# Mictronics/multi-sdr-gps-sim

Measured on NVIDIA H100. Metric: IQ Msamples/s, higher is better.
Workload: dtype f64 NCO / int32 accumulate / int8 out

## Files before the change

### include/gpsb200.h

```cpp
#ifndef GPSB200_H
#define GPSB200_H

#include <stdbool.h>
#include <stddef.h>
#include <stdint.h>

#ifdef __cplusplus
extern "C" {
#endif

#define GPSB200_SAMPLERATE        3000000
#define GPSB200_BLOCK_SAMPLES     300000
#define GPSB200_BLOCK_ELEMS       600000
#define GPSB200_MAX_CHAN          32
#define GPSB200_NAV_WORDS         60
#define GPSB200_CA_LEN            1023
#define GPSB200_SC08              1
#define GPSB200_SC16              2
#define GPSB200_HACKRF_BUFFER     262144

enum {
    GPSB200_OK = 0,
    GPSB200_ERR_ARG = -1,
    GPSB200_ERR_CUDA = -2,
    GPSB200_ERR_RANGE = -3,
    GPSB200_ERR_NOMEM = -4,
    GPSB200_ERR_INTERNAL = -5,
    GPSB200_ERR_END = -6
};

typedef struct gpsb200_chan {
    int32_t prn;
    int32_t iword;
    int32_t ibit;
    int32_t icode;
    int32_t nav_frame;
    int32_t reserved;
    double f_carr;
    double f_code;
    double carr_phase;
    double code_phase;
    double gain;
} gpsb200_chan_t;

typedef struct gpsb200_config {
    int32_t device;
    int32_t max_chan;
    int32_t max_blocks;
    int32_t max_nav_frames;
    int32_t host_threads;
    int32_t run_samples;
} gpsb200_config_t;

typedef struct gpsb200_ctx gpsb200_ctx_t;

typedef struct gpsb200_stats {
    double host_chain_ms;
    double h2d_ms, kernel_ms, d2h_ms;
    double checkpoint_kernel_ms, synth_kernel_ms, probe_kernel_ms;
    int64_t h2d_bytes, d2h_bytes;
    int32_t launches;
    int32_t chain_fallbacks;
} gpsb200_stats_t;

int gpsb200_create(const gpsb200_config_t *cfg, gpsb200_ctx_t **out);
void gpsb200_destroy(gpsb200_ctx_t *ctx);
const char *gpsb200_last_error(const gpsb200_ctx_t *ctx);
const char *gpsb200_version(void);

int gpsb200_bind_numa(int device);

int gpsb200_set_nav(gpsb200_ctx_t *ctx, int frame, int chan, const uint32_t dwrd[GPSB200_NAV_WORDS]);

int gpsb200_synth_blocks(gpsb200_ctx_t *ctx, const gpsb200_chan_t *chans, int nblk, int nchan,
                         int sample_size, void *dst, double *carr_phase_out, gpsb200_stats_t *stats);

int gpsb200_synth_blocks_scatter(gpsb200_ctx_t *ctx, const gpsb200_chan_t *chans, int nblk, int nchan,
                                 int sample_size, void *const *dst_blocks, double *carr_phase_out,
                                 gpsb200_stats_t *stats);

int gpsb200_synth_blocks_device(gpsb200_ctx_t *ctx, const gpsb200_chan_t *chans, int nblk, int nchan,
                                int sample_size, void *dst_device, void *stream,
                                double *carr_phase_out, gpsb200_stats_t *stats);

typedef struct gpsb200_slice_link {
    int32_t prn_first[GPSB200_MAX_CHAN];
    int32_t prn_last[GPSB200_MAX_CHAN];
    int32_t reset_inside[GPSB200_MAX_CHAN];
    double first_phase[GPSB200_MAX_CHAN];
    double value[GPSB200_MAX_CHAN];
} gpsb200_slice_link_t;
int gpsb200_slice_prepare(gpsb200_ctx_t *ctx, const gpsb200_chan_t *chans, int nblk, int nchan, int sample_size,
                          void *dst_device, void *dst_host, void *stream, gpsb200_slice_link_t *link);
int gpsb200_slice_wait(gpsb200_ctx_t *ctx);
int gpsb200_slice_probe(gpsb200_ctx_t *ctx, const int32_t *prn_in, const double *phase_guess_in, int eager);
int gpsb200_slice_finish(gpsb200_ctx_t *ctx, const int32_t *prn_in, const double *phase_in, int32_t *prn_out,
                         double *phase_out, gpsb200_stats_t *stats);
typedef void (*gpsb200_handoff_fn)(void *user, const int32_t *prn_out, const double *phase_out);
int gpsb200_slice_finish_cb(gpsb200_ctx_t *ctx, const int32_t *prn_in, const double *phase_in, int32_t *prn_out,
                            double *phase_out, gpsb200_stats_t *stats, gpsb200_handoff_fn handoff, void *user);
int gpsb200_slice_link_host(const gpsb200_chan_t *chans, int nblk, int nchan, gpsb200_slice_link_t *link);
int gpsb200_link_apply(const gpsb200_slice_link_t *link, int nchan, const int32_t *prn_in, const double *phase_in,
                       int32_t *prn_out, double *phase_out);

int gpsb200_debug_corrupt_chain(gpsb200_ctx_t *ctx, int on);

int gpsb200_debug_run_checkpoints(gpsb200_ctx_t *ctx, int nblk, int nchan, void *out);

int gpsb200_debug_block_probes(gpsb200_ctx_t *ctx, int nblk, int nchan, void *probes_out, double *seg_out,
                               double *guess_out);

int gpsb200_debug_synth_shape(gpsb200_ctx_t *ctx, int nblk, int nchan, int sample_size, const char **kernel,
                              int *ctas_per_block, int *runs_per_cta);

const char *gpsb200_synth_kernel_name(const gpsb200_ctx_t *ctx, int nchan);

int gpsb200_replay_device(gpsb200_ctx_t *ctx, void *dst_device, void *stream, int kernel_mask);

double gpsb200_carrier_advance(double carr_phase, double f_carr, int64_t nsamples);

int gpsb200_carrier_chain(const gpsb200_chan_t *chans, int nblk, int nchan, const double *phase_in,
                          double *phase_out, int threads);

int gpsb200_carrier_chain_device(gpsb200_ctx_t *ctx, const gpsb200_chan_t *chans, int nblk, int nchan,
                                 const double *phase_in, double *phase_out);

int gpsb200_carrier_probe_fixup(double start, double guess, double f_carr, int64_t nsamples, double *end_out);

int gpsb200_span_chain_host(const double *f_carr, int nblk, double start_true, double start_guess, double *starts_out);

int gpsb200_checkpoint_segments_host(double start_true, double start_guess, double f_carr, int run_samples,
                                     double *starts_out, int *nseg_out);

int gpsb200_carrier_probe_host(double guess, double f_carr, int64_t nsamples, int run_samples, int mode, void *probe_out,
                               double *seg_out);

int gpsb200_lanes_model_block(const gpsb200_chan_t *chans, int nchan, const uint32_t *nav, int run_samples, int force,
                              int16_t *iq, double *carr_out, int64_t *counters, uint32_t *signs);

int gpsb200_lanes_window_band_host(const uint32_t *steps, const uint32_t *bases, int64_t n, uint8_t *out);

int gpsb200_codegen(int prn, uint8_t ca[GPSB200_CA_LEN]);

#define GPSB200_ACQ_MAX_MS    100
#define GPSB200_ACQ_MAX_BINS  1024
#define GPSB200_ACQ_CODE_SAMPLES 3000
typedef struct gpsb200_acq_config {
    int64_t s0;
    int32_t ms;
    int32_t nprn;
    int32_t prn[32];
    double f_lo_hz;
    double step_hz;
    int32_t nbins;
    int32_t reserved;
} gpsb200_acq_config_t;
typedef struct gpsb200_acq_result {
    int32_t prn;
    int32_t bin;
    int32_t delay;
    int32_t reserved;
    double doppler_hz;
    double delay_chips;
    uint64_t p1, p2;
    double ratio;
} gpsb200_acq_result_t;
int gpsb200_acquire(gpsb200_ctx_t *ctx, const void *iq, int64_t nsamples, int sample_size, const gpsb200_acq_config_t *cfg,
                    gpsb200_acq_result_t *res, uint64_t *grid);
int gpsb200_acquire_device(gpsb200_ctx_t *ctx, const void *iq_device, int64_t nsamples, int sample_size,
                           const gpsb200_acq_config_t *cfg, gpsb200_acq_result_t *res, uint64_t *grid, void *stream);
int gpsb200_acquire_windows(gpsb200_ctx_t *ctx, const void *iq, int64_t nsamples, int sample_size,
                            const gpsb200_acq_config_t *cfg, const double *f_lo_prn, gpsb200_acq_result_t *res,
                            uint64_t *grid);
int gpsb200_debug_acq_split(gpsb200_ctx_t *ctx, int force, int nprn, int nbins);
int gpsb200_acquire_windows_device(gpsb200_ctx_t *ctx, const void *iq_device, int64_t nsamples, int sample_size,
                                   const gpsb200_acq_config_t *cfg, const double *f_lo_prn, gpsb200_acq_result_t *res,
                                   uint64_t *grid, void *stream);

#define GPSB200_TRK_CODE_STEP_NOM 1464583848u
#define GPSB200_TRK_CODE_STEP_MIN 1464095816u
#define GPSB200_TRK_CODE_STEP_MAX 1465072205u
#define GPSB200_TRK_FLL_EPOCHS    200
#define GPSB200_TRK_MAX_CHAN      32
typedef struct gpsb200_track_state {
    int32_t prn;
    int32_t epochs;
    int64_t sample;
    uint64_t code_phase;
    int64_t carr_freq;
    uint32_t carr_phase;
    int32_t carr_step;
    uint32_t code_step;
    int32_t prev_i, prev_q;
    int32_t lock_i, lock_q;
    int32_t lock;
} gpsb200_track_state_t;
typedef struct gpsb200_track_epoch {
    int64_t sample;
    int32_t e_i, e_q, p_i, p_q, l_i, l_q;
    uint32_t carr_phase;
    int32_t carr_step;
    uint32_t code_phase;
    uint32_t code_step;
    int32_t lock;
    int32_t reserved;
} gpsb200_track_epoch_t;
int gpsb200_track_start(int prn, double doppler_hz, int64_t sample, gpsb200_track_state_t *state);
int gpsb200_track(gpsb200_ctx_t *ctx, const void *iq, int64_t nsamples, int sample_size, int64_t base,
                  gpsb200_track_state_t *state, int nchan, int max_epochs, gpsb200_track_epoch_t *epochs,
                  int32_t *nepochs);
int gpsb200_track_device(gpsb200_ctx_t *ctx, const void *iq_device, int64_t nsamples, int sample_size, int64_t base,
                         gpsb200_track_state_t *state, int nchan, int max_epochs, gpsb200_track_epoch_t *epochs,
                         int32_t *nepochs, void *stream);

typedef struct gpsb200_nav_bit {
    int64_t sample;
    int64_t sum;
    int32_t value;
    int32_t locked;
} gpsb200_nav_bit_t;
typedef struct gpsb200_nav_word {
    int64_t sample;
    uint32_t raw;
    uint32_t data;
    int32_t parity_ok;
    int32_t subframe;
    int32_t tow;
    int32_t index;
} gpsb200_nav_word_t;
typedef struct gpsb200_nav_sync {
    int32_t bit_edge;
    int32_t nbits;
    int32_t frame_bit;
    int32_t inverted;
    int32_t nwords;
    int32_t words_ok;
    int32_t subframes;
    int32_t first_tow;
} gpsb200_nav_sync_t;
int gpsb200_nav_decode(const gpsb200_track_epoch_t *epochs, int64_t n, gpsb200_nav_bit_t *bits, int64_t max_bits,
                       gpsb200_nav_word_t *words, int64_t max_words, gpsb200_nav_sync_t *sync);
int gpsb200_nav_word_check(uint32_t word, uint32_t prev, uint32_t *data);
uint32_t gpsb200_nav_parity(uint32_t data24, int d29, int d30);

typedef struct gpsb200_ephemeris {
    int32_t valid;
    int32_t week;
    int32_t iodc, iode;
    int32_t health;
    int32_t ura;
    int32_t reserved[2];
    double toc;
    double af0, af1, af2;
    double tgd;
    double toe;
    double m0, deltan;
    double ecc, sqrta;
    double omg0, inc0, aop;
// ... 362 lines not shown
```

### multi-sdr-gps-sim_b200/api.py

```python
import ctypes as C
import os

import numpy as np

BLOCK_SAMPLES = 300000
BLOCK_ELEMS = 600000
SC08, SC16 = 1, 2

_HERE = os.path.dirname(os.path.abspath(__file__))


def lib_path():
    return os.path.join(_HERE, "libgpsb200.so")


class GpsB200Error(RuntimeError):
    def __init__(self, code, msg):
        super().__init__("gpsb200 error %d: %s" % (code, msg))
        self.code = code


class Chan(C.Structure):
    _fields_ = [("prn", C.c_int32), ("iword", C.c_int32), ("ibit", C.c_int32), ("icode", C.c_int32),
                ("nav_frame", C.c_int32), ("reserved", C.c_int32),
# ... 221 lines not shown
    c["t_a"], c["s_a"], c["week"], c["nodes"] = float(t_a), int(s_a), int(week), int(nodes)
    return c


SNAPSHOT_CONFIG_DTYPE = np.dtype([("min_ratio", "<f8"), ("iterations", "<i4"), ("reserved", "<i4")])
SNAPSHOT_DTYPE = np.dtype([("prn", "<i4"), ("status", "<i4"), ("sample", "<i8"), ("code_phase", "<u8"),
                           ("code_step", "<u4"), ("carr_step", "<i4"), ("iterations", "<i4"), ("last_step", "<i4"),
                           ("power", "<u8"), ("ratio", "<f8")])
assert (SNAPSHOT_CONFIG_DTYPE.itemsize, SNAPSHOT_DTYPE.itemsize) == (16, 56)
SNAP_OK, SNAP_WEAK, SNAP_NO_CONVERGENCE = 0, 1, 2
SNAP_ITERATIONS, SNAP_MAX_ITER = 12, 16
SNAP_BATCH_SCRATCH = 256 << 20


def snapshot_batch_pass(nprn, nbins, ms, sample_size=SC08):
    b = nprn * nbins * 24028 + nprn * 128 + 8 + acq_window_samples(ms) * 2 * int(sample_size)
    return max(1, SNAP_BATCH_SCRATCH // b)


def snapshot_config(min_ratio=2.5, iterations=SNAP_ITERATIONS):
    c = np.zeros(1, SNAPSHOT_CONFIG_DTYPE)[0]
    c["min_ratio"], c["iterations"] = float(min_ratio), int(iterations)
    return c


COLLECTIVE_CONFIG_DTYPE = np.dtype([("n", "<i4", 4), ("step", "<f8", 4), ("mask_deg", "<f8"), ("distinct_m", "<f8"),
                                    ("reserved", "<i8")])
COLLECTIVE_DTYPE = np.dtype([("status", "<i4"), ("nused", "<i4"), ("used", "<u4"), ("shift", "<i4"), ("winner", "<i4"),
                             ("runner", "<i4"), ("score", "<u4"), ("runner_score", "<u4"), ("o_t", "<f8"),
                             ("x", "<f8", 3), ("lat_deg", "<f8"), ("lon_deg", "<f8"), ("height", "<f8"),
                             ("runner_dist", "<f8")])
CD_SCORE_DTYPE = np.dtype([("score", "<u4"), ("shift", "<i4")])
CD_CELL_DTYPE = np.dtype([("bin", "<i4"), ("delay", "<i4")])
assert (COLLECTIVE_CONFIG_DTYPE.itemsize, COLLECTIVE_DTYPE.itemsize) == (72, 96)
CD_OK, CD_FEW, CD_AMBIGUOUS = 0, 1, 2
CD_MAX_HYP, CD_MIN_USED, CD_Q_SHIFT, CD_Q_CAP, CD_AMBIGUOUS_PCT = 1 << 24, 4, 8, 8192, 90


def collective_config(ext_m, step_m, ext_s=0.0, step_s=1.0, up_ext_m=0.0, up_step_m=1.0, mask_deg=5.0,
                      distinct_m=None):
    c = np.zeros(1, COLLECTIVE_CONFIG_DTYPE)[0]
    for a, (e, st) in enumerate(((ext_m, step_m), (ext_m, step_m), (up_ext_m, up_step_m), (ext_s, step_s))):
        c["n"][a] = 2 * int(np.floor(float(e) / float(st) + 1e-9)) + 1 if e > 0 else 1
        c["step"][a] = float(st)
    c["mask_deg"] = float(mask_deg)
    c["distinct_m"] = 2.0 * float(step_m) if distinct_m is None else float(distinct_m)
    return c


def search_nodes(n=SEARCH_NODES):
    xyz = np.zeros((max(1, int(n)), 3))
    rc = lib().gpsb200_search_nodes(int(n), xyz.ctypes.data)
    if rc:
        raise GpsB200Error(rc, "gpsb200_search_nodes")
    return xyz


def rinex_ephemeris(path, week, sow, rinex3=False):
    eph = np.zeros(32, EPHEMERIS_DTYPE)
    rc = lib().gpsb200_rinex_ephemeris(os.fsencode(str(path)), int(bool(rinex3)), int(week), float(sow), eph.ctypes.data)
    if rc:
        raise GpsB200Error(rc, "gpsb200_rinex_ephemeris")
    return eph


def raim_thresholds(p_fa, p_md):
    T, lam = np.zeros(RAIM_MAX_DOF), np.zeros(RAIM_MAX_DOF)
    rc = lib().gpsb200_raim_thresholds(float(p_fa), float(p_md), T.ctypes.data, lam.ctypes.data)
    if rc:
        raise GpsB200Error(rc, "gpsb200_raim_thresholds")
    return T, lam


def nav_words_of_frame(words60):
    w = np.asarray(words60, np.uint32) & 0x3FFFFFFF
    out = np.zeros(w.size, NAV_WORD_DTYPE)
    prev = 0
    for i, raw in enumerate(w):
        ok, data = nav_word_check(int(raw), prev)
        out[i]["raw"], out[i]["data"], out[i]["parity_ok"], out[i]["index"] = int(raw), data, int(ok), i
        out[i]["subframe"], out[i]["tow"] = ((data >> 2) & 7, (data >> 7) & 0x1FFFF) if i % 10 == 1 else (0, -1)
        prev = int(raw)
    return out


def nav_ephemeris(words):
    w = np.ascontiguousarray(words, dtype=NAV_WORD_DTYPE)
    eph, iono = np.zeros(1, EPHEMERIS_DTYPE), np.zeros(1, IONO_DTYPE)
    rc = lib().gpsb200_nav_ephemeris(w.ctypes.data if w.size else None, w.size, eph.ctypes.data, iono.ctypes.data)
    if rc:
        raise GpsB200Error(rc, "gpsb200_nav_ephemeris")
    return eph[0], iono[0]


def nav_almanac(words, week):
    w = np.ascontiguousarray(words, dtype=NAV_WORD_DTYPE)
    rec = np.zeros(32, ALMANAC_RECORD_DTYPE)
    wna = C.c_int32(0)
    rc = lib().gpsb200_nav_almanac(w.ctypes.data if w.size else None, w.size, int(week), rec.ctypes.data, C.byref(wna))
    if rc:
        raise GpsB200Error(rc, "gpsb200_nav_almanac")
    return rec, int(wna.value)


SKY_DTYPE = np.dtype([("prn", "<i4"), ("valid", "<i4"), ("el_deg", "<f8"), ("az_deg", "<f8"), ("range_m", "<f8"),
                      ("doppler_hz", "<f8")])
assert SKY_DTYPE.itemsize == 40


def almanac_predict(rec, week, sow, x_a):
    r = np.ascontiguousarray(rec, dtype=ALMANAC_RECORD_DTYPE)
    assert r.size == 32
    x = np.ascontiguousarray(x_a, dtype=np.float64).reshape(3)
    out = np.zeros(32, SKY_DTYPE)
    rc = lib().gpsb200_almanac_predict(r.ctypes.data, int(week), float(sow), x.ctypes.data, out.ctypes.data)
    if rc:
        raise GpsB200Error(rc, "gpsb200_almanac_predict")
    return out


def nav_time_anchor(words, sync):
    w = np.ascontiguousarray(words, dtype=NAV_WORD_DTYPE)
    sy = np.array(sync, dtype=NAV_SYNC_DTYPE).reshape(1)
    ep, ms = C.c_int32(0), C.c_int64(0)
    rc = lib().gpsb200_nav_time_anchor(w.ctypes.data if w.size else None, w.size, sy.ctypes.data, C.byref(ep), C.byref(ms))
    if rc:
        raise GpsB200Error(rc, "gpsb200_nav_time_anchor")
    return int(ep.value), int(ms.value)


def pvt_config(s0, step, nfix, iono=None):
    c = np.zeros(1, PVT_CONFIG_DTYPE)[0]
    c["s0"], c["step"], c["nfix"] = int(s0), int(step), int(nfix)
    if iono is not None:
        c["iono"] = 1
        c["alpha"], c["beta"] = np.asarray(iono[0], np.float64), np.asarray(iono[1], np.float64)
    return c


HANDOFF_FN = C.CFUNCTYPE(None, C.c_void_p, C.POINTER(C.c_int32), C.POINTER(C.c_double))

_lib = None

EXPORTS = ["gpsb200_create", "gpsb200_destroy", "gpsb200_last_error", "gpsb200_version", "gpsb200_set_nav",
           "gpsb200_synth_blocks", "gpsb200_synth_blocks_scatter", "gpsb200_synth_blocks_device", "gpsb200_replay_device",
           "gpsb200_carrier_advance", "gpsb200_carrier_chain", "gpsb200_carrier_chain_device", "gpsb200_carrier_probe_fixup",
           "gpsb200_codegen", "gpsb200_acquire", "gpsb200_acquire_device", "gpsb200_acquire_windows",
           "gpsb200_acquire_windows_device", "gpsb200_debug_acq_split", "gpsb200_nav_almanac", "gpsb200_almanac_predict", "gpsb200_track_start",
           "gpsb200_track",
           "gpsb200_track_device", "gpsb200_nav_decode", "gpsb200_nav_word_check", "gpsb200_nav_parity",
           "gpsb200_nav_ephemeris", "gpsb200_nav_time_anchor", "gpsb200_pvt", "gpsb200_pvt_replay",
           "gpsb200_pvt_raim", "gpsb200_raim_thresholds", "gpsb200_pvt_araim", "gpsb200_araim_kfa", "gpsb200_pvt_coarse", "gpsb200_pvt_search", "gpsb200_search_nodes", "gpsb200_snapshot_measure", "gpsb200_snapshot_measure_device", "gpsb200_snapshot_batch", "gpsb200_snapshot_batch_device", "gpsb200_pvt_snapshot", "gpsb200_pvt_snapshot_search", "gpsb200_collective", "gpsb200_collective_device", "gpsb200_rinex_ephemeris", "gpsb200_bind_numa", "gpsb200_span_chain_host", "gpsb200_lanes_model_block",
           "gpsb200_lanes_window_band_host", "gpsb200_slice_prepare", "gpsb200_slice_probe",
           "gpsb200_slice_finish", "gpsb200_slice_finish_cb", "gpsb200_slice_wait", "gpsb200_link_apply", "gpsb200_slice_link_host", "gpsb200_debug_corrupt_chain", "gpsb200_synth_kernel_name",
           "gpsb200_debug_run_checkpoints", "gpsb200_checkpoint_segments_host",
           "gpsb200_carrier_probe_host", "gpsb200_debug_block_probes", "gpsb200_debug_synth_shape",
           "gpsb200_scenario_create", "gpsb200_scenario_destroy", "gpsb200_scenario_error",
           "gpsb200_scenario_blocks", "gpsb200_scenario_channels", "gpsb200_scenario_nav_frames",
           "gpsb200_scenario_chans", "gpsb200_scenario_nav", "gpsb200_scenario_almanac_date", "gpsb200_almanac_read",
           "gpsb200_scenario_open", "gpsb200_scenario_advance", "gpsb200_scenario_frame", "gpsb200_scenario_key",
           "gpsb200_scenario_steer_state", "gpsb200_scenario_open_now", "gpsb200_scenario_create_now",
           "gpsb200_scenario_start_date", "gpsb200_scenario_start_time",
           "fifo_create", "fifo_destroy", "fifo_wait_next", "fifo_wait_full", "fifo_halt", "fifo_acquire",
           "fifo_enqueue", "fifo_dequeue", "fifo_release", "fifo_set_compat_drop",
           "gpsb200_iqfile_start", "gpsb200_iqfile_stop", "gpsb200_fifo_push", "gpsb200_fifo_push_flush"]


def lib():
    global _lib
    if _lib is None:
        if not os.path.exists(lib_path()):
            raise GpsB200Error(-2, "libgpsb200.so not built (run __graft_entry__.build()); there is no CPU fallback")
        L = C.CDLL(lib_path())
        L.gpsb200_create.argtypes = [C.POINTER(Config), C.POINTER(C.c_void_p)]
        L.gpsb200_destroy.argtypes = [C.c_void_p]
        L.gpsb200_last_error.argtypes = [C.c_void_p]
        L.gpsb200_last_error.restype = C.c_char_p
        L.gpsb200_version.restype = C.c_char_p
        L.gpsb200_set_nav.argtypes = [C.c_void_p, C.c_int, C.c_int, C.c_void_p]
        L.gpsb200_synth_blocks.argtypes = [C.c_void_p, C.c_void_p, C.c_int, C.c_int, C.c_int, C.c_void_p,
                                           C.c_void_p, C.POINTER(Stats)]
        L.gpsb200_synth_blocks_scatter.argtypes = [C.c_void_p, C.c_void_p, C.c_int, C.c_int, C.c_int, C.c_void_p,
                                                   C.c_void_p, C.POINTER(Stats)]
        L.gpsb200_synth_blocks_device.argtypes = [C.c_void_p, C.c_void_p, C.c_int, C.c_int, C.c_int, C.c_void_p,
                                                  C.c_void_p, C.c_void_p, C.POINTER(Stats)]
        L.gpsb200_replay_device.argtypes = [C.c_void_p, C.c_void_p, C.c_void_p, C.c_int]
        L.gpsb200_carrier_advance.argtypes = [C.c_double, C.c_double, C.c_int64]
        L.gpsb200_carrier_advance.restype = C.c_double
        L.gpsb200_codegen.argtypes = [C.c_int, C.c_void_p]
        L.gpsb200_scenario_create.argtypes = [C.POINTER(ScenarioConfig), C.POINTER(C.c_void_p)]
        L.gpsb200_scenario_destroy.argtypes = [C.c_void_p]
        L.gpsb200_scenario_error.argtypes = [C.c_void_p]
        L.gpsb200_scenario_error.restype = C.c_char_p
        for fn in ("blocks", "channels", "nav_frames"):
            getattr(L, "gpsb200_scenario_" + fn).argtypes = [C.c_void_p]
        L.gpsb200_scenario_chans.argtypes = [C.c_void_p]
        L.gpsb200_scenario_chans.restype = C.c_void_p
        L.gpsb200_scenario_nav.argtypes = [C.c_void_p]
        L.gpsb200_scenario_nav.restype = C.c_void_p
        L.gpsb200_scenario_almanac_date.argtypes = [C.c_void_p]
        L.gpsb200_scenario_almanac_date.restype = C.c_char_p
        L.gpsb200_almanac_read.argtypes = [C.c_char_p, C.c_void_p, C.POINTER(C.c_int32)]
        L.gpsb200_scenario_open.argtypes = [C.POINTER(ScenarioConfig), C.POINTER(C.c_void_p)]
        L.gpsb200_scenario_open_now.argtypes = [C.POINTER(ScenarioConfig), C.POINTER(C.c_void_p)]
        L.gpsb200_scenario_create_now.argtypes = [C.POINTER(ScenarioConfig), C.POINTER(C.c_void_p)]
        L.gpsb200_scenario_start_date.argtypes = [C.c_void_p]
        L.gpsb200_scenario_start_date.restype = C.c_char_p
        L.gpsb200_scenario_start_time.argtypes = [C.c_void_p, C.POINTER(C.c_int32), C.POINTER(C.c_double)]
        L.gpsb200_scenario_advance.argtypes = [C.c_void_p, C.c_int, C.c_void_p, C.POINTER(C.c_int32)]
        L.gpsb200_scenario_frame.argtypes = [C.c_void_p, C.c_int]
        L.gpsb200_scenario_frame.restype = C.c_void_p
        L.gpsb200_scenario_key.argtypes = [C.c_void_p, C.c_int]
        L.gpsb200_scenario_steer_state.argtypes = [C.c_void_p, C.POINTER(SteerState)]
        L.gpsb200_carrier_probe_fixup.argtypes = [C.c_double, C.c_double, C.c_double, C.c_int64, C.POINTER(C.c_double)]
        L.gpsb200_carrier_chain_device.argtypes = [C.c_void_p, C.c_void_p, C.c_int, C.c_int, C.c_void_p, C.c_void_p]
        L.gpsb200_carrier_chain.argtypes = [C.c_void_p, C.c_int, C.c_int, C.c_void_p, C.c_void_p, C.c_int]
        L.gpsb200_span_chain_host.argtypes = [C.c_void_p, C.c_int, C.c_double, C.c_double, C.c_void_p]
        L.gpsb200_slice_prepare.argtypes = [C.c_void_p, C.c_void_p, C.c_int, C.c_int, C.c_int, C.c_void_p, C.c_void_p,
                                            C.c_void_p, C.POINTER(SliceLink)]
        L.gpsb200_slice_finish_cb.argtypes = [C.c_void_p, C.c_void_p, C.c_void_p, C.c_void_p, C.c_void_p, C.POINTER(Stats),
                                              HANDOFF_FN, C.c_void_p]
        L.gpsb200_slice_wait.argtypes = [C.c_void_p]
        L.gpsb200_slice_link_host.argtypes = [C.c_void_p, C.c_int, C.c_int, C.POINTER(SliceLink)]
        L.gpsb200_slice_probe.argtypes = [C.c_void_p, C.c_void_p, C.c_void_p, C.c_int]
        L.gpsb200_slice_finish.argtypes = [C.c_void_p, C.c_void_p, C.c_void_p, C.c_void_p, C.c_void_p, C.POINTER(Stats)]
        L.gpsb200_link_apply.argtypes = [C.POINTER(SliceLink), C.c_int, C.c_void_p, C.c_void_p, C.c_void_p, C.c_void_p]
        L.gpsb200_debug_corrupt_chain.argtypes = [C.c_void_p, C.c_int]
        L.gpsb200_debug_run_checkpoints.argtypes = [C.c_void_p, C.c_int, C.c_int, C.c_void_p]
        L.gpsb200_checkpoint_segments_host.argtypes = [C.c_double, C.c_double, C.c_double, C.c_int, C.c_void_p,
                                                       C.POINTER(C.c_int)]
        L.gpsb200_carrier_probe_host.argtypes = [C.c_double, C.c_double, C.c_int64, C.c_int, C.c_int, C.c_void_p,
                                                 C.c_void_p]
        L.gpsb200_debug_block_probes.argtypes = [C.c_void_p, C.c_int, C.c_int, C.c_void_p, C.c_void_p, C.c_void_p]
        L.gpsb200_debug_synth_shape.argtypes = [C.c_void_p, C.c_int, C.c_int, C.c_int, C.POINTER(C.c_char_p),
                                                C.POINTER(C.c_int), C.POINTER(C.c_int)]
        L.gpsb200_synth_kernel_name.argtypes = [C.c_void_p, C.c_int]
        L.gpsb200_synth_kernel_name.restype = C.c_char_p
        L.gpsb200_acquire.argtypes = [C.c_void_p, C.c_void_p, C.c_int64, C.c_int, C.POINTER(AcqConfig), C.c_void_p,
                                      C.c_void_p]
        L.gpsb200_acquire_device.argtypes = [C.c_void_p, C.c_void_p, C.c_int64, C.c_int, C.POINTER(AcqConfig),
                                             C.c_void_p, C.c_void_p, C.c_void_p]
        L.gpsb200_acquire_windows.argtypes = [C.c_void_p, C.c_void_p, C.c_int64, C.c_int, C.POINTER(AcqConfig),
                                              C.c_void_p, C.c_void_p, C.c_void_p]
        L.gpsb200_acquire_windows_device.argtypes = [C.c_void_p, C.c_void_p, C.c_int64, C.c_int, C.POINTER(AcqConfig),
                                                     C.c_void_p, C.c_void_p, C.c_void_p, C.c_void_p]
        L.gpsb200_debug_acq_split.argtypes = [C.c_void_p, C.c_int, C.c_int, C.c_int]
        L.gpsb200_nav_almanac.argtypes = [C.c_void_p, C.c_int64, C.c_int32, C.c_void_p, C.POINTER(C.c_int32)]
        L.gpsb200_almanac_predict.argtypes = [C.c_void_p, C.c_int32, C.c_double, C.c_void_p, C.c_void_p]
        L.gpsb200_track_start.argtypes = [C.c_int, C.c_double, C.c_int64, C.c_void_p]
        L.gpsb200_track.argtypes = [C.c_void_p, C.c_void_p, C.c_int64, C.c_int, C.c_int64, C.c_void_p, C.c_int, C.c_int,
                                    C.c_void_p, C.c_void_p]
        L.gpsb200_track_device.argtypes = [C.c_void_p, C.c_void_p, C.c_int64, C.c_int, C.c_int64, C.c_void_p, C.c_int,
                                           C.c_int, C.c_void_p, C.c_void_p, C.c_void_p]
        L.gpsb200_nav_decode.argtypes = [C.c_void_p, C.c_int64, C.c_void_p, C.c_int64, C.c_void_p, C.c_int64, C.c_void_p]
        L.gpsb200_nav_word_check.argtypes = [C.c_uint32, C.c_uint32, C.POINTER(C.c_uint32)]
        L.gpsb200_nav_parity.argtypes = [C.c_uint32, C.c_int, C.c_int]
        L.gpsb200_nav_parity.restype = C.c_uint32
        L.gpsb200_nav_ephemeris.argtypes = [C.c_void_p, C.c_int64, C.c_void_p, C.c_void_p]
        L.gpsb200_nav_time_anchor.argtypes = [C.c_void_p, C.c_int64, C.c_void_p, C.POINTER(C.c_int32),
                                              C.POINTER(C.c_int64)]
        L.gpsb200_pvt.argtypes = [C.c_void_p, C.c_void_p, C.c_int, C.c_void_p, C.c_void_p, C.c_int, C.c_void_p, C.c_void_p,
                                  C.c_void_p]
        L.gpsb200_pvt_replay.argtypes = [C.c_void_p, C.c_void_p]
        L.gpsb200_pvt_raim.argtypes = [C.c_void_p, C.c_void_p, C.c_int, C.c_void_p, C.c_void_p, C.c_int, C.c_void_p,
                                       C.c_void_p, C.c_void_p, C.c_void_p, C.c_void_p]
        L.gpsb200_raim_thresholds.argtypes = [C.c_double, C.c_double, C.c_void_p, C.c_void_p]
        L.gpsb200_pvt_araim.argtypes = L.gpsb200_pvt_raim.argtypes
        L.gpsb200_araim_kfa.argtypes = [C.c_double, C.c_double, C.c_void_p, C.c_void_p]
        L.gpsb200_pvt_coarse.argtypes = L.gpsb200_pvt_raim.argtypes + [C.c_void_p]
        L.gpsb200_pvt_search.argtypes = L.gpsb200_pvt_coarse.argtypes + [C.c_void_p]
        L.gpsb200_search_nodes.argtypes = [C.c_int, C.c_void_p]
        L.gpsb200_snapshot_measure.argtypes = [C.c_void_p, C.c_void_p, C.c_int64, C.c_int, C.POINTER(AcqConfig),
                                               C.c_void_p, C.c_void_p, C.c_void_p]
        L.gpsb200_snapshot_measure_device.argtypes = L.gpsb200_snapshot_measure.argtypes + [C.c_void_p]
        L.gpsb200_snapshot_batch.argtypes = [C.c_void_p, C.c_void_p, C.c_int64, C.c_int, C.POINTER(AcqConfig), C.c_int,
                                             C.c_void_p, C.c_void_p, C.c_void_p, C.c_void_p, C.c_void_p]
        L.gpsb200_snapshot_batch_device.argtypes = L.gpsb200_snapshot_batch.argtypes + [C.c_void_p]
        L.gpsb200_pvt_snapshot.argtypes = [C.c_void_p, C.c_void_p, C.c_int, C.c_void_p, C.c_void_p, C.c_void_p,
                                           C.c_void_p, C.c_void_p, C.c_void_p, C.c_void_p]
        L.gpsb200_pvt_snapshot_search.argtypes = L.gpsb200_pvt_snapshot.argtypes + [C.c_void_p]
        L.gpsb200_collective.argtypes = [C.c_void_p, C.c_void_p, C.c_int64, C.c_int, C.POINTER(AcqConfig), C.c_void_p,
                                         C.c_void_p, C.c_void_p, C.c_void_p, C.c_void_p, C.c_void_p, C.c_void_p,
                                         C.c_void_p, C.c_void_p]
        L.gpsb200_collective_device.argtypes = L.gpsb200_collective.argtypes + [C.c_void_p]
        L.gpsb200_rinex_ephemeris.argtypes = [C.c_char_p, C.c_int, C.c_int32, C.c_double, C.c_void_p]
        _lib = L
    return _lib


def bind_numa(device=0):
    L = lib()
    L.gpsb200_bind_numa.argtypes = [C.c_int]
    L.gpsb200_bind_numa.restype = C.c_int
    return int(L.gpsb200_bind_numa(int(device)))


def codegen(prn):
    ca = np.zeros(1023, np.uint8)
    rc = lib().gpsb200_codegen(prn, ca.ctypes.data)
    if rc:
        raise GpsB200Error(rc, "gpsb200_codegen(%d)" % prn)
    return ca


def carrier_advance(phase, f_carr, nsamples):
    return lib().gpsb200_carrier_advance(float(phase), float(f_carr), int(nsamples))


def carrier_chain(chans, phase_in=None, threads=16):
    a = np.ascontiguousarray(chans, dtype=CHAN_DTYPE)
    nblk, nchan = a.shape
    out = np.zeros(nchan, np.float64)
    pin = None if phase_in is None else np.ascontiguousarray(phase_in, dtype=np.float64)
    rc = lib().gpsb200_carrier_chain(a.ctypes.data, nblk, nchan, None if pin is None else pin.ctypes.data,
                                     out.ctypes.data, threads)
    if rc:
        raise GpsB200Error(rc, "gpsb200_carrier_chain")
    return out


def lanes_model_block(chans_row, nav_frame, run_samples=2400, force=0, want_signs=False):
    a = np.ascontiguousarray(chans_row, dtype=CHAN_DTYPE)
    nv = np.ascontiguousarray(nav_frame, dtype=np.uint32)
    iq = np.zeros(BLOCK_ELEMS, np.int16)
    co = np.zeros(a.size, np.float64)
    cnt = np.zeros(4, np.int64)
    signs = np.zeros((a.size, BLOCK_SAMPLES // 96, 3), np.uint32) if want_signs else None
    L = lib()
    L.gpsb200_lanes_model_block.argtypes = [C.c_void_p, C.c_int, C.c_void_p, C.c_int, C.c_int, C.c_void_p, C.c_void_p, C.c_void_p,
                                            C.c_void_p]
    rc = L.gpsb200_lanes_model_block(a.ctypes.data, a.size, nv.ctypes.data, run_samples, force, iq.ctypes.data, co.ctypes.data,
                                     cnt.ctypes.data, None if signs is None else signs.ctypes.data)
    if rc:
        raise GpsB200Error(rc, "gpsb200_lanes_model_block")
    return (iq, co, cnt, signs) if want_signs else (iq, co, cnt)


def lanes_window_band(steps, bases):
    st, bs = np.broadcast_arrays(np.asarray(steps, np.uint32), np.asarray(bases, np.uint32))
    st = np.ascontiguousarray(st.ravel())
    bs = np.ascontiguousarray(bs.ravel())
    out = np.zeros(st.size, np.uint8)
    L = lib()
    L.gpsb200_lanes_window_band_host.argtypes = [C.c_void_p, C.c_void_p, C.c_int64, C.c_void_p]
    rc = L.gpsb200_lanes_window_band_host(st.ctypes.data, bs.ctypes.data, st.size, out.ctypes.data)
    if rc:
        raise GpsB200Error(rc, "gpsb200_lanes_window_band_host")
    return out.astype(bool)


def span_chain_host(f_carr, start_true, start_guess):
    f = np.ascontiguousarray(f_carr, dtype=np.float64)
    out = np.zeros(f.size + 1)
    rc = lib().gpsb200_span_chain_host(f.ctypes.data, f.size, float(start_true), float(start_guess), out.ctypes.data)
    if rc < 0:
        raise GpsB200Error(rc, "gpsb200_span_chain_host")
    return out if rc == 1 else None


def checkpoint_segments_host(start_true, start_guess, f_carr, run_samples=2400):
    out = np.zeros(8)
    nseg = C.c_int(0)
    rc = lib().gpsb200_checkpoint_segments_host(float(start_true), float(start_guess), float(f_carr), int(run_samples),
                                            out.ctypes.data, C.byref(nseg))
    if rc < 0:
        raise GpsB200Error(rc, "gpsb200_checkpoint_segments_host")
    return rc == 1, out[:nseg.value]


def carrier_probe_host(guess, f_carr, nsamples=BLOCK_SAMPLES, run_samples=2400, mode=1):
    probe = np.zeros(1, CARRIER_PROBE_DTYPE)
    seg = np.zeros((2, 7))
    rc = lib().gpsb200_carrier_probe_host(float(guess), float(f_carr), int(nsamples), int(run_samples), int(mode),
                                          probe.ctypes.data, seg.ctypes.data)
    if rc:
        raise GpsB200Error(rc, "gpsb200_carrier_probe_host")
    return probe[0], seg


def slice_link_host(chans):
# ... 141 lines not shown
        self._check(lib().gpsb200_scenario_key(self._h, ord(k) if isinstance(k, str) else int(k)))

    def state(self):
        st = SteerState()
        self._check(lib().gpsb200_scenario_steer_state(self._h, C.byref(st)))
        return st

    def run(self, steer, chunk=None):
        events = {}
        for b, keys, rep in steer:
            events[int(b)] = events.get(int(b), "") + keys * int(rep)
        parts, frames = [], {}
        b = 0
        while True:
            if b in events:
                for k in events.pop(b):
                    self.key(k)
            st = self.state()
            if st.next_block >= st.end_block:
                break
            nxt = min([e for e in events if e > b] + [st.end_block])
            n = nxt - b if chunk is None else min(chunk, nxt - b)
            ch = self.advance(n)
            for f in np.unique(ch["nav_frame"]):
                if f not in frames:
                    frames[int(f)] = self.frame(int(f))
            parts.append(ch)
            b += ch.shape[0]
        chans = np.concatenate(parts) if parts else np.zeros((0, self.channels), CHAN_DTYPE)
        nav = np.stack([frames[f] for f in sorted(frames)]) if frames else np.zeros((0, self.channels, 60), np.uint32)
        return chans, nav


class Context:

    def __init__(self, max_chan, max_blocks, device=0, max_nav_frames=1, host_threads=0, run_samples=0):
        self._h = C.c_void_p()
        self.cfg = Config(device, max_chan, max_blocks, max_nav_frames, host_threads, run_samples)
        rc = lib().gpsb200_create(C.byref(self.cfg), C.byref(self._h))
        if rc:
            msg = lib().gpsb200_last_error(self._h).decode() if self._h else "gpsb200_create: bad configuration"
            if self._h:
                lib().gpsb200_destroy(self._h)
                self._h = C.c_void_p()
            raise GpsB200Error(rc, msg)

    def close(self):
        if self._h:
            lib().gpsb200_destroy(self._h)
            self._h = C.c_void_p()

    def __enter__(self):
        return self

    def __exit__(self, *a):
        self.close()

    def _check(self, rc):
        if rc:
            raise GpsB200Error(rc, lib().gpsb200_last_error(self._h).decode())

    def set_nav(self, frame, chan, words):
        w = np.ascontiguousarray(words, dtype=np.uint32)
        assert w.size == 60
        self._check(lib().gpsb200_set_nav(self._h, frame, chan, w.ctypes.data))

    def set_nav_frames(self, frames):
        for f in range(frames.shape[0]):
            for c in range(frames.shape[1]):
                self.set_nav(f, c, frames[f, c])

    @staticmethod
    def _chans(chans):
        a = np.ascontiguousarray(chans, dtype=CHAN_DTYPE)
        assert a.ndim == 2
        return a

    def synth_blocks(self, chans, sample_size=SC08, out=None, want_stats=False):
        a = self._chans(chans)
        nblk, nchan = a.shape
        dt = np.int16 if sample_size == SC16 else np.int8
        if out is None:
            out = np.empty(nblk * BLOCK_ELEMS, dt)
        assert out.dtype == dt and out.size >= nblk * BLOCK_ELEMS and out.flags.c_contiguous
        cp = np.zeros(nchan, np.float64)
        st = Stats()
        self._check(lib().gpsb200_synth_blocks(self._h, a.ctypes.data, nblk, nchan, sample_size,
                                               out.ctypes.data, cp.ctypes.data, C.byref(st)))
        return (out, cp, st) if want_stats else (out, cp)

    def synth_blocks_scatter(self, chans, sample_size, blocks, want_stats=False):
        a = self._chans(chans)
        nblk, nchan = a.shape
        dt = np.int16 if sample_size == SC16 else np.int8
        assert len(blocks) == nblk and all(b.dtype == dt and b.size >= BLOCK_ELEMS and b.flags.c_contiguous for b in blocks)
        ptrs = (C.c_void_p * nblk)(*[b.ctypes.data for b in blocks])
        cp = np.zeros(nchan, np.float64)
        st = Stats()
        self._check(lib().gpsb200_synth_blocks_scatter(self._h, a.ctypes.data, nblk, nchan, sample_size,
                                                       C.cast(ptrs, C.c_void_p), cp.ctypes.data, C.byref(st)))
        return (cp, st) if want_stats else cp

    def synth_blocks_device(self, chans, sample_size, dst_ptr, stream=0, want_stats=False):
        a = self._chans(chans)
        nblk, nchan = a.shape
        cp = np.zeros(nchan, np.float64)
        st = Stats()
        self._check(lib().gpsb200_synth_blocks_device(self._h, a.ctypes.data, nblk, nchan, sample_size,
                                                      C.c_void_p(dst_ptr), C.c_void_p(stream), cp.ctypes.data,
                                                      C.byref(st) if want_stats else None))
        return (cp, st) if want_stats else cp

    def slice_prepare(self, chans, sample_size, dst_ptr=0, stream=0, dst_host=None):
        a = self._chans(chans)
        nblk, nchan = a.shape
        link = SliceLink()
        hp = None if dst_host is None else C.c_void_p(dst_host.ctypes.data)
        self._check(lib().gpsb200_slice_prepare(self._h, a.ctypes.data, nblk, nchan, sample_size, C.c_void_p(dst_ptr),
                                                hp, C.c_void_p(stream), C.byref(link)))
        self._slice_nchan = nchan
        return link

    def slice_probe(self, prn_in=None, phase_guess_in=None, eager=False):
        pi = None if prn_in is None else np.ascontiguousarray(prn_in, dtype=np.int32)
        xi = None if phase_guess_in is None else np.ascontiguousarray(phase_guess_in, dtype=np.float64)
        self._check(lib().gpsb200_slice_probe(self._h, None if pi is None else pi.ctypes.data,
                                              None if xi is None else xi.ctypes.data, 1 if eager else 0))

    def slice_finish(self, prn_in=None, phase_in=None, want_stats=False, handoff=None):
        n = self._slice_nchan
        pi = None if prn_in is None else np.ascontiguousarray(prn_in, dtype=np.int32)
        xi = None if phase_in is None else np.ascontiguousarray(phase_in, dtype=np.float64)
        po, xo = np.zeros(n, np.int32), np.zeros(n, np.float64)
        st = Stats()

        def _cb(_user, p_prn, p_ph):
            handoff(np.ctypeslib.as_array(p_prn, shape=(n,)).copy(), np.ctypeslib.as_array(p_ph, shape=(n,)).copy())

        cb = HANDOFF_FN(_cb) if handoff is not None else C.cast(None, HANDOFF_FN)
        self._check(lib().gpsb200_slice_finish_cb(self._h, None if pi is None else pi.ctypes.data,
                                                  None if xi is None else xi.ctypes.data, po.ctypes.data, xo.ctypes.data,
                                                  C.byref(st), cb, None))
        return (po, xo, st) if want_stats else (po, xo)

    def slice_wait(self):
        self._check(lib().gpsb200_slice_wait(self._h))

    def synth_kernel_name(self, nchan):
        return lib().gpsb200_synth_kernel_name(self._h, int(nchan)).decode()

    def debug_corrupt_chain(self, on):
        self._check(lib().gpsb200_debug_corrupt_chain(self._h, int(on)))

    def debug_run_checkpoints(self, nblk, nchan):
        nruns = BLOCK_SAMPLES // (self.cfg.run_samples or 2400)
        out = np.zeros((nblk, nruns, nchan), RUN_CKPT_DTYPE)
        self._check(lib().gpsb200_debug_run_checkpoints(self._h, nblk, nchan, out.ctypes.data))
        return out

    def debug_block_probes(self, nblk, nchan):
        probes = np.zeros((nblk, nchan), CARRIER_PROBE_DTYPE)
        seg = np.zeros((nblk, nchan, 2, 7))
        guess = np.zeros((nblk, nchan))
        self._check(lib().gpsb200_debug_block_probes(self._h, nblk, nchan, probes.ctypes.data, seg.ctypes.data,
                                                     guess.ctypes.data))
        return probes, seg, guess

    def debug_synth_shape(self, nblk, nchan, sample_size=SC08):
        name, per_block, per_cta = C.c_char_p(), C.c_int(0), C.c_int(0)
        self._check(lib().gpsb200_debug_synth_shape(self._h, int(nblk), int(nchan), int(sample_size), C.byref(name),
                                                    C.byref(per_block), C.byref(per_cta)))
        return name.value.decode(), per_block.value, per_cta.value

    def carrier_chain(self, chans, phase_in=None):
        a = self._chans(chans)
        nblk, nchan = a.shape
        out = np.zeros(nchan, np.float64)
        pin = None if phase_in is None else np.ascontiguousarray(phase_in, dtype=np.float64)
        self._check(lib().gpsb200_carrier_chain_device(self._h, a.ctypes.data, nblk, nchan,
                                                       None if pin is None else pin.ctypes.data, out.ctypes.data))
        return out

    def acquire(self, iq=None, sample_size=SC08, prns=range(1, 33), ms=10, s0=0, f_lo=-5000.0, step=250.0, nbins=41,
                want_grid=False, device_ptr=None, nsamples=None, stream=0):
        return self._acquire(None, iq, sample_size, [int(p) for p in prns], ms, s0, f_lo, step, nbins, want_grid,
                             device_ptr, nsamples, stream)

    def acquire_windows(self, iq=None, sample_size=SC08, prns=(), f_lo_prn=(), step=250.0, nbins=5, ms=10, s0=0,
                        want_grid=False, device_ptr=None, nsamples=None, stream=0):
        prns = [int(p) for p in prns]
        flo = np.ascontiguousarray(f_lo_prn, dtype=np.float64).reshape(-1)
        if flo.size != len(prns):
            raise GpsB200Error(ERR_ARG, "acquire_windows: %d first bins for %d PRNs" % (flo.size, len(prns)))
        return self._acquire(flo, iq, sample_size, prns, ms, s0, 0.0, step, nbins, want_grid, device_ptr, nsamples,
                             stream)

    def _acquire(self, f_lo_prn, iq, sample_size, prns, ms, s0, f_lo, step, nbins, want_grid, device_ptr, nsamples,
                 stream):
        cfg = self._acq_config(prns, ms, s0, f_lo, step, nbins)
        res = np.zeros(max(1, min(len(prns), 32)), ACQ_RESULT_DTYPE)
        grid = np.zeros((max(1, len(prns)), max(1, int(nbins)), ACQ_CODE_SAMPLES), np.uint64) if want_grid else None
        gp = None if grid is None else grid.ctypes.data
        src, n, dev = self._rx_source(iq, device_ptr, nsamples, stream)
        if f_lo_prn is None:
            fn, fp = lib().gpsb200_acquire_device if dev else lib().gpsb200_acquire, ()
        else:
            fn = lib().gpsb200_acquire_windows_device if dev else lib().gpsb200_acquire_windows
            fp = (f_lo_prn.ctypes.data if f_lo_prn.size else None,)
        self._check(fn(self._h, src, n, int(sample_size), C.byref(cfg), *fp, res.ctypes.data, gp, *dev))
        return (res, grid) if want_grid else res

    @staticmethod
    def _acq_config(prns, ms, s0, f_lo, step, nbins):
        cfg = AcqConfig()
        cfg.s0, cfg.ms, cfg.nprn = int(s0), int(ms), len(prns)
        for i, p in enumerate(prns[:32]):
            cfg.prn[i] = p
        cfg.f_lo_hz, cfg.step_hz, cfg.nbins = float(f_lo), float(step), int(nbins)
        return cfg

    @staticmethod
    def _rx_source(iq, device_ptr, nsamples, stream):
        if device_ptr is not None:
            assert iq is None and nsamples is not None
            return C.c_void_p(device_ptr), int(nsamples), (C.c_void_p(stream),)
        a = np.ascontiguousarray(iq)
        n = a.size // 2 if nsamples is None else int(nsamples)
        assert n <= a.size // 2
        return a.ctypes, n, ()

    def debug_acq_split(self, nprn, nbins, force=-1):
        rc = lib().gpsb200_debug_acq_split(self._h, int(force), int(nprn), int(nbins))
        if rc < 0:
            self._check(rc)
        return rc

    def track(self, states, iq=None, sample_size=SC08, base=0, max_epochs=None, device_ptr=None, nsamples=None, stream=0):
        st = np.array(states, dtype=TRACK_STATE_DTYPE).reshape(-1).copy()
        nchan = st.size
        src, n, dev = self._rx_source(iq, device_ptr, nsamples, stream)
        me = int(max_epochs) if max_epochs is not None else n // 2999 + 1
        out = np.zeros((max(1, nchan), max(1, me)), TRACK_EPOCH_DTYPE)
        cnt = np.zeros(max(1, nchan), np.int32)
        fn = lib().gpsb200_track_device if dev else lib().gpsb200_track
        self._check(fn(self._h, src, n, int(sample_size), int(base), st.ctypes.data, nchan, me, out.ctypes.data,
                       cnt.ctypes.data, *dev))
        return [out[c, :cnt[c]].copy() for c in range(nchan)], st

    def pvt(self, chans, epochs, cfg, want_residuals=False, nepochs=None):
        ch, nchan, ep, n, me, cf, fixes, res = self._pvt_args(chans, epochs, cfg, want_residuals, nepochs)
        self._check(lib().gpsb200_pvt(self._h, ch.ctypes.data, nchan, ep.ctypes.data, n.ctypes.data, me, cf.ctypes.data,
                                      fixes.ctypes.data, None if res is None else res.ctypes.data))
        return (fixes, res) if want_residuals else fixes

    def pvt_raim(self, chans, epochs, cfg, raim, want_residuals=False, nepochs=None):
        ch, nchan, ep, n, me, cf, fixes, res = self._pvt_args(chans, epochs, cfg, want_residuals, nepochs)
        rc = np.array(raim, dtype=RAIM_CONFIG_DTYPE).reshape(1)
        out = np.zeros(fixes.size, RAIM_DTYPE)
        self._check(lib().gpsb200_pvt_raim(self._h, ch.ctypes.data, nchan, ep.ctypes.data, n.ctypes.data, me,
                                           cf.ctypes.data, rc.ctypes.data, fixes.ctypes.data,
                                           None if res is None else res.ctypes.data, out.ctypes.data))
        return (fixes, out, res) if want_residuals else (fixes, out)

    def pvt_araim(self, chans, epochs, cfg, araim, want_residuals=False, nepochs=None):
        ch, nchan, ep, n, me, cf, fixes, res = self._pvt_args(chans, epochs, cfg, want_residuals, nepochs)
        ac = np.array(araim, dtype=ARAIM_CONFIG_DTYPE).reshape(1)
        out = np.zeros(fixes.size, ARAIM_DTYPE)
        self._check(lib().gpsb200_pvt_araim(self._h, ch.ctypes.data, nchan, ep.ctypes.data, n.ctypes.data, me,
                                            cf.ctypes.data, ac.ctypes.data, fixes.ctypes.data,
                                            None if res is None else res.ctypes.data, out.ctypes.data))
        return (fixes, out, res) if want_residuals else (fixes, out)

    def pvt_coarse(self, chans, epochs, cfg, apriori, want_residuals=False, want_ms=False, nepochs=None):
        ch, nchan, ep, n, me, cf, fixes, res = self._pvt_args(chans, epochs, cfg, want_residuals, nepochs)
        ap = np.array(apriori, dtype=COARSE_CONFIG_DTYPE).reshape(1)
        out = np.zeros(fixes.size, COARSE_DTYPE)
        ms = np.zeros((fixes.size, max(1, nchan)), np.int64) if want_ms else None
        self._check(lib().gpsb200_pvt_coarse(self._h, ch.ctypes.data, nchan, ep.ctypes.data, n.ctypes.data, me,
                                             cf.ctypes.data, ap.ctypes.data, fixes.ctypes.data,
                                             None if res is None else res.ctypes.data, out.ctypes.data,
                                             None if ms is None else ms.ctypes.data))
        return (fixes, out) + ((res,) if want_residuals else ()) + ((ms,) if want_ms else ())

    def pvt_search(self, chans, epochs, cfg, search, want_residuals=False, want_ms=False, want_node_rms=False,
                   nepochs=None):
        ch, nchan, ep, n, me, cf, fixes, res = self._pvt_args(chans, epochs, cfg, want_residuals, nepochs)
        sc = np.array(search, dtype=SEARCH_CONFIG_DTYPE).reshape(1)
        out = np.zeros(fixes.size, SEARCH_DTYPE)
        ms = np.zeros((fixes.size, max(1, nchan)), np.int64) if want_ms else None
        nr = np.zeros((fixes.size, max(1, int(sc[0]["nodes"]))), np.float64) if want_node_rms else None
        self._check(lib().gpsb200_pvt_search(self._h, ch.ctypes.data, nchan, ep.ctypes.data, n.ctypes.data, me,
                                             cf.ctypes.data, sc.ctypes.data, fixes.ctypes.data,
                                             None if res is None else res.ctypes.data, out.ctypes.data,
                                             None if ms is None else ms.ctypes.data,
                                             None if nr is None else nr.ctypes.data))
        return ((fixes, out) + ((res,) if want_residuals else ()) + ((ms,) if want_ms else ())
                + ((nr,) if want_node_rms else ()))

    def snapshot_measure(self, res, iq=None, sample_size=SC08, ms=10, s0=0, prns=None, f_lo=-5000.0, step=250.0,
                         nbins=41, cfg=None, device_ptr=None, nsamples=None, stream=0):
        r = np.ascontiguousarray(res, dtype=ACQ_RESULT_DTYPE).reshape(-1)
        prns = [int(p) for p in (r["prn"] if prns is None else prns)]
        acq = self._acq_config(prns, ms, s0, f_lo, step, nbins)
        sc = np.array(snapshot_config() if cfg is None else cfg, dtype=SNAPSHOT_CONFIG_DTYPE).reshape(1)
        if r.size < len(prns):
            raise GpsB200Error(ERR_ARG, "snapshot_measure: %d results for %d PRNs" % (r.size, len(prns)))
# ... 125 lines not shown
```

### multi-sdr-gps-sim_b200/csrc/gpsb200_api.cu

```cuda
#include <cuda_runtime.h>
#include <sched.h>

#include <algorithm>
#include <atomic>
#include <chrono>
#include <condition_variable>
#include <functional>
#include <mutex>
#include <cctype>
#include <cmath>
#include <cstdio>
#include <cstring>
#include <memory>
#include <string>
#include <thread>
#include <vector>

#include "../../include/gpsb200.h"
#include "acquire.h"
#include "snapshot.h"
#include "collective.h"
#include "device_buffer.h"
#include "track.h"
#include "pvt.h"
#include "nco_exact.h"
#include "synth_kernels.h"
#include "synth_lanes.h"
#include "synth_tables.h"

using namespace gpsb200;

namespace {

constexpr int kSynthChunk = 256;
constexpr int kSegFirst = 256;
constexpr int kSegBlocks = 1024;
constexpr int kSpanBlocks = 32;
constexpr int kHostChainBlocks = 2;

struct ChainState {
    int prn = 0;
    double phase = 0.0;
};

class WorkerPool {
public:
    explicit WorkerPool(int n) {
        for (int i = 0; i < n; i++) th_.emplace_back([this, i] { loop(i); });
    }
    ~WorkerPool() {
        {
            std::lock_guard<std::mutex> lk(mu_);
            stop_ = true;
        }
        cv_.notify_all();
        for (auto &t : th_) t.join();
    }
    int size() const { return (int) th_.size(); }
    void run(int n, const std::function<void(int, int)> &job) {
        const int parts = std::max(1, std::min(size(), n));
        if (parts <= 1 || th_.empty()) {
            job(0, n);
            return;
        }
        std::unique_lock<std::mutex> lk(mu_);
        job_ = &job;
        n_ = n;
        parts_ = parts;
        pending_ = parts;
        ++epoch_;
        cv_.notify_all();
        done_.wait(lk, [this] { return pending_ == 0; });
        job_ = nullptr;
    }

private:
    void loop(int id) {
        uint64_t seen = 0;
        for (;;) {
            const std::function<void(int, int)> *job;
            int n, parts;
            {
                std::unique_lock<std::mutex> lk(mu_);
                cv_.wait(lk, [&] { return stop_ || epoch_ != seen; });
                if (stop_) return;
                seen = epoch_;
                job = job_;
                n = n_;
                parts = parts_;
            }
            if (id < parts) {
                const int per = (n + parts - 1) / parts, lo = id * per, hi = std::min(n, lo + per);
                if (lo < hi) (*job)(lo, hi);
                std::lock_guard<std::mutex> lk(mu_);
                if (--pending_ == 0) done_.notify_all();
            }
        }
    }
    std::vector<std::thread> th_;
    std::mutex mu_;
    std::condition_variable cv_, done_;
    const std::function<void(int, int)> *job_ = nullptr;
    int n_ = 0, parts_ = 0, pending_ = 0;
    uint64_t epoch_ = 0;
    bool stop_ = false;
};

std::vector<std::pair<int, int>> segments_of(int nblk) {
    std::vector<std::pair<int, int>> v;
    int len = kSegFirst;
    for (int b0 = 0; b0 < nblk; len = kSegBlocks) {
        const int b1 = std::min(nblk, b0 + len);
        v.emplace_back(b0, b1);
        b0 = b1;
    }
    return v;
}

struct Call {
    const gpsb200_chan_t *chans = nullptr;
    int nblk = 0, nchan = 0, sample_size = 0;
    void *dst = nullptr;
    void *dst_host = nullptr;
    void *const *scatter = nullptr;
    cudaStream_t stream = nullptr;
    std::vector<std::pair<int, int>> segs;
    std::vector<ChainState> chain;
    std::vector<std::vector<ChainState>> after;
    std::vector<int64_t> slow;
    int rows = 0;
    int ichunk = 0;
    gpsb200_stats_t st{};
    bool active = false, eager = false, probed = false, finished = false;

    Call() = default;
    Call(const gpsb200_chan_t *chans_, int nblk_, int nchan_, int sample_size_, void *dst_, void *dst_host_,
         void *const *scatter_, cudaStream_t stream_)
        : chans(chans_), nblk(nblk_), nchan(nchan_), sample_size(sample_size_), dst(dst_), dst_host(dst_host_),
          scatter(scatter_), stream(stream_), chain(nchan_) {
        plan(segments_of(nblk_));
    }
    void plan(std::vector<std::pair<int, int>> s) {
        segs = std::move(s);
        after.assign(segs.size(), {});
        slow.assign(segs.size(), 0);
    }
    bool host() const { return dst_host || scatter; }
};

enum { kEvCallStart, kEvProbeStart, kEvProbeEnd, kEvCkptStart, kEvCkptEnd, kEvCallEnd, kCallEvents };

}

struct gpsb200_ctx {
    gpsb200_config_t cfg{};
    int nruns = 0;
    cudaStream_t s_compute = nullptr, s_copy = nullptr, s_pre = nullptr, s_ck = nullptr;
    cudaEvent_t ev[kCallEvents]{};
    std::vector<cudaEvent_t> ev_done;
    BlockChanDev *d_bc = nullptr, *h_bc = nullptr;
    RunCkpt *d_ck = nullptr, *h_ck = nullptr;
    uint32_t *d_nav = nullptr, *h_nav = nullptr;
    uint32_t *d_chips = nullptr;
    int32_t *d_atab = nullptr;
    double *d_carr_end = nullptr;
    int *d_chain_errors = nullptr, *h_chain_errors = nullptr;
    double *d_guess = nullptr, *h_guess = nullptr;
    std::vector<uint8_t> h_guess_abs;
    std::vector<uint8_t> h_span_flags;
    double *d_carr0 = nullptr, *h_carr0 = nullptr;
    CarrierProbe *d_probe = nullptr;
    CarrierProbe *h_probe = nullptr, *d_probe_host = nullptr;
    double *d_seg = nullptr;
    CarrierProbe *h_span_sum = nullptr, *d_span_sum = nullptr;
    SpanBlockState *d_spec = nullptr;
    bool lanes_on = true;
    bool lanes_veto = false;
    SpanRes *d_span_res = nullptr, *h_span_res = nullptr;
    int max_spans = 0;
    double *h_seg_end = nullptr, *d_seg_end = nullptr;
    std::vector<double> seg_expect;
    std::vector<cudaEvent_t> ev_seg;
    int fault_inject_chain = 0;
    bool trace_on = false;
    double trace_t0 = 0.0;
    Call call;
    uint8_t *d_out = nullptr;
    size_t out_bytes = 0;
    uint8_t *d_rx = nullptr;
    size_t rx_bytes = 0;
    int8_t *d_rx_chips = nullptr;
    bool nav_dirty = true;
    std::unique_ptr<WorkerPool> pool;
    SynthArgs last{};
    bool have_last = false;
    acq::Scratch acq;
    trk::Scratch trk;
    pvt::Scratch pvt;
    snap::Scratch snap;
    cd::Scratch cd;
    std::string err;
};

namespace {

struct OneSatellite {
    const double *cc;
    __host__ __device__ void operator()(int j, double &c, int32_t &prn) const {
        c = cc[j];
        prn = 1;
    }
};

double now_ms();
void trace(gpsb200_ctx *ctx, const char *what);

int fail(gpsb200_ctx *c, int code, const std::string &msg) {
    if (c) c->err = msg;
    return code;
}

#define CU(call)                                                                              \
    do {                                                                                      \
        cudaError_t e_ = (call);                                                              \
        if (e_ != cudaSuccess)                                                                \
            return fail(ctx, GPSB200_ERR_CUDA, std::string(#call) + ": " + cudaGetErrorString(e_)); \
    } while (0)

double now_ms() {
    using namespace std::chrono;
    return duration<double, std::milli>(steady_clock::now().time_since_epoch()).count();
}

void trace(gpsb200_ctx *ctx, const char *what) {
    if (!ctx->trace_on) return;
    const double t = now_ms();
    fprintf(stderr, "[gpsb200 dev %d +%8.3f ms] %s (%d host workers)\n", ctx->cfg.device, t - ctx->trace_t0, what,
            ctx->pool ? ctx->pool->size() : 0);
}

inline uint64_t phase_to_fix(double p) { return (p >= 0.0 && p < 1.0) ? (uint64_t) (p * 0x1p64) : 0; }
inline double fix_to_phase(uint64_t a) { return (double) (a >> 11) * 0x1p-53; }
inline uint64_t step_to_fix(double c) {
    const uint64_t m = (uint64_t) (std::fabs(c) * 0x1p64);
    return c < 0.0 ? (uint64_t) 0 - m : m;
}
inline uint64_t guess_block(uint64_t acc, double c) {
    acc += (uint64_t) GPSB200_BLOCK_SAMPLES * step_to_fix(c);
    return acc + (uint64_t) (int64_t) ((double) GPSB200_BLOCK_SAMPLES * carrier_drift_per_step(c) * 0x1p64);
}


int prepare_blocks(gpsb200_ctx *ctx, const gpsb200_chan_t *chans, int b0, int b1, int nchan,
                   const std::vector<ChainState> &chain, gpsb200_slice_link_t *link = nullptr,
                   std::vector<ChainState> *end_guess = nullptr) {
    const double delt = 1.0 / (double) GPSB200_SAMPLERATE;
    std::vector<int> status(nchan, GPSB200_OK);
    std::vector<uint8_t> lanes_bad(nchan, 0);
    ctx->pool->run(nchan, [&](int c_lo, int c_hi) {
        for (int c = c_lo; c < c_hi; c++) {
            uint64_t acc = phase_to_fix(chain[c].phase);
            int prev_prn = chain[c].prn;
            bool absolute = link == nullptr;
            if (link) {
                acc = 0;
                prev_prn = chans[(size_t) b0 * nchan + c].prn;
                link->prn_first[c] = prev_prn;
                link->first_phase[c] = prev_prn > 0 ? chans[(size_t) b0 * nchan + c].carr_phase : 0.0;
            }
            int span_first_prn = 0;
            uint8_t span_idle = 1, span_uniform = 1;
            for (int b = b0; b < b1; b++) {
                const gpsb200_chan_t &in = chans[(size_t) b * nchan + c];
                const size_t i = (size_t) b * nchan + c;
                BlockChanDev &o = ctx->h_bc[i];
                memset(&o, 0, sizeof o);
                if (b % kSpanBlocks == 0) {
                    span_first_prn = in.prn;
                    span_idle = span_uniform = 1;
                }
                span_idle &= in.prn <= 0;
                span_uniform &= in.prn == span_first_prn;
                if ((b + 1) % kSpanBlocks == 0 || b + 1 == b1)
                    ctx->h_span_flags[(size_t) (b / kSpanBlocks) * nchan + c] = (uint8_t) (span_idle | (span_uniform << 1));
                ctx->h_guess[i] = 0.0;
                ctx->h_guess_abs[i] = absolute ? 1 : 0;
                if (in.prn <= 0) {
                    prev_prn = 0;
                    absolute = true;
                    continue;
                }
                if (in.prn > 32 || in.iword < 0 || in.iword >= GPSB200_NAV_WORDS || in.ibit < 0 || in.ibit >= 30 ||
                    in.icode < 0 || in.icode >= 20 || in.nav_frame < 0 || in.nav_frame >= ctx->cfg.max_nav_frames ||
                    !(in.code_phase >= 0.0 && in.code_phase < 1023.0) ||
                    !(in.f_code > 0.0 && in.f_code <= 1.07e6) ||
                    !(std::isfinite(in.f_carr) && std::fabs(in.f_carr) < 2.9e6) || !std::isfinite(in.gain)) {
                    status[c] = GPSB200_ERR_ARG;
                    return;
                }
                if (!(in.carr_phase >= 0.0 && in.carr_phase < 1.0)) {
                    status[c] = GPSB200_ERR_ARG;
                    return;
                }
                if (in.prn != prev_prn) {
                    acc = phase_to_fix(in.carr_phase);
                    absolute = true;
                }
                ctx->h_guess_abs[i] = absolute ? 1 : 0;
                prev_prn = in.prn;
                o.c_carr = in.f_carr * delt;
                o.c_code = in.f_code * delt;
                if (!lanes::code_step_ok(o.c_code) || !(std::fabs(o.c_carr) < 0.5)) lanes_bad[c] = 1;
                o.gain = in.gain;
                o.carr_in = in.carr_phase;
                o.code0 = in.code_phase;
                o.prn = in.prn;
                o.nav0 = (uint32_t) in.iword | ((uint32_t) in.ibit << 8) | ((uint32_t) in.icode << 16);
                o.frame = in.nav_frame;
                ctx->h_guess[i] = fix_to_phase(acc);
                acc = guess_block(acc, o.c_carr);
            }
            if (end_guess) {
                (*end_guess)[c].prn = prev_prn > 0 ? prev_prn : 0;
                (*end_guess)[c].phase = prev_prn > 0 ? fix_to_phase(acc) : 0.0;
            }
            if (link) {
                link->prn_last[c] = prev_prn > 0 ? prev_prn : 0;
                link->reset_inside[c] = absolute ? 1 : 0;
                link->value[c] = fix_to_phase(acc);
            }
        }
    });
    for (int c = 0; c < nchan; c++)
        if (status[c] != GPSB200_OK) return fail(ctx, status[c], "invalid channel parameters in slot " + std::to_string(c));
    for (int c = 0; c < nchan; c++)
        if (lanes_bad[c]) ctx->lanes_veto = true;
    for (int b = b0; b < b1; b++) {
        double amp = 0.0;
        for (int c = 0; c < nchan; c++) amp += std::fabs(ctx->h_bc[(size_t) b * nchan + c].gain) * 250.0;
        if (amp > 32767.0) return fail(ctx, GPSB200_ERR_RANGE, "sum of channel amplitudes exceeds int16 range");
    }
    return GPSB200_OK;
}

void finalize_guesses(gpsb200_ctx *ctx, int b0, int b1, int nchan, const int32_t *prn_in, const double *phase_in) {
    ctx->pool->run(nchan, [&](int c_lo, int c_hi) {
        for (int c = c_lo; c < c_hi; c++) {
            const BlockChanDev &first = ctx->h_bc[(size_t) b0 * nchan + c];
            const bool cont = prn_in && phase_in && first.prn > 0 && prn_in[c] == first.prn;
            const double off = cont ? phase_in[c] : first.carr_in;
            for (int b = b0; b < b1; b++) {
                const size_t i = (size_t) b * nchan + c;
                if (ctx->h_guess_abs[i] || ctx->h_bc[i].prn <= 0) continue;
                double g = ctx->h_guess[i] + off;
                if (g >= 1.0) g -= 1.0;
                if (!(g >= 0.0 && g < 1.0)) g = 0.0;
                ctx->h_guess[i] = g;
            }
        }
    });
}

void reanchor_guesses(gpsb200_ctx *ctx, int b0, int b1, int nchan, const std::vector<ChainState> &chain) {
    ctx->pool->run(nchan, [&](int c_lo, int c_hi) {
        for (int c = c_lo; c < c_hi; c++) {
            const BlockChanDev &first = ctx->h_bc[(size_t) b0 * nchan + c];
            if (first.prn <= 0 || chain[c].prn != first.prn) continue;
            double delta = chain[c].phase - ctx->h_guess[(size_t) b0 * nchan + c];
            if (delta > 0.5) delta -= 1.0;
            if (delta < -0.5) delta += 1.0;
            for (int b = b0; b < b1; b++) {
                const size_t i = (size_t) b * nchan + c;
                if (ctx->h_bc[i].prn != first.prn) break;
                double g = ctx->h_guess[i] + delta;
                if (g >= 1.0) g -= 1.0;
                if (g < 0.0) g += 1.0;
                if (!(g >= 0.0 && g < 1.0)) g = 0.0;
                ctx->h_guess[i] = g;
            }
        }
    });
}

inline int resolve_block(ChainState &st, const BlockChanDev &bc, const CarrierProbe &probe, double &start_out) {
    if (bc.prn <= 0) {
        st.prn = 0;
        start_out = 0.0;
        return 0;
    }
    if (st.prn != bc.prn) st.phase = bc.carr_in;
    st.prn = bc.prn;
    start_out = st.phase;
    double xe;
    if (carrier_fixup(st.phase, bc.c_carr, probe, xe)) {
        st.phase = xe;
        return 0;
    }
    int64_t dummy = 0;
    nco_advance<NCO_CARRIER>(st.phase, bc.c_carr, GPSB200_BLOCK_SAMPLES, dummy);
    return 1;
}

int64_t resolve_chain(gpsb200_ctx *ctx, int b0, int b1, int nchan, std::vector<ChainState> &chain, int64_t *spans_slow) {
    std::vector<int64_t> fallbacks(nchan, 0), slow(nchan, 0);
    const int K = kSpanBlocks;
    const int nspan = (b1 - b0 + K - 1) / K;
    ctx->pool->run(nchan, [&](int c_lo, int c_hi) {
        for (int c = c_lo; c < c_hi; c++) {
            ChainState st = chain[c];
            for (int sp = 0; sp < nspan; sp++) {
                const int s0 = b0 + sp * K, s1 = std::min(b1, s0 + K);
                SpanRes &res = ctx->h_span_res[(size_t) (s0 / K) * nchan + c];
                const BlockChanDev &first = ctx->h_bc[(size_t) s0 * nchan + c];
                const uint8_t flags = ctx->h_span_flags[(size_t) (s0 / K) * nchan + c];
                const bool idle = flags & 1, uniform = flags & 2;
                res.start = res.shift = 0.0;
                res.variant = 0;
                if (idle) {
                    res.mode = 2;
                    st.prn = 0;
                    continue;
                }
                if (uniform && first.prn > 0) {
                    const double start = st.prn == first.prn ? st.phase : first.carr_in;
                    const CarrierProbe &sum = ctx->h_span_sum[(size_t) (s0 / K) * nchan + c];
                    double xe, d;
                    int v;
                    if (carrier_fixup(start, first.c_carr, sum, xe, &v, &d, 1.0)) {
                        res.mode = 0;
                        res.start = start;
                        res.shift = d;
                        res.variant = v;
                        st.prn = first.prn;
                        st.phase = xe;
                        continue;
                    }
                }
                res.mode = 1;
                ++slow[c];
                for (int b = s0; b < s1; b++) {
                    const size_t i = (size_t) b * nchan + c;
                    fallbacks[c] += resolve_block(st, ctx->h_bc[i], ctx->h_probe[i], ctx->h_carr0[i]);
                }
            }
            chain[c] = st;
        }
    });
    if (ctx->fault_inject_chain == 1 && b1 - b0 > 6) {
        SpanRes &r = ctx->h_span_res[(size_t) (b0 / K) * nchan];
        if (r.mode == 0) r.shift += 0x1p-51;
        else if (r.mode == 1) ctx->h_carr0[(size_t) (b0 + 5) * nchan] += 0x1p-51;
    }
    int64_t n = 0;
    for (int c = 0; c < nchan; c++) {
        n += fallbacks[c];
        if (spans_slow) *spans_slow += slow[c];
    }
    return n;
}

SynthArgs make_args(gpsb200_ctx *ctx, int blk0, int nblk, int nchan, int sample_size, void *out) {
    SynthArgs a{};
    const size_t off = (size_t) blk0 * nchan;
    a.bc = ctx->d_bc + off;
    a.carr0 = ctx->d_carr0 + off;
    a.guess = ctx->d_guess + off;
    a.probe = ctx->d_probe + off;
    a.probe_host = ctx->d_probe_host + off;
    a.seg = ctx->d_seg + off * kSegStates;
    a.spec = ctx->d_spec + off;
    a.span_blocks = kSpanBlocks;
    a.nspan = (nblk + kSpanBlocks - 1) / kSpanBlocks;
    a.span_sum = ctx->d_span_sum + (size_t) (blk0 / kSpanBlocks) * nchan;
    a.span_res = ctx->d_span_res + (size_t) (blk0 / kSpanBlocks) * nchan;
    a.ck = ctx->d_ck + off * ctx->nruns;
    a.nav = ctx->d_nav;
    a.nav_stride = ctx->cfg.max_chan;
    a.chipbits = ctx->d_chips;
    a.atab = ctx->d_atab + (size_t) blk0 * kAtabRows * 32;
    a.carr_end = ctx->d_carr_end + off;
    a.chain_errors = ctx->d_chain_errors;
    a.out = out;
    a.nblk = nblk;
    a.nchan = nchan;
    a.nruns = ctx->nruns;
    a.run_samples = ctx->cfg.run_samples;
    a.iq16 = sample_size == GPSB200_SC16;
    a.lanes = ctx->lanes_on && !ctx->lanes_veto ? 1 : 0;
    const int grp = nchan > 16 ? 32 : (nchan > 8 ? 16 : 8);
    const int rpw = 32 / grp;
    int per_cta = 24 * rpw;
    const int ctas = (ctx->nruns + per_cta - 1) / per_cta;
    per_cta = (ctx->nruns + ctas - 1) / ctas;
    a.runs_per_cta = per_cta;
    a.ctas_per_block = ctas;
    return a;
}

SynthArgs call_args(gpsb200_ctx *ctx, const Call &call, int b0, int nb) {
    const size_t blk_bytes = (size_t) GPSB200_BLOCK_ELEMS * call.sample_size;
    return make_args(ctx, b0, nb, call.nchan, call.sample_size, (char *) call.dst + (size_t) b0 * blk_bytes);
}

int upload_nav(gpsb200_ctx *ctx, cudaStream_t s) {
    if (!ctx->nav_dirty) return GPSB200_OK;
    const size_t bytes = (size_t) ctx->cfg.max_nav_frames * ctx->cfg.max_chan * GPSB200_NAV_WORDS * 4;
    CU(cudaMemcpyAsync(ctx->d_nav, ctx->h_nav, bytes, cudaMemcpyHostToDevice, s));
    ctx->nav_dirty = false;
    return GPSB200_OK;
}

int check_entry(gpsb200_ctx *ctx) {
    if (!ctx->s_compute) return fail(ctx, GPSB200_ERR_CUDA, "context has no CUDA device");
    if (ctx->call.active) return fail(ctx, GPSB200_ERR_ARG, "a call begun with gpsb200_slice_prepare has not been finished");
    CU(cudaSetDevice(ctx->cfg.device));
    return GPSB200_OK;
}

int check_call(gpsb200_ctx *ctx, const gpsb200_chan_t *chans, int nblk, int nchan, int sample_size, void *dst) {
    if (!chans || !dst || nblk < 1 || nblk > ctx->cfg.max_blocks || nchan < 1 || nchan > ctx->cfg.max_chan ||
        (sample_size != GPSB200_SC08 && sample_size != GPSB200_SC16))
        return fail(ctx, GPSB200_ERR_ARG, "bad arguments (1 <= nchan <= cfg.max_chan; 1 <= nblk <= cfg.max_blocks)");
    return check_entry(ctx);
}

int check_aligned(gpsb200_ctx *ctx, const void *p, const char *fn, const char *arg) {
    if ((reinterpret_cast<uintptr_t>(p) & 15u) != 0)
        return fail(ctx, GPSB200_ERR_ARG, std::string(fn) + ": " + arg + " is not 16-byte aligned");
    return GPSB200_OK;
}

int ensure_staging(gpsb200_ctx *ctx, int sample_size) {
    CU(grow(ctx->d_out, ctx->out_bytes, (size_t) ctx->cfg.max_blocks * GPSB200_BLOCK_ELEMS * sample_size));
    return GPSB200_OK;
}

int rx_source(gpsb200_ctx *ctx, const char *fn, const void *iq, int64_t first, int64_t count, int sample_size,
              bool device, cudaStream_t s, const void **dev) {
    int rc = device ? check_aligned(ctx, iq, fn, "iq_device") : GPSB200_OK;
    if (!rc) rc = check_entry(ctx);
    if (rc) return rc;
    const size_t elem = sample_size == GPSB200_SC16 ? 4 : 2;
    *dev = static_cast<const char *>(iq) + (size_t) first * elem;
    if (device) return GPSB200_OK;
    CU(grow(ctx->d_rx, ctx->rx_bytes, (size_t) count * elem));
    if (count) CU(cudaMemcpyAsync(ctx->d_rx, *dev, (size_t) count * elem, cudaMemcpyHostToDevice, s));
    *dev = ctx->d_rx;
    return GPSB200_OK;
}

int settle(gpsb200_ctx *ctx, cudaStream_t caller, int rc) {
    if (rc == GPSB200_OK) return rc;
    ctx->call.active = false;
    if (!ctx->s_compute) return rc;
    if (caller) cudaStreamSynchronize(caller);
    cudaStreamSynchronize(ctx->s_compute);
    cudaStreamSynchronize(ctx->s_pre);
    cudaStreamSynchronize(ctx->s_ck);
    cudaStreamSynchronize(ctx->s_copy);
    return rc;
}

cudaStream_t caller_stream(gpsb200_ctx *ctx, void *stream_) {
    return stream_ ? (cudaStream_t) stream_ : ctx->s_compute;
}


int call_open(gpsb200_ctx *ctx, const Call &call) {
    CU(cudaEventRecord(ctx->ev[kEvCallStart], call.stream));
    CU(cudaStreamWaitEvent(ctx->s_pre, ctx->ev[kEvCallStart], 0));
    CU(cudaStreamWaitEvent(ctx->s_ck, ctx->ev[kEvCallStart], 0));
    const int rc = upload_nav(ctx, ctx->s_pre);
    if (rc) return rc;
    CU(cudaMemsetAsync(ctx->d_chain_errors, 0, sizeof(int), ctx->s_pre));
    return GPSB200_OK;
}

int seg_params(gpsb200_ctx *ctx, Call &call, int b0, int b1, cudaStream_t sp, std::vector<ChainState> *guessed,
               gpsb200_slice_link_t *link) {
    const size_t off = (size_t) b0 * call.nchan, cnt = (size_t) (b1 - b0) * call.nchan;
    const double t0 = now_ms();
    const int rc = prepare_blocks(ctx, call.chans, b0, b1, call.nchan, guessed ? *guessed : call.chain, link, guessed);
    if (rc) return rc;
    call.st.host_chain_ms += now_ms() - t0;
    CU(cudaMemcpyAsync(ctx->d_bc + off, ctx->h_bc + off, cnt * sizeof(BlockChanDev), cudaMemcpyHostToDevice, sp));
    call.st.h2d_bytes += (int64_t) (cnt * sizeof(BlockChanDev));
    if (call.dst) {
        CU(launch_tables(call_args(ctx, call, b0, b1 - b0), sp));
        call.st.launches += 1;
    }
    return GPSB200_OK;
}

int seg_probe(gpsb200_ctx *ctx, Call &call, int b0, int b1, cudaStream_t sp) {
    const size_t off = (size_t) b0 * call.nchan, cnt = (size_t) (b1 - b0) * call.nchan;
    SynthArgs a = make_args(ctx, b0, b1 - b0, call.nchan, call.sample_size, nullptr);
    if (!call.dst) a.ck = nullptr;
    CU(cudaMemcpyAsync(ctx->d_guess + off, ctx->h_guess + off, cnt * sizeof(double), cudaMemcpyHostToDevice, sp));
    if (b0 == 0) CU(cudaEventRecord(ctx->ev[kEvProbeStart], sp));
    CU(launch_probe(a, sp));
    CU(launch_chain(a, sp));
    if (b0 == 0) CU(cudaEventRecord(ctx->ev[kEvProbeEnd], sp));
    call.st.launches += 2;
    call.st.h2d_bytes += (int64_t) (cnt * sizeof(double));
    call.st.d2h_bytes += (int64_t) (cnt * sizeof(CarrierProbe) + (size_t) a.nspan * call.nchan * sizeof(CarrierProbe));
    return GPSB200_OK;
}

int seg_scan(gpsb200_ctx *ctx, Call &call, int i, cudaEvent_t probes_done, cudaStream_t sp) {
    if (probes_done) CU(cudaEventSynchronize(probes_done));
    else CU(cudaStreamSynchronize(sp));
    const double t0 = now_ms();
    call.slow[i] = 0;
    call.st.chain_fallbacks +=
        (int32_t) resolve_chain(ctx, call.segs[i].first, call.segs[i].second, call.nchan, call.chain, &call.slow[i]);
    call.st.host_chain_ms += now_ms() - t0;
    call.after[i] = call.chain;
    return GPSB200_OK;
}

int download(gpsb200_ctx *ctx, Call &call, int b0, int b1, cudaStream_t s) {
    const size_t blk_bytes = (size_t) GPSB200_BLOCK_ELEMS * call.sample_size;
    const char *src = (const char *) call.dst;
    if (call.scatter) {
        for (int b = b0; b < b1; b++)
            CU(cudaMemcpyAsync(call.scatter[b], src + (size_t) b * blk_bytes, blk_bytes, cudaMemcpyDeviceToHost, s));
    } else {
        CU(cudaMemcpyAsync((char *) call.dst_host + (size_t) b0 * blk_bytes, src + (size_t) b0 * blk_bytes,
                           (size_t) (b1 - b0) * blk_bytes, cudaMemcpyDeviceToHost, s));
    }
    call.st.d2h_bytes += (int64_t) (b1 - b0) * (int64_t) blk_bytes;
    return GPSB200_OK;
}

int seg_commit(gpsb200_ctx *ctx, Call &call, int i0, int i1, cudaStream_t sp) {
    const int b0 = call.segs[i0].first, b1 = call.segs[i1 - 1].second, nchan = call.nchan;
    const size_t off = (size_t) b0 * nchan, cnt = (size_t) (b1 - b0) * nchan;
    int64_t slow = 0;
    for (int i = i0; i < i1; i++) slow += call.slow[i];
    SynthArgs a = call_args(ctx, call, b0, b1 - b0);
    const size_t soff = (size_t) (b0 / kSpanBlocks) * nchan, scnt = (size_t) a.nspan * nchan;
    if (b0 == 0) CU(cudaEventRecord(ctx->ev[kEvCkptStart], sp));
    CU(cudaMemcpyAsync(ctx->d_span_res + soff, ctx->h_span_res + soff, scnt * sizeof(SpanRes), cudaMemcpyHostToDevice, sp));
    call.st.h2d_bytes += (int64_t) (scnt * sizeof(SpanRes));
    if (slow > 0) {
        CU(cudaMemcpyAsync(ctx->d_carr0 + off, ctx->h_carr0 + off, cnt * sizeof(double), cudaMemcpyHostToDevice, sp));
        call.st.h2d_bytes += (int64_t) (cnt * sizeof(double));
    }
    const int jm = ckpt_segments(ctx->nruns) / 2;
    if (ctx->fault_inject_chain == 2 && b1 - b0 > 6 && jm >= 1) {
        double *p = ctx->d_seg + (size_t) (b0 + 5) * nchan * kSegStates, h[kSegStates];
        CU(cudaMemcpyAsync(h, p, sizeof h, cudaMemcpyDeviceToHost, sp));
        CU(cudaStreamSynchronize(sp));
        h[jm - 1] += 0x1p-51;
        h[kCkptSegs - 1 + jm - 1] += 0x1p-51;
        CU(cudaMemcpyAsync(p, h, sizeof h, cudaMemcpyHostToDevice, sp));
        CU(cudaStreamSynchronize(sp));
    }
    SynthArgs ack = a;
    ack.last_end_host = ctx->d_seg_end + (size_t) i0 * nchan;
    CU(launch_checkpoints(ack, sp));
    if (b0 == 0) CU(cudaEventRecord(ctx->ev[kEvCkptEnd], sp));
    call.st.launches += 1;
    for (int c = 0; c < nchan; c++) {
        const ChainState &e = call.after[i1 - 1][c];
        const bool live = e.prn > 0 && ctx->h_bc[(size_t) (b1 - 1) * nchan + c].prn == e.prn;
        ctx->seg_expect[(size_t) i0 * nchan + c] = live ? e.phase : -1.0;
    }
    call.rows = i0 + 1;
    CU(cudaEventRecord(ctx->ev_done[call.ichunk], sp));
    CU(cudaStreamWaitEvent(call.stream, ctx->ev_done[call.ichunk], 0));
    call.ichunk++;
    if (!call.host()) {
        CU(launch_synth(a, call.stream));
        call.st.launches += 1;
        return GPSB200_OK;
    }
    for (int c0 = b0, nc = 0; c0 < b1; c0 += nc, call.ichunk++) {
        nc = c0 == 0 ? 32 : (c0 == 32 ? 96 : (c0 == 128 ? 128 : kSynthChunk));
        nc = std::min(nc, b1 - c0);
        CU(launch_synth(call_args(ctx, call, c0, nc), call.stream));
        call.st.launches += 1;
        CU(cudaEventRecord(ctx->ev_done[call.ichunk], call.stream));
        CU(cudaStreamWaitEvent(ctx->s_copy, ctx->ev_done[call.ichunk], 0));
        const int rc = download(ctx, call, c0, c0 + nc, ctx->s_copy);
        if (rc) return rc;
    }
    return GPSB200_OK;
}

int call_close(gpsb200_ctx *ctx, const Call &call, cudaStream_t sp) {
    CU(cudaEventRecord(ctx->ev[kEvCallEnd], call.stream));
    CU(cudaMemcpyAsync(ctx->h_chain_errors, ctx->d_chain_errors, sizeof(int), cudaMemcpyDeviceToHost, sp));
    ctx->last = call_args(ctx, call, 0, call.nblk);
    ctx->have_last = true;
    return GPSB200_OK;
}

int call_verdict(gpsb200_ctx *ctx, const Call &call) {
    int bad = *ctx->h_chain_errors;
    for (int i = 0; i < call.rows; i++)
        for (int c = 0; c < call.nchan; c++) {
            const double want = ctx->seg_expect[(size_t) i * call.nchan + c];
            if (want >= 0.0 && f64_bits(want) != f64_bits(ctx->h_seg_end[(size_t) i * call.nchan + c])) ++bad;
        }
    if (bad != 0)
        return fail(ctx, GPSB200_ERR_INTERNAL, "carrier chain self-check failed on " + std::to_string(bad) + " blocks");
    return GPSB200_OK;
}

void seed_chain(std::vector<ChainState> &chain, int nchan, const int32_t *prn_in, const double *phase_in) {
    for (int c = 0; c < nchan; c++) {
        chain[c].prn = (prn_in && phase_in && prn_in[c] > 0) ? prn_in[c] : 0;
        chain[c].phase = chain[c].prn ? phase_in[c] : 0.0;
    }
}

void export_chain(const std::vector<ChainState> &chain, int nchan, int32_t *prn_out, double *phase_out) {
    for (int c = 0; c < nchan; c++) {
        if (prn_out) prn_out[c] = chain[c].prn;
        if (phase_out) phase_out[c] = chain[c].prn > 0 ? chain[c].phase : 0.0;
    }
}

int small_call(gpsb200_ctx *ctx, Call &call, double *carr_phase_out, gpsb200_stats_t *stats) {
    const int nblk = call.nblk, nchan = call.nchan;
    cudaStream_t s = call.stream;
    double t0 = now_ms();
    int rc = prepare_blocks(ctx, call.chans, 0, nblk, nchan, call.chain);
    if (rc) return rc;
    const int nruns = ctx->nruns, run = ctx->cfg.run_samples;
    ctx->pool->run(nchan, [&](int c_lo, int c_hi) {
        for (int c = c_lo; c < c_hi; c++) {
            ChainState stc = call.chain[c];
            for (int b = 0; b < nblk; b++) {
                const BlockChanDev &p = ctx->h_bc[(size_t) b * nchan + c];
                RunCkpt *ck = ctx->h_ck + (size_t) b * nruns * nchan + c;
                if (p.prn <= 0) {
                    stc.prn = 0;
                    for (int r = 0; r < nruns; r++) ck[(size_t) r * nchan] = RunCkpt{0.0, 0.0, 0u, 0u};
                    continue;
                }
                if (stc.prn != p.prn) stc.phase = p.carr_in;
                stc.prn = p.prn;
                double x = stc.phase, y = p.code0;
                int iword = p.nav0 & 0xFF, ibit = (p.nav0 >> 8) & 0xFF, icode = (p.nav0 >> 16) & 0xFF;
                const WalkConst wx = walk_const(p.c_carr), wy = walk_const(p.c_code);
                for (int r = 0; r < nruns; r++) {
                    ck[(size_t) r * nchan] = RunCkpt{x, y, (uint32_t) iword | ((uint32_t) ibit << 8) | ((uint32_t) icode << 16), 0u};
                    int64_t periods = 0, dummy = 0;
                    nco_advance<NCO_CARRIER>(x, wx, run, dummy);
                    nco_advance<NCO_CODE>(y, wy, run, periods);
                    nav_advance(iword, ibit, icode, periods);
                }
                stc.phase = x;
            }
            call.chain[c] = stc;
        }
    });
    call.st.host_chain_ms = now_ms() - t0;
    rc = upload_nav(ctx, s);
    if (rc) return rc;
    const size_t cnt = (size_t) nblk * nchan;
    CU(cudaEventRecord(ctx->ev[kEvCallStart], s));
    CU(cudaMemcpyAsync(ctx->d_bc, ctx->h_bc, cnt * sizeof(BlockChanDev), cudaMemcpyHostToDevice, s));
    CU(cudaMemcpyAsync(ctx->d_ck, ctx->h_ck, cnt * nruns * sizeof(RunCkpt), cudaMemcpyHostToDevice, s));
    const SynthArgs a = call_args(ctx, call, 0, nblk);
    CU(launch_tables(a, s));
    CU(launch_synth(a, s));
    CU(cudaEventRecord(ctx->ev[kEvCallEnd], s));
    call.st.launches = 2;
    call.st.h2d_bytes = (int64_t) (cnt * (sizeof(BlockChanDev) + nruns * sizeof(RunCkpt)));
    if (call.host()) {
        rc = download(ctx, call, 0, nblk, s);
        if (rc) return rc;
        CU(cudaStreamSynchronize(s));
    }
    ctx->have_last = false;
    export_chain(call.chain, nchan, nullptr, carr_phase_out);
    if (stats) *stats = call.st;
    return GPSB200_OK;
}

int run_pipeline(gpsb200_ctx *ctx, Call &call, double *carr_phase_out, gpsb200_stats_t *stats) {
    ctx->trace_t0 = now_ms();
    trace(ctx, "call");
    if (call.nblk <= kHostChainBlocks && !ctx->fault_inject_chain) return small_call(ctx, call, carr_phase_out, stats);
    cudaStream_t sp = ctx->s_pre;
    int rc = call_open(ctx, call);
    if (rc) return rc;
    const auto &segs = call.segs;
    const int nseg = (int) segs.size();
    if (!call.host()) {
        std::vector<ChainState> guess = call.chain;
        for (int i = 0; i < nseg; i++) {
            cudaStream_t sw = (i & 1) ? ctx->s_ck : sp;
            rc = seg_params(ctx, call, segs[i].first, segs[i].second, sw, &guess, nullptr);
            if (rc) return rc;
            rc = seg_probe(ctx, call, segs[i].first, segs[i].second, sw);
            if (rc) return rc;
            CU(cudaEventRecord(ctx->ev_seg[i], sw));
        }
        trace(ctx, "speculative work enqueued");
        for (int i = 0; i < nseg; i++) {
            rc = seg_scan(ctx, call, i, ctx->ev_seg[i], nullptr);
            if (rc) return rc;
        }
        CU(cudaStreamSynchronize(ctx->s_ck));
        trace(ctx, "host scan done");
        rc = seg_commit(ctx, call, 0, nseg, sp);
        if (rc) return rc;
        trace(ctx, "checkpoints + synthesis enqueued");
    } else {
        for (int i = 0; i < nseg; i++) {
            rc = seg_params(ctx, call, segs[i].first, segs[i].second, sp, nullptr, nullptr);
            if (rc) return rc;
            rc = seg_probe(ctx, call, segs[i].first, segs[i].second, sp);
            if (rc) return rc;
            rc = seg_scan(ctx, call, i, nullptr, sp);
            if (rc) return rc;
            rc = seg_commit(ctx, call, i, i + 1, sp);
            if (rc) return rc;
        }
    }
    rc = call_close(ctx, call, sp);
    if (rc) return rc;
    export_chain(call.chain, call.nchan, nullptr, carr_phase_out);
    CU(cudaStreamSynchronize(sp));
    trace(ctx, "pre-phase stream drained (self-check read)");
    rc = call_verdict(ctx, call);
    if (rc) return rc;
    if (call.host()) {
        CU(cudaStreamSynchronize(call.stream));
        CU(cudaStreamSynchronize(ctx->s_copy));
    }
    if (stats) {
        float ms = 0;
        cudaEventElapsedTime(&ms, ctx->ev[kEvProbeStart], ctx->ev[kEvProbeEnd]);
        call.st.probe_kernel_ms = ms;
        cudaEventElapsedTime(&ms, ctx->ev[kEvCkptStart], ctx->ev[kEvCkptEnd]);
        call.st.checkpoint_kernel_ms = ms;
        if (call.host()) {
            cudaEventElapsedTime(&ms, ctx->ev[kEvCallStart], ctx->ev[kEvCallEnd]);
            call.st.kernel_ms = ms;
        }
        *stats = call.st;
    }
    return GPSB200_OK;
}

int slice_prepare(gpsb200_ctx *ctx, const gpsb200_chan_t *chans, int nblk, int nchan, int sample_size, void *dst_device,
                  void *dst_host, cudaStream_t s, gpsb200_slice_link_t *link) {
    int rc = check_call(ctx, chans, nblk, nchan, sample_size, dst_device ? dst_device : dst_host);
    if (rc) return rc;
    rc = check_aligned(ctx, dst_device, "gpsb200_slice_prepare", "dst_device");
    if (rc) return rc;
    if (!dst_device) {
        rc = ensure_staging(ctx, sample_size);
        if (rc) return rc;
        dst_device = ctx->d_out;
    }
    if (!link) return fail(ctx, GPSB200_ERR_ARG, "gpsb200_slice_prepare: link is NULL");
    Call &call = ctx->call = Call(chans, nblk, nchan, sample_size, dst_device, dst_host, nullptr, s);
    call.active = true;
    rc = call_open(ctx, call);
    if (rc) return rc;
    memset(link, 0, sizeof *link);
    rc = seg_params(ctx, call, 0, nblk, ctx->s_pre, nullptr, link);
    if (rc) return rc;
    call.chans = nullptr;
    ctx->have_last = false;
    return GPSB200_OK;
}

int slice_probe(gpsb200_ctx *ctx, const int32_t *prn_in, const double *phase_guess_in, int eager) {
    Call &call = ctx->call;
    if (!call.active || call.probed) return fail(ctx, GPSB200_ERR_ARG, "gpsb200_slice_probe: call gpsb200_slice_prepare first");
    CU(cudaSetDevice(ctx->cfg.device));
    const double t0 = now_ms();
    finalize_guesses(ctx, 0, call.nblk, call.nchan, prn_in, phase_guess_in);
    call.st.host_chain_ms += now_ms() - t0;
    call.eager = eager != 0;
    const int n = call.eager ? (int) call.segs.size() : 1;
    int rc = seg_probe(ctx, call, 0, call.segs[n - 1].second, ctx->s_pre);
    if (rc) return rc;
    for (int i = 0; i < n; i++) CU(cudaEventRecord(ctx->ev_seg[i], ctx->s_pre));
    call.probed = true;
    return GPSB200_OK;
}

int slice_finish(gpsb200_ctx *ctx, const int32_t *prn_in, const double *phase_in, int32_t *prn_out, double *phase_out,
                 gpsb200_stats_t *stats, gpsb200_handoff_fn handoff, void *user) {
    Call &call = ctx->call;
    if (!call.active || !call.probed)
        return fail(ctx, GPSB200_ERR_ARG, "gpsb200_slice_finish: call gpsb200_slice_prepare and gpsb200_slice_probe first");
    CU(cudaSetDevice(ctx->cfg.device));
    const int nchan = call.nchan, nseg = (int) call.segs.size();
    cudaStream_t sk = ctx->s_ck;
    seed_chain(call.chain, nchan, prn_in, phase_in);
    std::vector<int32_t> po(nchan, 0);
    std::vector<double> xo(nchan, 0.0);
    ctx->trace_t0 = now_ms();
    trace(ctx, "slice_finish");
    int rc;
    if (call.eager) {
        for (int i = 0; i < nseg; i++) {
            rc = seg_scan(ctx, call, i, ctx->ev_seg[i], sk);
            if (rc) return rc;
        }
        trace(ctx, "host scan done");
        export_chain(call.chain, nchan, po.data(), xo.data());
        if (handoff) handoff(user, po.data(), xo.data());
        trace(ctx, "handed over");
    }
    for (int i = 0; i < nseg; i++) {
        if (!call.eager) {
            rc = seg_scan(ctx, call, i, ctx->ev_seg[i], sk);
            if (rc) return rc;
        }
        rc = seg_commit(ctx, call, i, i + 1, sk);
        if (rc) return rc;
        if (!call.eager && i + 1 < nseg) {
            const int b0 = call.segs[i + 1].first, b1 = call.segs[i + 1].second;
            reanchor_guesses(ctx, b0, b1, nchan, call.chain);
            rc = seg_probe(ctx, call, b0, b1, ctx->s_pre);
            if (rc) return rc;
            CU(cudaEventRecord(ctx->ev_seg[i + 1], ctx->s_pre));
        }
    }
    if (!call.eager) {
        export_chain(call.chain, nchan, po.data(), xo.data());
        if (handoff) handoff(user, po.data(), xo.data());
    }
    rc = call_close(ctx, call, sk);
    if (rc) return rc;
    trace(ctx, "checkpoints + synthesis enqueued");
    call.active = false;
    call.finished = true;
    for (int c = 0; c < nchan; c++) {
        if (prn_out) prn_out[c] = po[c];
        if (phase_out) phase_out[c] = xo[c];
    }
    if (stats) *stats = call.st;
    return GPSB200_OK;
}

int synth_host(gpsb200_ctx *ctx, const gpsb200_chan_t *chans, int nblk, int nchan, int sample_size, void *dst_host,
               void *const *scatter, double *carr_phase_out, gpsb200_stats_t *stats) {
    for (int b = 0; scatter && b < nblk; b++)
        if (!scatter[b]) return fail(ctx, GPSB200_ERR_ARG, "gpsb200_synth_blocks_scatter: NULL block destination");
    int rc = check_call(ctx, chans, nblk, nchan, sample_size, scatter ? scatter[0] : dst_host);
    if (rc) return rc;
    rc = ensure_staging(ctx, sample_size);
    if (rc) return rc;
// ... 247 lines not shown
    const double delt = 1.0 / (double) GPSB200_SAMPLERATE;
    std::vector<CarrierProbe> probes(nblk);
    std::vector<double> cc(nblk);
    std::vector<SpanBlockState> spec(nblk);
    uint64_t acc = phase_to_fix(start_guess);
    const double guess0 = fix_to_phase(acc);
    for (int j = 0; j < nblk; j++) {
        cc[j] = f_carr[j] * delt;
        carrier_probe(fix_to_phase(acc), cc[j], GPSB200_BLOCK_SAMPLES, probes[j]);
        acc = guess_block(acc, cc[j]);
    }
    CarrierProbe sum{}, part{};
    bool ok[2];
    for (int V = 0; V < 2; V++) {
        span_chain(probes.data(), OneSatellite{cc.data()}, nblk, 1, guess0, V, part, ok[V], spec.data());
        if (V == 0) {
            sum.x_w = part.x_w;
            sum.n_w = part.n_w;
        }
        sum.x_end[V] = part.x_end[V];
        sum.m_pos[V] = ok[V] ? part.m_pos[V] : 0.0;
        sum.m_neg[V] = ok[V] ? part.m_neg[V] : 0.0;
    }
    double xe, d;
    int v;
    if (!carrier_fixup(start_true, cc[0], sum, xe, &v, &d, 1.0)) return 0;
    starts_out[0] = start_true;
    for (int j = 1; j < nblk; j++) starts_out[j] = spec[j].start[v] + d;
    starts_out[nblk] = xe;
    return 1;
}

int gpsb200_checkpoint_segments_host(double start_true, double start_guess, double f_carr, int run_samples,
                                     double *starts_out, int *nseg_out) {
    if (!starts_out || run_samples <= 0 || GPSB200_BLOCK_SAMPLES % run_samples != 0) return GPSB200_ERR_ARG;
    const double c = f_carr * (1.0 / (double) GPSB200_SAMPLERATE);
    const int nruns = GPSB200_BLOCK_SAMPLES / run_samples, nseg = ckpt_segments(nruns);
    CarrierProbe p;
    double seg[kSegStates];
    carrier_probe_walk2(start_guess, c, GPSB200_BLOCK_SAMPLES, p, seg, nruns, run_samples);
    if (nseg_out) *nseg_out = nseg;
    starts_out[0] = start_true;
    for (int j = 1; j < kCkptSegs; j++) starts_out[j] = NAN;
    double xe, d;
    int v;
    if (!carrier_fixup(start_true, c, p, xe, &v, &d)) return 0;
    for (int j = first_derived_segment(p, nseg, nruns, run_samples); j < nseg; j++)
        starts_out[j] = seg[v * (kCkptSegs - 1) + j - 1] + d;
    return 1;
}

int gpsb200_carrier_probe_host(double guess, double f_carr, int64_t nsamples, int run_samples, int mode, void *probe_out,
                               double *seg_out) {
    if (!probe_out || nsamples < 0 || nsamples >= ((int64_t) 1 << 31) || (mode != 0 && mode != 1) || run_samples < 0 ||
        (run_samples > 0 && nsamples % run_samples != 0))
        return GPSB200_ERR_ARG;
    const double c = f_carr * (1.0 / (double) GPSB200_SAMPLERATE);
    const int nruns = run_samples > 0 ? (int) (nsamples / run_samples) : 0;
    double *seg = run_samples > 0 ? seg_out : nullptr;
    if (seg)
        for (int k = 0; k < kSegStates; k++) seg[k] = NAN;
    CarrierProbe p{};
    if (mode == 0) {
        for (int v = 0; v < 2; v++)
            carrier_probe_walk(guess, c, nsamples, v, p.n_w, p.x_w, p.x_end[v], p.m_pos[v], p.m_neg[v],
                               seg ? seg + v * (kCkptSegs - 1) : nullptr, nruns, run_samples);
    } else {
        carrier_probe_walk2(guess, c, nsamples, p, seg, nruns, run_samples);
    }
    memcpy(probe_out, &p, sizeof p);
    return GPSB200_OK;
}

int gpsb200_carrier_chain(const gpsb200_chan_t *chans, int nblk, int nchan, const double *phase_in,
                          double *phase_out, int threads) {
    if (!chans || !phase_out || nblk < 0 || nchan < 1) return GPSB200_ERR_ARG;
    const double delt = 1.0 / (double) GPSB200_SAMPLERATE;
    auto work = [&](int lo, int hi) {
        for (int c = lo; c < hi; c++) {
            int prn = 0;
            double ph = phase_in ? phase_in[c] : 0.0;
            for (int b = 0; b < nblk; b++) {
                const gpsb200_chan_t &in = chans[(size_t) b * nchan + c];
                if (in.prn <= 0) {
                    prn = 0;
                    continue;
                }
                if ((b == 0 && !phase_in) || in.prn != prn) {
                    if (!(b == 0 && phase_in)) ph = in.carr_phase;
                    prn = in.prn;
                }
                int64_t dummy = 0;
                nco_advance<NCO_CARRIER>(ph, in.f_carr * delt, GPSB200_BLOCK_SAMPLES, dummy);
            }
            phase_out[c] = prn > 0 ? ph : 0.0;
        }
    };
    threads = std::max(1, std::min(threads, nchan));
    std::vector<std::thread> th;
    const int per = (nchan + threads - 1) / threads;
    for (int t = 0; t < threads; t++) {
        const int lo = t * per, hi = std::min(nchan, lo + per);
        if (lo < hi) th.emplace_back(work, lo, hi);
    }
    for (auto &t : th) t.join();
    return GPSB200_OK;
}

int gpsb200_create(const gpsb200_config_t *cfg, gpsb200_ctx_t **out) {
    if (!cfg || !out) return GPSB200_ERR_ARG;
    gpsb200_ctx *ctx = new gpsb200_ctx();
    ctx->cfg = *cfg;
    gpsb200_config_t &c = ctx->cfg;
    if (c.run_samples == 0) c.run_samples = 2400;
    if (c.host_threads <= 0) c.host_threads = (int) std::max(1u, std::min(16u, std::thread::hardware_concurrency()));
    if (c.max_nav_frames <= 0) c.max_nav_frames = 1;
    if (c.max_chan < 1 || c.max_chan > GPSB200_MAX_CHAN || c.max_blocks < 1 || c.run_samples < 32 ||
        c.run_samples % 32 != 0 || GPSB200_BLOCK_SAMPLES % c.run_samples != 0) {
        delete ctx;
        return GPSB200_ERR_ARG;
    }
    ctx->nruns = GPSB200_BLOCK_SAMPLES / c.run_samples;
    ctx->pool.reset(new WorkerPool(std::min(c.host_threads, c.max_chan)));
    *out = ctx;
    int ndev = 0;
    if (cudaGetDeviceCount(&ndev) != cudaSuccess || ndev == 0)
        return fail(ctx, GPSB200_ERR_CUDA, "no CUDA device: gpsb200 has no CPU fallback");
    CU(cudaSetDevice(c.device));
    CU(cudaStreamCreateWithFlags(&ctx->s_compute, cudaStreamNonBlocking));
    CU(cudaStreamCreateWithFlags(&ctx->s_copy, cudaStreamNonBlocking));
    {
        int lo = 0, hi = 0;
        CU(cudaDeviceGetStreamPriorityRange(&lo, &hi));
        CU(cudaStreamCreateWithPriority(&ctx->s_pre, cudaStreamNonBlocking, hi));
        CU(cudaStreamCreateWithPriority(&ctx->s_ck, cudaStreamNonBlocking, hi));
    }
    for (auto &e : ctx->ev) CU(cudaEventCreate(&e));
    const int nchunk = (c.max_blocks + kSynthChunk - 1) / kSynthChunk + (c.max_blocks + kSegBlocks - 1) / kSegBlocks + 5;
    ctx->ev_done.resize(nchunk);
    for (auto &e : ctx->ev_done) CU(cudaEventCreateWithFlags(&e, cudaEventDisableTiming));
    const size_t max_segs = segments_of(c.max_blocks).size();
    ctx->ev_seg.resize(max_segs);
    for (auto &e : ctx->ev_seg) CU(cudaEventCreateWithFlags(&e, cudaEventDisableTiming));
    CU(cudaHostAlloc(&ctx->h_seg_end, max_segs * c.max_chan * sizeof(double), cudaHostAllocMapped));
    CU(cudaHostGetDevicePointer((void **) &ctx->d_seg_end, ctx->h_seg_end, 0));
    ctx->seg_expect.assign(max_segs * c.max_chan, -1.0);
    const size_t nbc = (size_t) c.max_blocks * c.max_chan;
    CU(cudaMalloc(&ctx->d_bc, nbc * sizeof(BlockChanDev)));
    CU(cudaHostAlloc(&ctx->h_bc, nbc * sizeof(BlockChanDev), cudaHostAllocDefault));
    CU(cudaMalloc(&ctx->d_ck, nbc * ctx->nruns * sizeof(RunCkpt)));
    CU(cudaHostAlloc(&ctx->h_ck, (size_t) std::min(c.max_blocks, kHostChainBlocks) * c.max_chan * ctx->nruns * sizeof(RunCkpt),
                     cudaHostAllocDefault));
    CU(cudaMalloc(&ctx->d_carr_end, nbc * sizeof(double)));
    CU(cudaMalloc(&ctx->d_atab, (size_t) c.max_blocks * kAtabRows * 32 * sizeof(int32_t)));
    CU(cudaMalloc(&ctx->d_chain_errors, sizeof(int)));
    CU(cudaHostAlloc(&ctx->h_chain_errors, sizeof(int), cudaHostAllocDefault));
    CU(cudaMalloc(&ctx->d_guess, nbc * sizeof(double)));
    CU(cudaHostAlloc(&ctx->h_guess, nbc * sizeof(double), cudaHostAllocDefault));
    ctx->h_guess_abs.assign(nbc, 1);
    ctx->h_span_flags.assign((size_t) ((c.max_blocks + kSpanBlocks - 1) / kSpanBlocks + 1) * c.max_chan, 0);
    CU(cudaMalloc(&ctx->d_carr0, nbc * sizeof(double)));
    CU(cudaHostAlloc(&ctx->h_carr0, nbc * sizeof(double), cudaHostAllocDefault));
    CU(cudaMalloc(&ctx->d_probe, nbc * sizeof(CarrierProbe)));
    CU(cudaHostAlloc(&ctx->h_probe, nbc * sizeof(CarrierProbe), cudaHostAllocMapped));
    CU(cudaHostGetDevicePointer((void **) &ctx->d_probe_host, ctx->h_probe, 0));
    CU(cudaMalloc(&ctx->d_seg, nbc * kSegStates * sizeof(double)));
    ctx->max_spans = (c.max_blocks + kSpanBlocks - 1) / kSpanBlocks + 1;
    const size_t nsc = (size_t) ctx->max_spans * c.max_chan;
    CU(cudaHostAlloc(&ctx->h_span_sum, nsc * sizeof(CarrierProbe), cudaHostAllocMapped));
    CU(cudaHostGetDevicePointer((void **) &ctx->d_span_sum, ctx->h_span_sum, 0));
    CU(cudaMalloc(&ctx->d_spec, nbc * sizeof(SpanBlockState)));
    if (const char *ev = getenv("GPSB200_TRACE")) ctx->trace_on = atoi(ev) != 0;
    if (const char *ev = getenv("GPSB200_LANES")) ctx->lanes_on = atoi(ev) != 0;
    CU(cudaMalloc(&ctx->d_span_res, nsc * sizeof(SpanRes)));
    CU(cudaHostAlloc(&ctx->h_span_res, nsc * sizeof(SpanRes), cudaHostAllocDefault));
    const size_t navb = (size_t) c.max_nav_frames * c.max_chan * GPSB200_NAV_WORDS * 4;
    CU(cudaMalloc(&ctx->d_nav, navb));
    CU(cudaHostAlloc(&ctx->h_nav, navb, cudaHostAllocDefault));
    memset(ctx->h_nav, 0, navb);
    std::vector<uint32_t> chips((size_t) 33 * kChipWords, 0);
    for (int prn = 1; prn <= 32; prn++) {
        uint8_t ca[GPSB200_CA_LEN];
        ca_code(prn, ca);
        for (int n = 0; n < kChipWords * 32; n++)
            if (ca[n % GPSB200_CA_LEN]) chips[(size_t) prn * kChipWords + (n >> 5)] |= 1u << (n & 31);
    }
    CU(cudaMalloc(&ctx->d_chips, chips.size() * 4));
    CU(cudaMemcpy(ctx->d_chips, chips.data(), chips.size() * 4, cudaMemcpyHostToDevice));
    return GPSB200_OK;
}

void gpsb200_destroy(gpsb200_ctx_t *ctx) {
    if (!ctx) return;
    if (ctx->s_compute) cudaSetDevice(ctx->cfg.device);
    if (ctx->s_compute) cudaStreamSynchronize(ctx->s_compute);
    if (ctx->s_copy) cudaStreamSynchronize(ctx->s_copy);
    if (ctx->s_pre) cudaStreamSynchronize(ctx->s_pre);
    if (ctx->s_ck) cudaStreamSynchronize(ctx->s_ck);
    cudaFree(ctx->d_bc);
    cudaFreeHost(ctx->h_bc);
    cudaFree(ctx->d_ck);
    cudaFreeHost(ctx->h_ck);
    cudaFree(ctx->d_carr_end);
    cudaFree(ctx->d_atab);
    cudaFree(ctx->d_chain_errors);
    cudaFreeHost(ctx->h_chain_errors);
    cudaFree(ctx->d_guess);
    cudaFreeHost(ctx->h_guess);
    cudaFree(ctx->d_carr0);
    cudaFreeHost(ctx->h_carr0);
    cudaFreeHost(ctx->h_probe);
    cudaFree(ctx->d_probe);
    cudaFree(ctx->d_seg);
    cudaFreeHost(ctx->h_span_sum);
    cudaFree(ctx->d_spec);
    cudaFree(ctx->d_span_res);
    cudaFreeHost(ctx->h_span_res);
    cudaFree(ctx->d_nav);
    cudaFreeHost(ctx->h_nav);
    cudaFree(ctx->d_chips);
    cudaFree(ctx->d_out);
    cudaFree(ctx->d_rx);
    cudaFree(ctx->d_rx_chips);
    for (auto &e : ctx->ev)
        if (e) cudaEventDestroy(e);
    for (auto &e : ctx->ev_done)
        if (e) cudaEventDestroy(e);
    for (auto &e : ctx->ev_seg)
        if (e) cudaEventDestroy(e);
    cudaFreeHost(ctx->h_seg_end);
    acq::scratch_free(ctx->acq);
    trk::scratch_free(ctx->trk);
    snap::scratch_free(ctx->snap);
    cd::scratch_free(ctx->cd);
    pvt::scratch_free(ctx->pvt);
    if (ctx->s_compute) cudaStreamDestroy(ctx->s_compute);
    if (ctx->s_copy) cudaStreamDestroy(ctx->s_copy);
    if (ctx->s_pre) cudaStreamDestroy(ctx->s_pre);
    if (ctx->s_ck) cudaStreamDestroy(ctx->s_ck);
    delete ctx;
}

int gpsb200_set_nav(gpsb200_ctx_t *ctx, int frame, int chan, const uint32_t dwrd[GPSB200_NAV_WORDS]) {
    if (!ctx || !dwrd) return GPSB200_ERR_ARG;
    if (frame < 0 || frame >= ctx->cfg.max_nav_frames || chan < 0 || chan >= ctx->cfg.max_chan)
        return fail(ctx, GPSB200_ERR_ARG, "gpsb200_set_nav: frame/channel out of range");
    memcpy(ctx->h_nav + ((size_t) frame * ctx->cfg.max_chan + chan) * GPSB200_NAV_WORDS, dwrd, GPSB200_NAV_WORDS * 4);
    ctx->nav_dirty = true;
    return GPSB200_OK;
}

int gpsb200_synth_blocks_device(gpsb200_ctx_t *ctx, const gpsb200_chan_t *chans, int nblk, int nchan,
                                int sample_size, void *dst_device, void *stream_, double *carr_phase_out,
                                gpsb200_stats_t *stats) {
    if (!ctx) return GPSB200_ERR_ARG;
    cudaStream_t s = caller_stream(ctx, stream_);
    int rc = check_call(ctx, chans, nblk, nchan, sample_size, dst_device);
    if (!rc) rc = check_aligned(ctx, dst_device, "gpsb200_synth_blocks_device", "dst_device");
    if (!rc) {
        Call call(chans, nblk, nchan, sample_size, dst_device, nullptr, nullptr, s);
        rc = run_pipeline(ctx, call, carr_phase_out, stats);
    }
    return settle(ctx, s, rc);
}

int gpsb200_slice_prepare(gpsb200_ctx_t *ctx, const gpsb200_chan_t *chans, int nblk, int nchan, int sample_size,
                          void *dst_device, void *dst_host, void *stream_, gpsb200_slice_link_t *link) {
    if (!ctx) return GPSB200_ERR_ARG;
    cudaStream_t s = caller_stream(ctx, stream_);
    return settle(ctx, s, slice_prepare(ctx, chans, nblk, nchan, sample_size, dst_device, dst_host, s, link));
}

int gpsb200_slice_probe(gpsb200_ctx_t *ctx, const int32_t *prn_in, const double *phase_guess_in, int eager) {
    if (!ctx) return GPSB200_ERR_ARG;
    cudaStream_t s = ctx->call.active ? ctx->call.stream : nullptr;
    return settle(ctx, s, slice_probe(ctx, prn_in, phase_guess_in, eager));
}

int gpsb200_slice_finish_cb(gpsb200_ctx_t *ctx, const int32_t *prn_in, const double *phase_in, int32_t *prn_out,
                            double *phase_out, gpsb200_stats_t *stats, gpsb200_handoff_fn handoff, void *user) {
    if (!ctx) return GPSB200_ERR_ARG;
    cudaStream_t s = ctx->call.active ? ctx->call.stream : nullptr;
    return settle(ctx, s, slice_finish(ctx, prn_in, phase_in, prn_out, phase_out, stats, handoff, user));
}

int gpsb200_slice_finish(gpsb200_ctx_t *ctx, const int32_t *prn_in, const double *phase_in, int32_t *prn_out,
                         double *phase_out, gpsb200_stats_t *stats) {
    return gpsb200_slice_finish_cb(ctx, prn_in, phase_in, prn_out, phase_out, stats, nullptr, nullptr);
}

int gpsb200_slice_wait(gpsb200_ctx_t *ctx) {
    if (!ctx || !ctx->s_compute) return GPSB200_ERR_ARG;
    CU(cudaSetDevice(ctx->cfg.device));
    CU(cudaStreamSynchronize(ctx->s_pre));
    CU(cudaStreamSynchronize(ctx->s_ck));
    if (ctx->call.stream) CU(cudaStreamSynchronize(ctx->call.stream));
    CU(cudaStreamSynchronize(ctx->s_copy));
    if (ctx->call.finished) {
        ctx->call.finished = false;
        return call_verdict(ctx, ctx->call);
    }
    return GPSB200_OK;
}

int gpsb200_slice_link_host(const gpsb200_chan_t *chans, int nblk, int nchan, gpsb200_slice_link_t *link) {
    if (!chans || !link || nblk < 1 || nchan < 1 || nchan > GPSB200_MAX_CHAN) return GPSB200_ERR_ARG;
    const double delt = 1.0 / (double) GPSB200_SAMPLERATE;
    memset(link, 0, sizeof *link);
    for (int c = 0; c < nchan; c++) {
        uint64_t acc = 0;
        int prev = chans[c].prn;
        bool absolute = false;
        link->prn_first[c] = prev;
        link->first_phase[c] = prev > 0 ? chans[c].carr_phase : 0.0;
        for (int b = 0; b < nblk; b++) {
            const gpsb200_chan_t &in = chans[(size_t) b * nchan + c];
            if (in.prn <= 0) {
                prev = 0;
                absolute = true;
                continue;
            }
            if (in.prn != prev) {
                acc = phase_to_fix(in.carr_phase);
                absolute = true;
            }
            prev = in.prn;
            acc = guess_block(acc, in.f_carr * delt);
        }
        link->prn_last[c] = prev > 0 ? prev : 0;
        link->reset_inside[c] = absolute ? 1 : 0;
        link->value[c] = fix_to_phase(acc);
    }
    return GPSB200_OK;
}

int gpsb200_link_apply(const gpsb200_slice_link_t *link, int nchan, const int32_t *prn_in, const double *phase_in,
                       int32_t *prn_out, double *phase_out) {
    if (!link || !prn_out || !phase_out || nchan < 1 || nchan > GPSB200_MAX_CHAN) return GPSB200_ERR_ARG;
    for (int c = 0; c < nchan; c++) {
        if (link->prn_last[c] <= 0) {
            prn_out[c] = 0;
            phase_out[c] = 0.0;
            continue;
        }
        double ph = link->value[c];
        if (!link->reset_inside[c]) {
            const bool cont = prn_in && phase_in && prn_in[c] > 0 && prn_in[c] == link->prn_first[c];
            ph += cont ? phase_in[c] : link->first_phase[c];
            if (ph >= 1.0) ph -= 1.0;
        }
        prn_out[c] = link->prn_last[c];
        phase_out[c] = (ph >= 0.0 && ph < 1.0) ? ph : 0.0;
    }
    return GPSB200_OK;
}

const char *gpsb200_synth_kernel_name(const gpsb200_ctx_t *ctx, int nchan) {
    if (!ctx) return "";
    SynthArgs a{};
    a.nchan = nchan;
    a.run_samples = ctx->cfg.run_samples;
    a.lanes = ctx->lanes_on && !ctx->lanes_veto ? 1 : 0;
    return synth_lanes_applicable(a) ? "k_synth_lanes" : "k_synth";
}

int gpsb200_debug_corrupt_chain(gpsb200_ctx_t *ctx, int on) {
    if (!ctx || on < 0 || on > 2) return GPSB200_ERR_ARG;
    ctx->fault_inject_chain = on;
    return GPSB200_OK;
}

int gpsb200_debug_run_checkpoints(gpsb200_ctx_t *ctx, int nblk, int nchan, void *out) {
    if (!ctx || !out || nblk < 1 || nblk > ctx->cfg.max_blocks || nchan < 1 || nchan > ctx->cfg.max_chan)
        return GPSB200_ERR_ARG;
    if (!ctx->s_compute) return fail(ctx, GPSB200_ERR_CUDA, "context has no CUDA device");
    CU(cudaSetDevice(ctx->cfg.device));
    CU(cudaDeviceSynchronize());
    CU(cudaMemcpy(out, ctx->d_ck, (size_t) nblk * ctx->nruns * nchan * sizeof(RunCkpt), cudaMemcpyDeviceToHost));
    return GPSB200_OK;
}

int gpsb200_debug_block_probes(gpsb200_ctx_t *ctx, int nblk, int nchan, void *probes_out, double *seg_out,
                               double *guess_out) {
    if (!ctx || !probes_out || nblk < 1 || nblk > ctx->cfg.max_blocks || nchan < 1 || nchan > ctx->cfg.max_chan)
        return GPSB200_ERR_ARG;
    if (!ctx->s_compute) return fail(ctx, GPSB200_ERR_CUDA, "context has no CUDA device");
    CU(cudaSetDevice(ctx->cfg.device));
    CU(cudaDeviceSynchronize());
    const size_t cnt = (size_t) nblk * nchan;
    CU(cudaMemcpy(probes_out, ctx->d_probe, cnt * sizeof(CarrierProbe), cudaMemcpyDeviceToHost));
    if (seg_out) CU(cudaMemcpy(seg_out, ctx->d_seg, cnt * kSegStates * sizeof(double), cudaMemcpyDeviceToHost));
    if (guess_out) CU(cudaMemcpy(guess_out, ctx->d_guess, cnt * sizeof(double), cudaMemcpyDeviceToHost));
    return GPSB200_OK;
}

int gpsb200_debug_synth_shape(gpsb200_ctx_t *ctx, int nblk, int nchan, int sample_size, const char **kernel,
                              int *ctas_per_block, int *runs_per_cta) {
    if (!ctx || !kernel || !ctas_per_block || !runs_per_cta || nblk < 1 || nchan < 1 || nchan > ctx->cfg.max_chan ||
        (sample_size != GPSB200_SC08 && sample_size != GPSB200_SC16))
        return GPSB200_ERR_ARG;
    if (!ctx->s_compute) return fail(ctx, GPSB200_ERR_CUDA, "context has no CUDA device");
    CU(cudaSetDevice(ctx->cfg.device));
    const SynthArgs a = make_args(ctx, 0, nblk, nchan, sample_size, nullptr);
    int ctas = 0, threads = 0;
    size_t smem = 0;
    synth_launch_shape(a, &ctas, &threads, &smem, ctas_per_block, runs_per_cta);
    *kernel = synth_lanes_applicable(a) ? "k_synth_lanes" : "k_synth";
    return GPSB200_OK;
}

int gpsb200_carrier_chain_device(gpsb200_ctx_t *ctx, const gpsb200_chan_t *chans, int nblk, int nchan,
                                 const double *phase_in, double *phase_out) {
    if (!ctx || !chans || !phase_out || nblk < 0 || nchan < 1 || nchan > ctx->cfg.max_chan) return GPSB200_ERR_ARG;
    return settle(ctx, nullptr, carrier_chain_device(ctx, chans, nblk, nchan, phase_in, phase_out));
}

int gpsb200_replay_device(gpsb200_ctx_t *ctx, void *dst_device, void *stream_, int kernel_mask) {
    if (!ctx || !ctx->have_last) return GPSB200_ERR_ARG;
    const int rc = check_aligned(ctx, dst_device, "gpsb200_replay_device", "dst_device");
    if (rc) return rc;
    CU(cudaSetDevice(ctx->cfg.device));
    cudaStream_t s = caller_stream(ctx, stream_);
    SynthArgs a = ctx->last;
    if (dst_device) a.out = dst_device;
    if (kernel_mask & 8) CU(launch_tables(a, s));
    if (kernel_mask & 4) {
        CU(launch_probe(a, s));
        CU(launch_chain(a, s));
    }
    if (kernel_mask & 1) CU(launch_checkpoints(a, s));
    if (kernel_mask & 2) CU(launch_synth(a, s));
    return GPSB200_OK;
}

int gpsb200_synth_blocks_scatter(gpsb200_ctx_t *ctx, const gpsb200_chan_t *chans, int nblk, int nchan, int sample_size,
                                 void *const *dst_blocks, double *carr_phase_out, gpsb200_stats_t *stats) {
    if (!ctx || !dst_blocks) return GPSB200_ERR_ARG;
    return settle(ctx, nullptr, synth_host(ctx, chans, nblk, nchan, sample_size, nullptr, dst_blocks, carr_phase_out, stats));
}

int gpsb200_synth_blocks(gpsb200_ctx_t *ctx, const gpsb200_chan_t *chans, int nblk, int nchan, int sample_size,
                         void *dst, double *carr_phase_out, gpsb200_stats_t *stats) {
    if (!ctx) return GPSB200_ERR_ARG;
    return settle(ctx, nullptr, synth_host(ctx, chans, nblk, nchan, sample_size, dst, nullptr, carr_phase_out, stats));
}

int gpsb200_acquire(gpsb200_ctx_t *ctx, const void *iq, int64_t nsamples, int sample_size, const gpsb200_acq_config_t *cfg,
                    gpsb200_acq_result_t *res, uint64_t *grid) {
    if (!ctx) return GPSB200_ERR_ARG;
    return settle(ctx, nullptr, acquire(ctx, iq, nsamples, sample_size, cfg, false, nullptr, res, grid, false,
                                        ctx->s_compute));
}

int gpsb200_acquire_device(gpsb200_ctx_t *ctx, const void *iq_device, int64_t nsamples, int sample_size,
                           const gpsb200_acq_config_t *cfg, gpsb200_acq_result_t *res, uint64_t *grid, void *stream_) {
    if (!ctx) return GPSB200_ERR_ARG;
    cudaStream_t s = caller_stream(ctx, stream_);
    return settle(ctx, s, acquire(ctx, iq_device, nsamples, sample_size, cfg, false, nullptr, res, grid, true, s));
}

int gpsb200_acquire_windows(gpsb200_ctx_t *ctx, const void *iq, int64_t nsamples, int sample_size,
                            const gpsb200_acq_config_t *cfg, const double *f_lo_prn, gpsb200_acq_result_t *res,
                            uint64_t *grid) {
    if (!ctx) return GPSB200_ERR_ARG;
    return settle(ctx, nullptr, acquire(ctx, iq, nsamples, sample_size, cfg, true, f_lo_prn, res, grid, false,
                                        ctx->s_compute));
}

int gpsb200_acquire_windows_device(gpsb200_ctx_t *ctx, const void *iq_device, int64_t nsamples, int sample_size,
                                   const gpsb200_acq_config_t *cfg, const double *f_lo_prn, gpsb200_acq_result_t *res,
                                   uint64_t *grid, void *stream_) {
    if (!ctx) return GPSB200_ERR_ARG;
    cudaStream_t s = caller_stream(ctx, stream_);
    return settle(ctx, s, acquire(ctx, iq_device, nsamples, sample_size, cfg, true, f_lo_prn, res, grid, true, s));
}

int gpsb200_debug_acq_split(gpsb200_ctx_t *ctx, int force, int nprn, int nbins) {
    if (!ctx || !(force == -1 || force == 0 || acq::split_allowed(force)) || nprn < 1 || nprn > 32 || nbins < 1 ||
        nbins > GPSB200_ACQ_MAX_BINS)
        return GPSB200_ERR_ARG;
    if (force >= 0) ctx->acq.force_split = force;
    if (!ctx->acq.sms) {
        if (!ctx->s_compute) return fail(ctx, GPSB200_ERR_CUDA, "context has no CUDA device");
        CU(cudaDeviceGetAttribute(&ctx->acq.sms, cudaDevAttrMultiProcessorCount, ctx->cfg.device));
    }
    return acq::split_of(ctx->acq, nprn, nbins);
}

int gpsb200_track_start(int prn, double doppler_hz, int64_t sample, gpsb200_track_state_t *st) {
    if (!st || prn < 1 || prn > 32 || !(std::fabs(doppler_hz) <= 10000.0) || sample < 0) return GPSB200_ERR_ARG;
    memset(st, 0, sizeof *st);
    st->prn = prn;
    st->sample = sample;
    trk::start_steps(doppler_hz, st->carr_step, st->code_step);
    st->carr_freq = (int64_t) st->carr_step * 1024;
    return GPSB200_OK;
}

int gpsb200_track(gpsb200_ctx_t *ctx, const void *iq, int64_t nsamples, int sample_size, int64_t base,
                  gpsb200_track_state_t *state, int nchan, int max_epochs, gpsb200_track_epoch_t *epochs,
                  int32_t *nepochs) {
    if (!ctx) return GPSB200_ERR_ARG;
    return settle(ctx, nullptr, track(ctx, iq, nsamples, sample_size, base, state, nchan, max_epochs, epochs, nepochs,
                                      false, ctx->s_compute));
}

int gpsb200_track_device(gpsb200_ctx_t *ctx, const void *iq_device, int64_t nsamples, int sample_size, int64_t base,
                         gpsb200_track_state_t *state, int nchan, int max_epochs, gpsb200_track_epoch_t *epochs,
                         int32_t *nepochs, void *stream_) {
    if (!ctx) return GPSB200_ERR_ARG;
    cudaStream_t s = caller_stream(ctx, stream_);
    return settle(ctx, s, track(ctx, iq_device, nsamples, sample_size, base, state, nchan, max_epochs, epochs, nepochs,
                                true, s));
}

int gpsb200_pvt(gpsb200_ctx_t *ctx, const gpsb200_pvt_chan_t *chans, int nchan, const gpsb200_track_epoch_t *epochs,
                const int32_t *nepochs, int max_epochs, const gpsb200_pvt_config_t *cfg, gpsb200_fix_t *fixes,
                double *residuals) {
    if (!ctx) return GPSB200_ERR_ARG;
    return settle(ctx, nullptr, pvt_fix(ctx, "gpsb200_pvt", chans, nchan, epochs, nepochs, max_epochs, cfg, fixes,
                                        residuals, pvt::Stage()));
}

int gpsb200_pvt_raim(gpsb200_ctx_t *ctx, const gpsb200_pvt_chan_t *chans, int nchan, const gpsb200_track_epoch_t *epochs,
                     const int32_t *nepochs, int max_epochs, const gpsb200_pvt_config_t *cfg,
                     const gpsb200_raim_config_t *raim, gpsb200_fix_t *fixes, double *residuals, gpsb200_raim_t *out) {
    if (!ctx) return GPSB200_ERR_ARG;
    if (!raim || !out) return settle(ctx, nullptr, fail(ctx, GPSB200_ERR_ARG, "gpsb200_pvt_raim: NULL raim or out"));
    pvt::Stage st;
    st.raim = raim;
    st.raim_out = out;
    return settle(ctx, nullptr, pvt_fix(ctx, "gpsb200_pvt_raim", chans, nchan, epochs, nepochs, max_epochs, cfg, fixes,
                                        residuals, st));
}

int gpsb200_pvt_araim(gpsb200_ctx_t *ctx, const gpsb200_pvt_chan_t *chans, int nchan, const gpsb200_track_epoch_t *epochs,
                      const int32_t *nepochs, int max_epochs, const gpsb200_pvt_config_t *cfg,
                      const gpsb200_araim_config_t *araim, gpsb200_fix_t *fixes, double *residuals,
                      gpsb200_araim_t *out) {
    if (!ctx) return GPSB200_ERR_ARG;
    if (!araim || !out) return settle(ctx, nullptr, fail(ctx, GPSB200_ERR_ARG, "gpsb200_pvt_araim: NULL araim or out"));
    pvt::Stage st;
    st.araim = araim;
    st.araim_out = out;
    return settle(ctx, nullptr, pvt_fix(ctx, "gpsb200_pvt_araim", chans, nchan, epochs, nepochs, max_epochs, cfg, fixes,
                                        residuals, st));
}

int gpsb200_pvt_coarse(gpsb200_ctx_t *ctx, const gpsb200_pvt_chan_t *chans, int nchan,
                       const gpsb200_track_epoch_t *epochs, const int32_t *nepochs, int max_epochs,
                       const gpsb200_pvt_config_t *cfg, const gpsb200_coarse_config_t *apriori, gpsb200_fix_t *fixes,
                       double *residuals, gpsb200_coarse_t *out, int64_t *ms) {
    if (!ctx) return GPSB200_ERR_ARG;
    if (!apriori || !out)
        return settle(ctx, nullptr, fail(ctx, GPSB200_ERR_ARG, "gpsb200_pvt_coarse: NULL apriori or out"));
    pvt::Stage st;
    st.coarse = apriori;
    st.coarse_out = out;
    st.ms = ms;
    return settle(ctx, nullptr, pvt_fix(ctx, "gpsb200_pvt_coarse", chans, nchan, epochs, nepochs, max_epochs, cfg, fixes,
                                        residuals, st));
}

int gpsb200_pvt_search(gpsb200_ctx_t *ctx, const gpsb200_pvt_chan_t *chans, int nchan,
                       const gpsb200_track_epoch_t *epochs, const int32_t *nepochs, int max_epochs,
                       const gpsb200_pvt_config_t *cfg, const gpsb200_search_config_t *search, gpsb200_fix_t *fixes,
                       double *residuals, gpsb200_search_t *out, int64_t *ms, double *node_rms) {
    if (!ctx) return GPSB200_ERR_ARG;
    if (!search || !out)
        return settle(ctx, nullptr, fail(ctx, GPSB200_ERR_ARG, "gpsb200_pvt_search: NULL search or out"));
    pvt::Stage st;
    st.search = search;
    st.search_out = out;
    st.ms = ms;
    st.node_rms = node_rms;
    return settle(ctx, nullptr, pvt_fix(ctx, "gpsb200_pvt_search", chans, nchan, epochs, nepochs, max_epochs, cfg, fixes,
                                        residuals, st));
// ... 113 lines not shown
```

### multi-sdr-gps-sim_b200/csrc/rx_samples.cuh

```cuda
#pragma once
#include <stdint.h>

#include "synth_tables.h"
#include "track.h"

namespace gpsb200 {
namespace rx {

namespace {

__constant__ uint8_t c_qsine[128] = {GPSB200_QUARTER_SINE};

__device__ __forceinline__ int sine512(int k) {
    k &= 511;
    const int r = k & 255;
    const int v = c_qsine[r < 128 ? r : 255 - r];
    return k < 256 ? v : -v;
}

template <typename T>
__device__ __forceinline__ void load_iq(const T *iq, int64_t i, int &I, int &Q);
template <>
__device__ __forceinline__ void load_iq<int8_t>(const int8_t *iq, int64_t i, int &I, int &Q) {
    const char2 v = reinterpret_cast<const char2 *>(iq)[i];
    I = v.x;
    Q = v.y;
}
template <>
__device__ __forceinline__ void load_iq<int16_t>(const int16_t *iq, int64_t i, int &I, int &Q) {
    const short2 v = reinterpret_cast<const short2 *>(iq)[i];
    I = min(max(v.x >> 4, -128), 127);
    Q = min(max(v.y >> 4, -128), 127);
}

__device__ __forceinline__ void fill_carrier_table(int2 *tab, int nthreads) {
    for (int i = threadIdx.x; i < 512; i += nthreads) tab[i] = make_int2(sine512(i + 128), sine512(i));
}

__device__ __forceinline__ int2 wipe_off(const int2 *tab, uint32_t ph, int I, int Q) {
    const int2 cs = tab[ph >> 23];
    return make_int2(I * cs.x + Q * cs.y, Q * cs.x - I * cs.y);
}

__device__ __forceinline__ void epl_chips(const int8_t *ca, uint64_t p, int &ce, int &cp, int &cl) {
    uint64_t e = p + trk::kHalf;
    if (e >= trk::kM) e -= trk::kM;
    const uint64_t l = p >= trk::kHalf ? p - trk::kHalf : p + trk::kM - trk::kHalf;
    ce = ca[e >> 32];
    cp = ca[p >> 32];
    cl = ca[l >> 32];
}

template <int N>
__device__ __forceinline__ void warp_partials(int (&a)[N], int32_t *part) {
#pragma unroll
    for (int j = 0; j < N; j++)
#pragma unroll
        for (int o = 16; o > 0; o >>= 1) a[j] += __shfl_xor_sync(0xffffffffu, a[j], o);
    if ((threadIdx.x & 31) == 0)
#pragma unroll
        for (int j = 0; j < N; j++) part[j] = a[j];
}

template <int kWarps>
__device__ __forceinline__ int warps_sum(const int32_t (*part)[6], int j) {
    int v = 0;
#pragma unroll
    for (int q = 0; q < kWarps; q++) v += part[q][j];
    return v;
}

}

}
}
```

### multi-sdr-gps-sim_b200/csrc/synth_kernels.cu

```cuda
#include <cuda_runtime.h>
#include <stdint.h>

#include <type_traits>

#include "nco_exact.h"
#include "rx_samples.cuh"
#include "synth_kernels.h"
#include "synth_tables.h"

namespace gpsb200 {

using rx::sine512;

static int group_for(int nchan) { return nchan > 16 ? 32 : (nchan > 8 ? 16 : 8); }

__global__ void __launch_bounds__(256) k_tables(SynthArgs a, int group) {
    const long idx = (long) blockIdx.x * blockDim.x + threadIdx.x;
    const long per_blk = 256L * 32;
    const int b = (int) (idx / per_blk);
    if (b >= a.nblk) return;
    const int rem = (int) (idx - (long) b * per_blk), k = rem >> 5, col = rem & 31, c = col % group;
    const BlockChanDev *bc = a.bc + (size_t) b * a.nchan;
    int32_t e = 0;
    if (c < a.nchan && bc[c].prn > 0) {
        const double gain = bc[c].gain;
        const int ai = __double2int_rz(__dmul_rn((double) sine512(k + 128), gain));
        const int aq = __double2int_rz(__dmul_rn((double) sine512(k), gain));
        e = ai + aq * 65536;
    }
    int32_t *t = a.atab + (size_t) b * kAtabRows * 32 + col;
    t[k * 32] = e;
    t[(k + 256) * 32] = -e;
    if (k == 255) t[512 * 32] = -e;
}

__device__ __forceinline__ bool map_block_chan(const SynthArgs &a, int idx, int &b, int &c) {
    const int nblk_pad = (a.nblk + 31) & ~31;
    c = idx / nblk_pad;
    b = idx - c * nblk_pad;
    return c < a.nchan && b < a.nblk;
}

__device__ __forceinline__ void code_walk(const SynthArgs &a, int b, int c) {
    const BlockChanDev p = a.bc[(size_t) b * a.nchan + c];
    RunCkpt *ck = a.ck + (size_t) b * a.nruns * a.nchan + c;
    const WalkConst w = walk_const(p.c_code);
    double y = p.code0;
    int iword = p.nav0 & 0xFF, ibit = (p.nav0 >> 8) & 0xFF, icode = (p.nav0 >> 16) & 0xFF;
    for (int r = 0; r < a.nruns; r++) {
        RunCkpt *o = ck + (size_t) r * a.nchan;
        o->y = y;
        o->nav = (uint32_t) iword | ((uint32_t) ibit << 8) | ((uint32_t) icode << 16);
        o->pad = 0;
        if (p.prn <= 0) continue;
        int64_t periods = 0;
        nco_advance<NCO_CODE>(y, w, a.run_samples, periods);
        nav_advance(iword, ibit, icode, periods);
    }
}

__global__ void __launch_bounds__(128) k_probe(SynthArgs a) {
    const int nblk_pad = (a.nblk + 31) & ~31;
    const int per_role = nblk_pad * a.nchan;
    int idx = blockIdx.x * blockDim.x + threadIdx.x;
    const int role = idx / per_role;
    idx -= role * per_role;
    int b, c;
    if (role > 1 || !map_block_chan(a, idx, b, c)) return;
    if (role == 1) {
        if (a.ck) code_walk(a, b, c);
        return;
    }
    const size_t i = (size_t) b * a.nchan + c;
    const BlockChanDev p = a.bc[i];
    CarrierProbe pr{0.0, {0.0, 0.0}, {0.0, 0.0}, {0.0, 0.0}, -1, 0};
    if (p.prn > 0)
        carrier_probe_walk2(a.guess[i], p.c_carr, kBlockSamples, pr, a.seg + i * kSegStates, a.nruns, a.run_samples);
    a.probe[i] = pr;
    if (a.probe_host) a.probe_host[i] = pr;
}

struct ColumnParams {
    const BlockChanDev *col;
    int nchan;
    __device__ __forceinline__ void operator()(int j, double &cc, int32_t &prn) const {
        const BlockChanDev &p = col[(size_t) j * nchan];
        cc = p.c_carr;
        prn = p.prn;
    }
};

__global__ void __launch_bounds__(64) k_chain(SynthArgs a) {
    int idx = blockIdx.x * blockDim.x + threadIdx.x;
    const int per_v = a.nspan * a.nchan;
    const int V = idx / per_v;
    idx -= V * per_v;
    if (V > 1) return;
    const int sp = idx / a.nchan, c = idx - sp * a.nchan;
    const int b0 = sp * a.span_blocks, nb = min(a.span_blocks, a.nblk - b0);
    const size_t i0 = (size_t) b0 * a.nchan + c;
    CarrierProbe sum;
    bool ok;
    const ColumnParams col{a.bc + i0, a.nchan};
    span_chain(a.probe + i0, col, nb, (size_t) a.nchan, a.guess[i0], V, sum, ok, a.spec + i0);
    CarrierProbe *dst = a.span_sum + (size_t) sp * a.nchan + c;
    if (V == 0) {
        dst->x_w = sum.x_w;
        dst->n_w = sum.n_w;
        dst->pad = 0;
    }
    dst->x_end[V] = sum.x_end[V];
    dst->m_pos[V] = ok ? sum.m_pos[V] : 0.0;
    dst->m_neg[V] = ok ? sum.m_neg[V] : 0.0;
}

__device__ __forceinline__ double resolved_start(const SynthArgs &a, int b, int c) {
    const int sp = b / a.span_blocks;
    const SpanRes r = a.span_res[(size_t) sp * a.nchan + c];
    if (r.mode == 1) return a.carr0[(size_t) b * a.nchan + c];
    if (r.mode == 2) return 0.0;
    if (b == sp * a.span_blocks) return r.start;
    return a.spec[(size_t) b * a.nchan + c].start[r.variant] + r.shift;
}

__global__ void __launch_bounds__(128) k_checkpoints(SynthArgs a) {
    const int nblk_pad = (a.nblk + 31) & ~31;
    const int per_j = nblk_pad * a.nchan;
    const int nseg = ckpt_segments(a.nruns);
    int idx = blockIdx.x * blockDim.x + threadIdx.x;
    const int j = idx / per_j;
    idx -= j * per_j;
    int b, c;
    if (j >= nseg || !map_block_chan(a, idx, b, c)) return;
    const size_t i = (size_t) b * a.nchan + c;
    const BlockChanDev p = a.bc[i];
    RunCkpt *ck = a.ck + (size_t) b * a.nruns * a.nchan + c;
    if (p.prn <= 0) {
        for (int r = seg_first_run(j, nseg, a.nruns); r < seg_first_run(j + 1, nseg, a.nruns); r++)
            ck[(size_t) r * a.nchan].x = 0.0;
        if (j == nseg - 1) {
            if (a.carr_end) a.carr_end[i] = 0.0;
            if (a.last_end_host && b == a.nblk - 1) a.last_end_host[c] = 0.0;
        }
        return;
    }
    const double s = resolved_start(a, b, c);
    const CarrierProbe &pr = a.probe[i];
    int v = 0;
    double d = 0.0, xe;
    const int jd = carrier_fixup(s, p.c_carr, pr, xe, &v, &d) ? first_derived_segment(pr, nseg, a.nruns, a.run_samples)
                                                               : nseg;
    if (j > 0 && j < jd) return;
    const double *seg = a.seg + i * kSegStates + v * (kCkptSegs - 1);
    const int jn = j == 0 ? jd : j + 1;
    double x = j == 0 ? s : seg[j - 1] + d;
    const WalkConst w = walk_const(p.c_carr);
    for (int r = seg_first_run(j, nseg, a.nruns); r < seg_first_run(jn, nseg, a.nruns); r++) {
        ck[(size_t) r * a.nchan].x = x;
        int64_t dummy = 0;
        nco_advance<NCO_CARRIER>(x, w, a.run_samples, dummy);
    }
    bool bad;
    if (jn < nseg) {
        bad = f64_bits(seg[jn - 1] + d) != f64_bits(x);
    } else {
        bad = b + 1 < a.nblk && a.bc[i + a.nchan].prn == p.prn && f64_bits(resolved_start(a, b + 1, c)) != f64_bits(x);
        if (a.carr_end) a.carr_end[i] = x;
        if (a.last_end_host && b == a.nblk - 1) a.last_end_host[c] = x;
    }
    if (bad && a.chain_errors) atomicAdd(a.chain_errors, 1);
}

constexpr int kMaxWarps = 24;
constexpr int kChunkMax = 64;

template <int GROUP>
struct SynthSmem {
    int32_t atab[kAtabRows][32];
    uint32_t cabits[kChipWords][GROUP];
    uint32_t nav[kNavWords][GROUP];
    alignas(16) int32_t stage[kMaxWarps][kChunkMax * (32 / GROUP)];
    alignas(8) uint64_t bar;
// ... 104 lines not shown
        const size_t samp0 = (size_t) b * kBlockSamples + (size_t) r * a.run_samples + (size_t) s0 + ch * SPL;
        uint32_t w[SPL];
#pragma unroll
        for (int t = 0; t < SPL; t++) {
            const int p = stage[sub * kChunkMax + ch * SPL + t];
            const int iv = (int) (short) (p & 0xFFFF);
            const int qv = (p - iv) >> 16;
            if (IQ16) {
                w[t] = ((uint32_t) iv & 0xFFFFu) | ((uint32_t) qv << 16);
            } else {
                const uint32_t two = (((uint32_t) (iv >> 4)) & 0xFFu) | ((((uint32_t) (qv >> 4)) & 0xFFu) << 8);
                if (t & 1) w[t >> 1] |= two << 16;
                else w[t >> 1] = two;
            }
        }
        constexpr int NBYTES = SPL * (IQ16 ? 4 : 2);
        char *dst = reinterpret_cast<char *>(a.out) + samp0 * (IQ16 ? 4 : 2);
        if (NBYTES == 2) *reinterpret_cast<uint16_t *>(dst) = (uint16_t) w[0];
        else if (NBYTES == 4) *reinterpret_cast<uint32_t *>(dst) = w[0];
        else if (NBYTES == 8) *reinterpret_cast<uint2 *>(dst) = make_uint2(w[0], w[1]);
        else {
#pragma unroll
            for (int q = 0; q < NBYTES / 16; q++)
                reinterpret_cast<uint4 *>(dst)[q] = make_uint4(w[4 * q], w[4 * q + 1], w[4 * q + 2], w[4 * q + 3]);
        }
    };

    auto do_chunk = [&](const int len, int s0) {
        const int j0 = __double2loint(__dadd_rz(y, K52));
        const uint32_t lo = ccol[(j0 >> 5) * GROUP], hi = ccol[((j0 >> 5) + 1) * GROUP];
        uint32_t w8 = (__funnelshift_r(lo, hi, j0 & 31) ^ (dbit ? 0xFFFFFFFFu : 0u)) << 8;
        double KY = K52 - (double) j0;
        auto emit = [&](double xs, double ys) -> int {
            const int k = __double2loint(__dadd_rz(xs, K43));
            const int rel = __double2loint(__dadd_rz(ys, KY));
            const int kk = k ^ ((w8 >> rel) & 0x100);
            int e;
            asm volatile("ld.shared.b32 %0, [%1];" : "=r"(e) : "r"(abase + (uint32_t) kk * 128u));
            return group_sum<GROUP>(e);
        };
        auto park = [&](int i, int s0_, int s1_, int s2_, int s3_) {
            *reinterpret_cast<int4 *>(&stage[sub * kChunkMax + i]) = make_int4(s0_, s1_, s2_, s3_);
        };
        auto step_checked = [&](double &xs, double &ys) {
            xs = __dadd_rn(xs, cc);
            ys = __dadd_rn(ys, dd);
            if (xs >= 1.0) xs = __dadd_rn(xs, -1.0);
            else if (xs < 0.0) {
                xs = __dadd_rn(xs, 1.0);
                if (xs >= 1.0) xs = kBelowOne;
            }
            if (ys >= 1023.0) {
                ys = __dadd_rn(ys, -1023.0);
                KY = __dadd_rn(KY, 1023.0);
                if (++icode >= 20) {
                    icode = 0;
                    if (++ibit >= 30) {
                        ibit = 0;
                        ++iword;
                    }
                    const int nb = nav_bit(iword, ibit);
                    if (nb != dbit) w8 = ~w8;
                    dbit = nb;
                }
            }
        };
#pragma unroll(GROUP == 32 ? 2 : 1)
        for (int g8 = 0; g8 < len; g8 += 8) {
            const int hx = __double2hiint(x), hy = __double2hiint(y);
            const bool risky = (hx >= thr_x_hi) | (hx <= thr_x_lo) | (hy >= thr_y);
            if (!__any_sync(0xFFFFFFFFu, risky)) {
#pragma unroll
                for (int h = 0; h < 8; h += 4) {
                    int sv[4];
#pragma unroll
                    for (int i = 0; i < 4; i++) {
                        sv[i] = emit(x, y);
                        x = __dadd_rn(x, cc);
                        y = __dadd_rn(y, dd);
                    }
                    park(g8 + h, sv[0], sv[1], sv[2], sv[3]);
                }
            } else {
#pragma unroll
                for (int h = 0; h < 8; h += 4) {
                    int sv[4];
#pragma unroll
                    for (int i = 0; i < 4; i++) {
                        sv[i] = emit(x, y);
                        const double xn = __dadd_rn(x, cc), yn = __dadd_rn(y, dd);
                        const bool wrap = ((unsigned) __double2hiint(xn) >= 0x3FF00000u) |
                                          ((unsigned) __double2hiint(yn) >= 0x408FF800u);
                        if (__any_sync(0xFFFFFFFFu, wrap)) step_checked(x, y);
                        else {
                            x = xn;
                            y = yn;
                        }
                    }
                    park(g8 + h, sv[0], sv[1], sv[2], sv[3]);
                }
            }
        }
        __syncwarp();
        if (len == 64) flush(std::integral_constant<int, 64>(), s0);
        else flush(std::integral_constant<int, 32>(), s0);
        __syncwarp();
    };

    int s0 = 0;
#pragma unroll 1
    for (; s0 < a.run_samples; s0 += 64)
        do_chunk(a.run_samples - s0 >= 64 ? 64 : 32, s0);
}

template <int GROUP>
static cudaError_t launch_synth_t(const SynthArgs &a, cudaStream_t s) {
    const int rpw = 32 / GROUP;
    const int warps = (a.runs_per_cta + rpw - 1) / rpw;
    const size_t smem = sizeof(SynthSmem<GROUP>);
    const int ctas = a.nblk * a.ctas_per_block;
    cudaError_t e;
    if (a.iq16) {
        e = cudaFuncSetAttribute(k_synth<GROUP, true>, cudaFuncAttributeMaxDynamicSharedMemorySize, (int) smem);
        if (e != cudaSuccess) return e;
        k_synth<GROUP, true><<<ctas, warps * 32, smem, s>>>(a);
    } else {
        e = cudaFuncSetAttribute(k_synth<GROUP, false>, cudaFuncAttributeMaxDynamicSharedMemorySize, (int) smem);
        if (e != cudaSuccess) return e;
        k_synth<GROUP, false><<<ctas, warps * 32, smem, s>>>(a);
    }
    return cudaGetLastError();
}

cudaError_t launch_synth(const SynthArgs &a, cudaStream_t s) {
    if (synth_lanes_applicable(a)) return launch_synth_lanes(a, s);
    switch (group_for(a.nchan)) {
        case 32: return launch_synth_t<32>(a, s);
        case 16: return launch_synth_t<16>(a, s);
        default: return launch_synth_t<8>(a, s);
    }
}

void synth_launch_shape(const SynthArgs &a, int *ctas, int *threads, size_t *smem, int *ctas_per_block, int *runs_per_cta) {
    if (synth_lanes_applicable(a)) return synth_lanes_launch_shape(a, ctas, threads, smem, ctas_per_block, runs_per_cta);
    const int grp = group_for(a.nchan), rpw = 32 / grp;
    *ctas = a.nblk * a.ctas_per_block;
    *ctas_per_block = a.ctas_per_block;
    *runs_per_cta = a.runs_per_cta;
    *threads = ((a.runs_per_cta + rpw - 1) / rpw) * 32;
    *smem = grp == 32 ? sizeof(SynthSmem<32>) : (grp == 16 ? sizeof(SynthSmem<16>) : sizeof(SynthSmem<8>));
}

cudaError_t launch_tables(const SynthArgs &a, cudaStream_t s) {
    const long total = (long) a.nblk * 256 * 32;
    k_tables<<<(unsigned) ((total + 255) / 256), 256, 0, s>>>(a, group_for(a.nchan));
    return cudaGetLastError();
}

cudaError_t launch_checkpoints(const SynthArgs &a, cudaStream_t s) {
    const int nblk_pad = (a.nblk + 31) & ~31;
    const long total = (long) ckpt_segments(a.nruns) * nblk_pad * a.nchan;
    const int threads = 128;
    k_checkpoints<<<(unsigned) ((total + threads - 1) / threads), threads, 0, s>>>(a);
    return cudaGetLastError();
}

cudaError_t launch_probe(const SynthArgs &a, cudaStream_t s) {
    const int nblk_pad = (a.nblk + 31) & ~31;
    const long total = (a.ck ? 2L : 1L) * nblk_pad * a.nchan;
    const int threads = 128;
    k_probe<<<(unsigned) ((total + threads - 1) / threads), threads, 0, s>>>(a);
    return cudaGetLastError();
}

cudaError_t launch_chain(const SynthArgs &a, cudaStream_t s) {
    const long total = 2L * a.nspan * a.nchan;
    const int threads = 64;
    k_chain<<<(unsigned) ((total + threads - 1) / threads), threads, 0, s>>>(a);
    return cudaGetLastError();
}

}
```

### multi-sdr-gps-sim_b200/csrc/synth_kernels.h

```cpp
#pragma once
#include <cuda_runtime.h>
#include <stdint.h>

namespace gpsb200 {

constexpr int kBlockSamples = 300000;
constexpr int kNavWords = 60;
constexpr int kChipWords = 33;
constexpr int kAtabRows = 513;

struct BlockChanDev {
    double c_carr;
    double c_code;
    double gain;
    double carr_in;
    double code0;
    int32_t prn;
    uint32_t nav0;
    int32_t frame;
    int32_t pad[3];
};
static_assert(sizeof(BlockChanDev) == 64, "BlockChanDev layout");

struct RunCkpt {
    double x;
    double y;
    uint32_t nav;
    uint32_t pad;
};
static_assert(sizeof(RunCkpt) == 24, "RunCkpt layout");

struct CarrierProbe;
struct SpanBlockState;

struct SpanRes {
    double start;
    double shift;
    int32_t variant;
    int32_t mode;
};
static_assert(sizeof(SpanRes) == 24, "SpanRes layout");

struct SynthArgs {
    const BlockChanDev *bc;
    const double *carr0;
    const double *guess;
    CarrierProbe *probe;
    CarrierProbe *probe_host;
    double *seg;
    CarrierProbe *span_sum;
    SpanBlockState *spec;
    const SpanRes *span_res;
    int span_blocks, nspan;
    RunCkpt *ck;
    const uint32_t *nav;
    int nav_stride;
    const uint32_t *chipbits;
    int32_t *atab;
    double *carr_end;
    double *last_end_host;
    int *chain_errors;
    void *out;
    int nblk, nchan, nruns, run_samples, runs_per_cta, ctas_per_block, iq16;
    int lanes;
};

cudaError_t launch_tables(const SynthArgs &a, cudaStream_t s);
cudaError_t launch_probe(const SynthArgs &a, cudaStream_t s);
cudaError_t launch_chain(const SynthArgs &a, cudaStream_t s);
cudaError_t launch_checkpoints(const SynthArgs &a, cudaStream_t s);
cudaError_t launch_synth(const SynthArgs &a, cudaStream_t s);
bool synth_lanes_applicable(const SynthArgs &a);
cudaError_t launch_synth_lanes(const SynthArgs &a, cudaStream_t s);
void synth_lanes_launch_shape(const SynthArgs &a, int *ctas, int *threads, size_t *smem, int *ctas_per_block,
                              int *runs_per_cta);
void synth_launch_shape(const SynthArgs &a, int *ctas, int *threads, size_t *smem, int *ctas_per_block, int *runs_per_cta);

}
```

### multi-sdr-gps-sim_b200/csrc/synth_lanes.cu

```cuda
#include <cuda_runtime.h>
#include <stdint.h>

#include "nco_exact.h"
#include "synth_kernels.h"
#include "synth_lanes.h"

namespace gpsb200 {

namespace {

constexpr int kLaneWarps = 16;
constexpr int kLaneCtas = 2;
constexpr int kLaneChipWords = 36;

struct LaneWin {
    uint32_t s0, s1, s2;
    uint32_t base;
};

struct LaneSteps {
    uint64_t D96, E96;
    uint32_t inv32, e22;
};

template <int CH>
struct LanesSmem {
    static constexpr int kWins = 32 / CH;
    uint32_t chips[CH][kLaneChipWords];
    uint32_t nav[CH][kNavWords];
    alignas(16) LaneWin win[kLaneWarps][kWins][CH];
    alignas(16) uint32_t step[CH];
    LaneSteps steps[CH];
    alignas(16) uint32_t stage[kLaneWarps][kWins * lanes::kWindow];
    uint32_t band[CH][lanes::kBandList + 1];
};
template <int CH>
constexpr size_t lanes_smem_bytes() { return sizeof(LanesSmem<CH>) + (size_t) CH * 2048; }

template <int OFF>
__device__ __forceinline__ int table_at(uint32_t p, uint32_t ta) {
    int e;
    asm volatile("{\n\t.reg .b32 i, ad;\n\tshr.b32 i, %1, 23;\n\tmad.lo.u32 ad, i, 4, %2;\n\tld.shared.b32 %0, [ad+%3];\n\t}"
                 : "=r"(e)
                 : "r"(p), "r"(ta), "n"(OFF));
    return e;
}

template <class ChipFn, class NavFn>
__device__ __noinline__ uint3 exact_signs_call(lanes::Anchor an, int w, ChipFn chips, NavFn nav) {
    uint32_t W[3];
    lanes::exact_signs(an, w, chips, nav, W);
    return make_uint3(W[0], W[1], W[2]);
}

__device__ __noinline__ int exact_index_call(lanes::Anchor an, int w, int n) {
    const uint64_t D = lanes::carr_step_fix(an.c);
    const uint64_t P = lanes::carr_fix(an.x0) + (uint64_t) w * ((uint64_t) lanes::kWindow * D);
    return lanes::exact_index(P, D, an, w, n);
}

__device__ __forceinline__ void add_if(int &acc, uint32_t w, uint32_t bit, int e) {
    asm("{\n\t.reg .pred p;\n\t.reg .b32 t;\n\tand.b32 t, %1, %2;\n\tsetp.ne.u32 p, t, 0;\n\t@p add.s32 %0, %0, %3;\n\t}"
        : "+r"(acc)
        : "r"(w), "r"(bit), "r"(e));
}

template <int NC>
__device__ __forceinline__ void window_sums(const LaneWin *wp, const uint32_t *sp, uint32_t ta, int nchan, uint32_t n0,
                                            uint32_t sbit, int accs[3]) {
    const int nc = NC > 0 ? NC : nchan;
    const uint32_t n1 = n0 + 32u, n2 = n0 + 64u;
    int all0 = 0, all1 = 0, all2 = 0, neg0 = 0, neg1 = 0, neg2 = 0;
#pragma unroll 4
    for (int c = 0; c < nc; c += 2, wp += 2, sp += 2, ta += 2 * 2048u) {
        const uint4 wa = *reinterpret_cast<const uint4 *>(&wp[0]);
        const uint4 wb = *reinterpret_cast<const uint4 *>(&wp[1]);
        const uint2 st = *reinterpret_cast<const uint2 *>(sp);
        const uint32_t a0 = wa.w + n0 * st.x, a1 = wa.w + n1 * st.x, a2 = wa.w + n2 * st.x;
        const uint32_t b0 = wb.w + n0 * st.y, b1 = wb.w + n1 * st.y, b2 = wb.w + n2 * st.y;
        const int ea0 = table_at<0>(a0, ta), eb0 = table_at<2048>(b0, ta);
        const int ea1 = table_at<0>(a1, ta), eb1 = table_at<2048>(b1, ta);
        const int ea2 = table_at<0>(a2, ta), eb2 = table_at<2048>(b2, ta);
        all0 += ea0 + eb0;
        all1 += ea1 + eb1;
        all2 += ea2 + eb2;
        add_if(neg0, wa.x, sbit, ea0);
        add_if(neg0, wb.x, sbit, eb0);
        add_if(neg1, wa.y, sbit, ea1);
        add_if(neg1, wb.y, sbit, eb1);
        add_if(neg2, wa.z, sbit, ea2);
        add_if(neg2, wb.z, sbit, eb2);
    }
    accs[0] = (int) ((uint32_t) all0 - 2u * (uint32_t) neg0);
    accs[1] = (int) ((uint32_t) all1 - 2u * (uint32_t) neg1);
    accs[2] = (int) ((uint32_t) all2 - 2u * (uint32_t) neg2);
}

template <bool IQ16, int CH>
__global__ void __launch_bounds__(kLaneWarps * 32, kLaneCtas) k_synth_lanes(SynthArgs a) {
    constexpr int WINS = 32 / CH;
    constexpr int SWZ = 32 / CH;
    constexpr int BYTES = IQ16 ? 4 : 2;
    extern __shared__ __align__(16) unsigned char smem_raw[];
    int32_t *tab = reinterpret_cast<int32_t *>(smem_raw);
    LanesSmem<CH> &sm = *reinterpret_cast<LanesSmem<CH> *>(smem_raw + CH * 2048);
    const uint32_t tab_base = (uint32_t) __cvta_generic_to_shared(smem_raw);
    constexpr uint32_t kFull = 0xFFFFFFFFu;

    const int b = blockIdx.x / a.ctas_per_block;
    const int g = blockIdx.x - b * a.ctas_per_block;
    const int tid = threadIdx.x, nthr = blockDim.x;
    const int lane = tid & 31, warp = tid >> 5;
    const int nchan = a.nchan;
    const BlockChanDev *bc = a.bc + (size_t) b * nchan;

    {
        const int32_t *src = a.atab + (size_t) b * kAtabRows * 32;
        for (int i = tid; i < 512 * CH; i += nthr) {
            const int k = i / CH, c = i - k * CH;
            tab[c * 512 + ((k + c * SWZ) & 511)] = c < nchan ? src[k * 32 + c] : 0;
        }
        for (int i = tid; i < CH * kLaneChipWords; i += nthr) {
            const int c = i / kLaneChipWords, w = i - c * kLaneChipWords;
            uint32_t v = 0;
            if (c < nchan && bc[c].prn > 0) {
                const uint32_t *cw = a.chipbits + bc[c].prn * kChipWords;
                v = w < kChipWords ? cw[w] : __funnelshift_r(cw[w - 32], cw[w - 31], 1);
            }
            sm.chips[c][w] = v;
        }
        for (int i = tid; i < CH * kNavWords; i += nthr) {
            const int c = i / kNavWords, w = i - c * kNavWords;
            uint32_t v = 0;
            if (c < nchan && bc[c].prn > 0) v = a.nav[((size_t) bc[c].frame * a.nav_stride + c) * kNavWords + w];
            sm.nav[c][w] = v;
        }
        if (warp == kLaneWarps - 1 && lane < CH) {
            const bool ok = lane < nchan && bc[lane].prn > 0;
            lanes::ChanRun k;
            lanes::init_steps(k, ok, ok ? bc[lane].c_carr : 0.0, ok ? bc[lane].c_code : 0.0);
            sm.steps[lane] = LaneSteps{k.D96, k.E96, k.inv32, k.e22};
            sm.step[lane] = lanes::fast_step(k);
            lanes::band_residues(lanes::fast_step(k), &sm.band[lane][0]);
        }
    }
    __syncthreads();

    const int ch = lane & (CH - 1), half = lane / CH;
    const bool chan_ok = ch < nchan && bc[ch < nchan ? ch : 0].prn > 0;
    const uint32_t *nav_row = &sm.nav[ch][0];
    const uint32_t *chip_row = &sm.chips[ch][0];
    const uint32_t *band_row = &sm.band[ch][0];
    auto navf = [nav_row](int iw) { return nav_row[iw]; };
    auto chipf = [chip_row](int i) { return chip_row[i]; };
    const uint32_t n0 = (uint32_t) lane, n1 = n0 + 32u, n2 = n0 + 64u;
    const uint32_t sbit = 1u << lanes::sign_pos(lane);
    const int nwin = a.run_samples / lanes::kWindow;
    uint32_t *stage = &sm.stage[warp][0];

    const int run_first = g * a.runs_per_cta;
    const int run_last = min(run_first + a.runs_per_cta, a.nruns);
#pragma unroll 1
    for (int r = run_first + warp; r < run_last; r += kLaneWarps) {
        auto anchor = [&](int c) {
            const RunCkpt k0 = a.ck[((size_t) b * a.nruns + r) * nchan + c];
            return lanes::Anchor{k0.x, k0.y, bc[c].c_carr, bc[c].c_code, k0.nav};
        };
        lanes::ChanRun s;
        auto load_steps = [&]() {
            const LaneSteps k = sm.steps[ch];
            s.D96 = k.D96;
            s.E96 = k.E96;
            s.inv32 = k.inv32;
            s.e22 = k.e22;
        };
        {
            const lanes::Anchor an = chan_ok ? anchor(ch) : lanes::Anchor{0.0, 0.0, 0.0, 0.0, 0u};
            lanes::init_run(s, chan_ok, an.x0, an.y0, an.navpos, an.c, an.d, navf);
        }
        if (WINS == 2 && chan_ok && half == 1) {
            load_steps();
            lanes::advance_window(s, navf);
        }
        uint4 *dst = reinterpret_cast<uint4 *>(reinterpret_cast<char *>(a.out) +
                                               ((size_t) b * kBlockSamples + (size_t) r * a.run_samples) * BYTES);

#pragma unroll 1
        for (int w = 0; w < nwin; w += WINS) {
            uint32_t flagged;
            {
                uint32_t S[3] = {0u, 0u, 0u};
                uint32_t base = (uint32_t) (ch * SWZ) << 23;
                bool band = false;
                if (chan_ok) load_steps();
                if (chan_ok && w > 0) {
#pragma unroll
                    for (int i = 0; i < WINS; i++) lanes::advance_window(s, navf);
                }
                if (chan_ok && w + half < nwin) {
                    base += lanes::fast_base(s);
                    band = lanes::window_band_risky(band_row, base);
                    if (!lanes::window_signs(s, chipf, navf, S)) {
                        const uint3 e = exact_signs_call(anchor(ch), w + half, chipf, navf);
                        S[0] = e.x;
                        S[1] = e.y;
                        S[2] = e.z;
                    }
                }
                *reinterpret_cast<uint4 *>(&sm.win[warp][half][ch]) = make_uint4(S[0], S[1], S[2], base);
                flagged = __ballot_sync(kFull, band);
            }
            __syncwarp();

#pragma unroll
            for (int hh = 0; hh < WINS; hh++) {
                if (w + hh >= nwin) break;
                const LaneWin *wrow = &sm.win[warp][hh][0];
                int accs[3];
                if (CH == 32 && nchan == CH)
                    window_sums<CH>(wrow, &sm.step[0], tab_base, nchan, n0, sbit, accs);
                else
                    window_sums<0>(wrow, &sm.step[0], tab_base, nchan, n0, sbit, accs);
                for (uint32_t m = WINS == 1 ? flagged : (flagged >> (hh * CH)) & 0xFFFFu; m != 0u; m &= m - 1u) {
                    const int c = __ffs((int) m) - 1;
                    const uint4 wv = *reinterpret_cast<const uint4 *>(&wrow[c]);
                    const uint32_t st = sm.step[c];
                    const uint32_t p0 = wv.w + n0 * st, p1 = wv.w + n1 * st, p2 = wv.w + n2 * st;
                    const bool risky = lanes::fast_risky(p0) | lanes::fast_risky(p1) | lanes::fast_risky(p2);
                    if (!risky) continue;
                    const lanes::Anchor ac = anchor(c);
                    const uint32_t ps[3] = {p0, p1, p2}, sw[3] = {wv.x, wv.y, wv.z};
#pragma unroll
                    for (int j = 0; j < 3; j++) {
                        if (!lanes::fast_risky(ps[j])) continue;
                        const int kf = (int) (ps[j] >> 23);
                        const int k = exact_index_call(ac, w + hh, 32 * j + lane);
                        const int fix = tab[c * 512 + ((k + c * SWZ) & 511)] - tab[c * 512 + kf];
                        accs[j] += (sw[j] & sbit) ? -fix : fix;
                    }
                }
#pragma unroll
                for (int j = 0; j < 3; j++) {
                    const uint32_t p = (uint32_t) accs[j];
                    const uint32_t x = p + ((p & 0x8000u) << 1);
                    const int n = hh * lanes::kWindow + 32 * j + lane;
                    if (IQ16)
                        stage[n] = x;
                    else
                        reinterpret_cast<uint16_t *>(stage)[n] = (uint16_t) (((p >> 4) & 0xFFu) | ((x >> 12) & 0xFF00u));
                }
            }
            __syncwarp();
            {
                constexpr int kVec = WINS * lanes::kWindow * BYTES / 16;
                const int nvec = WINS == 1 || nwin - w >= WINS ? kVec : kVec / WINS;
                const uint4 *srcv = reinterpret_cast<const uint4 *>(stage);
#pragma unroll
                for (int i = lane; i < ((kVec + 31) & ~31); i += 32)
                    if (i < nvec) dst[i] = srcv[i];
                dst += kVec;
            }
        }
    }
}

}

bool synth_lanes_applicable(const SynthArgs &a) {
    return a.lanes && a.nchan <= 32 && a.run_samples % lanes::kWindow == 0 && a.run_samples <= lanes::kMaxRun;
}

static int device_sms() {
    int dev = 0, n = 0;
    if (cudaGetDevice(&dev) != cudaSuccess || cudaDeviceGetAttribute(&n, cudaDevAttrMultiProcessorCount, dev) != cudaSuccess)
        return 132;
    return n;
}

static void lanes_shape(const SynthArgs &a, int *ctas_per_block, int *runs_per_cta) {
    int per_block = (40 * kLaneCtas * device_sms() + a.nblk - 1) / a.nblk;
    if (per_block > 16) per_block = 16;
    if (per_block < 1) per_block = 1;
    int per_cta = (a.nruns + per_block - 1) / per_block;
    per_cta = (per_cta + kLaneWarps - 1) / kLaneWarps * kLaneWarps;
    per_block = (a.nruns + per_cta - 1) / per_cta;
    *ctas_per_block = per_block;
    *runs_per_cta = per_cta;
}

template <bool IQ16, int CH>
static cudaError_t launch_lanes_t(const SynthArgs &a, cudaStream_t s) {
    const size_t smem = lanes_smem_bytes<CH>();
    cudaError_t e = cudaFuncSetAttribute(k_synth_lanes<IQ16, CH>, cudaFuncAttributeMaxDynamicSharedMemorySize, (int) smem);
    if (e != cudaSuccess) return e;
    k_synth_lanes<IQ16, CH><<<a.nblk * a.ctas_per_block, kLaneWarps * 32, smem, s>>>(a);
    return cudaGetLastError();
}

cudaError_t launch_synth_lanes(const SynthArgs &a_in, cudaStream_t s) {
    SynthArgs a = a_in;
    lanes_shape(a, &a.ctas_per_block, &a.runs_per_cta);
    if (a.nchan <= 16) return a.iq16 ? launch_lanes_t<true, 16>(a, s) : launch_lanes_t<false, 16>(a, s);
    return a.iq16 ? launch_lanes_t<true, 32>(a, s) : launch_lanes_t<false, 32>(a, s);
}

void synth_lanes_launch_shape(const SynthArgs &a, int *ctas, int *threads, size_t *smem, int *ctas_per_block,
                              int *runs_per_cta) {
    int per_block, per_cta;
    lanes_shape(a, &per_block, &per_cta);
    *ctas = a.nblk * per_block;
    *threads = kLaneWarps * 32;
    *smem = a.nchan <= 16 ? lanes_smem_bytes<16>() : lanes_smem_bytes<32>();
    *ctas_per_block = per_block;
    *runs_per_cta = per_cta;
}

}
```

Measured before the change: 71480.

## Prebuild per-block lanes shared-memory image and load it with TMA bulk copies

Adds a k_lanes_images kernel, run once per block in place of the old table kernel. It writes a contiguous per-block image holding the swizzled carrier table, chip words, nav words, step parameters and band residues. The k_synth_lanes prologue then loads this image with four cp.async.bulk copies tracked by an mbarrier, instead of every CTA rebuilding its shared state with scattered global loads and init_steps math. Table launches for speculative segments are moved after all probes are enqueued, and a nav-upload event makes the checkpoint stream wait for the upload. The image buffer is larger, and a fallback regenerates the old tables when the lanes path no longer applies.

```diff
diff --git a/include/gpsb200.h b/include/gpsb200.h
--- a/include/gpsb200.h
+++ b/include/gpsb200.h
@@ -104,6 +104,10 @@
                        int32_t *prn_out, double *phase_out);
 
 int gpsb200_debug_corrupt_chain(gpsb200_ctx_t *ctx, int on);
+
+int gpsb200_debug_lanes(gpsb200_ctx_t *ctx, int prologue_only, int ctas_per_block);
+
+int gpsb200_debug_lanes_image(gpsb200_ctx_t *ctx, int blk, void *dev_out, void *host_out, int64_t *bytes);
 
 int gpsb200_debug_run_checkpoints(gpsb200_ctx_t *ctx, int nblk, int nchan, void *out);
 
diff --git a/multi-sdr-gps-sim_b200/api.py b/multi-sdr-gps-sim_b200/api.py
--- a/multi-sdr-gps-sim_b200/api.py
+++ b/multi-sdr-gps-sim_b200/api.py
@@ -397,7 +397,7 @@
            "gpsb200_nav_ephemeris", "gpsb200_nav_time_anchor", "gpsb200_pvt", "gpsb200_pvt_replay",
            "gpsb200_pvt_raim", "gpsb200_raim_thresholds", "gpsb200_pvt_araim", "gpsb200_araim_kfa", "gpsb200_pvt_coarse", "gpsb200_pvt_search", "gpsb200_search_nodes", "gpsb200_snapshot_measure", "gpsb200_snapshot_measure_device", "gpsb200_snapshot_batch", "gpsb200_snapshot_batch_device", "gpsb200_pvt_snapshot", "gpsb200_pvt_snapshot_search", "gpsb200_collective", "gpsb200_collective_device", "gpsb200_rinex_ephemeris", "gpsb200_bind_numa", "gpsb200_span_chain_host", "gpsb200_lanes_model_block",
            "gpsb200_lanes_window_band_host", "gpsb200_slice_prepare", "gpsb200_slice_probe",
-           "gpsb200_slice_finish", "gpsb200_slice_finish_cb", "gpsb200_slice_wait", "gpsb200_link_apply", "gpsb200_slice_link_host", "gpsb200_debug_corrupt_chain", "gpsb200_synth_kernel_name",
+           "gpsb200_slice_finish", "gpsb200_slice_finish_cb", "gpsb200_slice_wait", "gpsb200_link_apply", "gpsb200_slice_link_host", "gpsb200_debug_corrupt_chain", "gpsb200_debug_lanes", "gpsb200_debug_lanes_image", "gpsb200_synth_kernel_name",
            "gpsb200_debug_run_checkpoints", "gpsb200_checkpoint_segments_host",
            "gpsb200_carrier_probe_host", "gpsb200_debug_block_probes", "gpsb200_debug_synth_shape",
            "gpsb200_scenario_create", "gpsb200_scenario_destroy", "gpsb200_scenario_error",
@@ -471,6 +471,8 @@
         L.gpsb200_slice_finish.argtypes = [C.c_void_p, C.c_void_p, C.c_void_p, C.c_void_p, C.c_void_p, C.POINTER(Stats)]
         L.gpsb200_link_apply.argtypes = [C.POINTER(SliceLink), C.c_int, C.c_void_p, C.c_void_p, C.c_void_p, C.c_void_p]
         L.gpsb200_debug_corrupt_chain.argtypes = [C.c_void_p, C.c_int]
+        L.gpsb200_debug_lanes.argtypes = [C.c_void_p, C.c_int, C.c_int]
+        L.gpsb200_debug_lanes_image.argtypes = [C.c_void_p, C.c_int, C.c_void_p, C.c_void_p, C.POINTER(C.c_int64)]
         L.gpsb200_debug_run_checkpoints.argtypes = [C.c_void_p, C.c_int, C.c_int, C.c_void_p]
         L.gpsb200_checkpoint_segments_host.argtypes = [C.c_double, C.c_double, C.c_double, C.c_int, C.c_void_p,
                                                        C.POINTER(C.c_int)]
@@ -918,6 +920,16 @@
     def debug_corrupt_chain(self, on):
         self._check(lib().gpsb200_debug_corrupt_chain(self._h, int(on)))
 
+    def debug_lanes(self, prologue_only=False, ctas_per_block=0):
+        self._check(lib().gpsb200_debug_lanes(self._h, int(bool(prologue_only)), int(ctas_per_block)))
+
+    def debug_lanes_image(self, blk):
+        n = C.c_int64(0)
+        self._check(lib().gpsb200_debug_lanes_image(self._h, int(blk), None, None, C.byref(n)))
+        dev, host = np.zeros(n.value, np.uint8), np.ones(n.value, np.uint8)
+        self._check(lib().gpsb200_debug_lanes_image(self._h, int(blk), dev.ctypes.data, host.ctypes.data, C.byref(n)))
+        return dev, host
+
     def debug_run_checkpoints(self, nblk, nchan):
         nruns = BLOCK_SAMPLES // (self.cfg.run_samples or 2400)
         out = np.zeros((nblk, nruns, nchan), RUN_CKPT_DTYPE)
diff --git a/multi-sdr-gps-sim_b200/csrc/gpsb200_api.cu b/multi-sdr-gps-sim_b200/csrc/gpsb200_api.cu
--- a/multi-sdr-gps-sim_b200/csrc/gpsb200_api.cu
+++ b/multi-sdr-gps-sim_b200/csrc/gpsb200_api.cu
@@ -146,9 +146,10 @@
         slow.assign(segs.size(), 0);
     }
     bool host() const { return dst_host || scatter; }
+    bool lanes_images = false;
 };
 
-enum { kEvCallStart, kEvProbeStart, kEvProbeEnd, kEvCkptStart, kEvCkptEnd, kEvCallEnd, kCallEvents };
+enum { kEvCallStart, kEvProbeStart, kEvProbeEnd, kEvCkptStart, kEvCkptEnd, kEvCallEnd, kEvNavUp, kCallEvents };
 
 }
 
@@ -182,6 +183,8 @@
     std::vector<double> seg_expect;
     std::vector<cudaEvent_t> ev_seg;
     int fault_inject_chain = 0;
+    int lanes_prologue_only = 0;
+    int lanes_ctas = 0;
     bool trace_on = false;
     double trace_t0 = 0.0;
     Call call;
@@ -477,7 +480,7 @@
     a.nav = ctx->d_nav;
     a.nav_stride = ctx->cfg.max_chan;
     a.chipbits = ctx->d_chips;
-    a.atab = ctx->d_atab + (size_t) blk0 * kAtabRows * 32;
+    a.atab = nullptr;
     a.carr_end = ctx->d_carr_end + off;
     a.chain_errors = ctx->d_chain_errors;
     a.out = out;
@@ -487,6 +490,9 @@
     a.run_samples = ctx->cfg.run_samples;
     a.iq16 = sample_size == GPSB200_SC16;
     a.lanes = ctx->lanes_on && !ctx->lanes_veto ? 1 : 0;
+    a.lanes_prologue_only = ctx->lanes_prologue_only;
+    a.lanes_ctas = ctx->lanes_ctas;
+    a.atab = ctx->d_atab + (size_t) blk0 * synth_table_words(a);
     const int grp = nchan > 16 ? 32 : (nchan > 8 ? 16 : 8);
     const int rpw = 32 / grp;
     int per_cta = 24 * rpw;
@@ -572,12 +578,23 @@
     CU(cudaStreamWaitEvent(ctx->s_ck, ctx->ev[kEvCallStart], 0));
     const int rc = upload_nav(ctx, ctx->s_pre);
     if (rc) return rc;
+    CU(cudaEventRecord(ctx->ev[kEvNavUp], ctx->s_pre));
+    CU(cudaStreamWaitEvent(ctx->s_ck, ctx->ev[kEvNavUp], 0));
     CU(cudaMemsetAsync(ctx->d_chain_errors, 0, sizeof(int), ctx->s_pre));
     return GPSB200_OK;
 }
 
+int seg_tables(gpsb200_ctx *ctx, Call &call, int b0, int b1, cudaStream_t sp) {
+    if (!call.dst) return GPSB200_OK;
+    const SynthArgs a = call_args(ctx, call, b0, b1 - b0);
+    CU(launch_tables(a, sp));
+    call.st.launches += 1;
+    if (synth_lanes_applicable(a)) call.lanes_images = true;
+    return GPSB200_OK;
+}
+
 int seg_params(gpsb200_ctx *ctx, Call &call, int b0, int b1, cudaStream_t sp, std::vector<ChainState> *guessed,
-               gpsb200_slice_link_t *link) {
+               gpsb200_slice_link_t *link, bool tables = true) {
     const size_t off = (size_t) b0 * call.nchan, cnt = (size_t) (b1 - b0) * call.nchan;
     const double t0 = now_ms();
     const int rc = prepare_blocks(ctx, call.chans, b0, b1, call.nchan, guessed ? *guessed : call.chain, link, guessed);
@@ -585,11 +602,7 @@
     call.st.host_chain_ms += now_ms() - t0;
     CU(cudaMemcpyAsync(ctx->d_bc + off, ctx->h_bc + off, cnt * sizeof(BlockChanDev), cudaMemcpyHostToDevice, sp));
     call.st.h2d_bytes += (int64_t) (cnt * sizeof(BlockChanDev));
-    if (call.dst) {
-        CU(launch_tables(call_args(ctx, call, b0, b1 - b0), sp));
-        call.st.launches += 1;
-    }
-    return GPSB200_OK;
+    return tables ? seg_tables(ctx, call, b0, b1, sp) : GPSB200_OK;
 }
 
 int seg_probe(gpsb200_ctx *ctx, Call &call, int b0, int b1, cudaStream_t sp) {
@@ -656,6 +669,10 @@
         h[kCkptSegs - 1 + jm - 1] += 0x1p-51;
         CU(cudaMemcpyAsync(p, h, sizeof h, cudaMemcpyHostToDevice, sp));
         CU(cudaStreamSynchronize(sp));
+    }
+    if (call.lanes_images && !synth_lanes_applicable(a)) {
+        CU(launch_tables(a, sp));
+        call.st.launches += 1;
     }
     SynthArgs ack = a;
     ack.last_end_host = ctx->d_seg_end + (size_t) i0 * nchan;
@@ -795,11 +812,15 @@
         std::vector<ChainState> guess = call.chain;
         for (int i = 0; i < nseg; i++) {
             cudaStream_t sw = (i & 1) ? ctx->s_ck : sp;
-            rc = seg_params(ctx, call, segs[i].first, segs[i].second, sw, &guess, nullptr);
+            rc = seg_params(ctx, call, segs[i].first, segs[i].second, sw, &guess, nullptr, false);
             if (rc) return rc;
             rc = seg_probe(ctx, call, segs[i].first, segs[i].second, sw);
             if (rc) return rc;
             CU(cudaEventRecord(ctx->ev_seg[i], sw));
+        }
+        for (int i = 0; i < nseg; i++) {
+            rc = seg_tables(ctx, call, segs[i].first, segs[i].second, (i & 1) ? ctx->s_ck : sp);
+            if (rc) return rc;
         }
         trace(ctx, "speculative work enqueued");
         for (int i = 0; i < nseg; i++) {
@@ -1353,7 +1374,7 @@
     CU(cudaHostAlloc(&ctx->h_ck, (size_t) std::min(c.max_blocks, kHostChainBlocks) * c.max_chan * ctx->nruns * sizeof(RunCkpt),
                      cudaHostAllocDefault));
     CU(cudaMalloc(&ctx->d_carr_end, nbc * sizeof(double)));
-    CU(cudaMalloc(&ctx->d_atab, (size_t) c.max_blocks * kAtabRows * 32 * sizeof(int32_t)));
+    CU(cudaMalloc(&ctx->d_atab, (size_t) c.max_blocks * synth_table_words_max(c.max_chan) * sizeof(int32_t)));
     CU(cudaMalloc(&ctx->d_chain_errors, sizeof(int)));
     CU(cudaHostAlloc(&ctx->h_chain_errors, sizeof(int), cudaHostAllocDefault));
     CU(cudaMalloc(&ctx->d_guess, nbc * sizeof(double)));
@@ -1571,6 +1592,28 @@
     return GPSB200_OK;
 }
 
+int gpsb200_debug_lanes(gpsb200_ctx_t *ctx, int prologue_only, int ctas_per_block) {
+    if (!ctx || prologue_only < 0 || prologue_only > 1 || ctas_per_block < 0 || ctas_per_block > 16) return GPSB200_ERR_ARG;
+    ctx->lanes_prologue_only = prologue_only;
+    ctx->lanes_ctas = ctas_per_block;
+    return GPSB200_OK;
+}
+
+int gpsb200_debug_lanes_image(gpsb200_ctx_t *ctx, int blk, void *dev_out, void *host_out, int64_t *bytes) {
+    if (!ctx || !bytes) return GPSB200_ERR_ARG;
+    const SynthArgs &a = ctx->last;
+    if (!ctx->have_last || !synth_lanes_applicable(a) || blk < 0 || blk >= a.nblk)
+        return fail(ctx, GPSB200_ERR_ARG, "gpsb200_debug_lanes_image: the previous call made no k_synth_lanes images");
+    const size_t n = lanes_image_host(nullptr, a.nchan, nullptr, 0, nullptr);
+    *bytes = (int64_t) n;
+    if (!dev_out || !host_out) return GPSB200_OK;
+    CU(cudaSetDevice(ctx->cfg.device));
+    CU(cudaDeviceSynchronize());
+    CU(cudaMemcpy(dev_out, (const char *) a.atab + (size_t) blk * n, n, cudaMemcpyDeviceToHost));
+    lanes_image_host(ctx->h_bc + (size_t) blk * a.nchan, a.nchan, ctx->h_nav, ctx->cfg.max_chan, host_out);
+    return GPSB200_OK;
+}
+
 int gpsb200_debug_run_checkpoints(gpsb200_ctx_t *ctx, int nblk, int nchan, void *out) {
     if (!ctx || !out || nblk < 1 || nblk > ctx->cfg.max_blocks || nchan < 1 || nchan > ctx->cfg.max_chan)
         return GPSB200_ERR_ARG;
@@ -1624,6 +1667,8 @@
     cudaStream_t s = caller_stream(ctx, stream_);
     SynthArgs a = ctx->last;
     if (dst_device) a.out = dst_device;
+    a.lanes_prologue_only = ctx->lanes_prologue_only;
+    a.lanes_ctas = ctx->lanes_ctas;
     if (kernel_mask & 8) CU(launch_tables(a, s));
     if (kernel_mask & 4) {
         CU(launch_probe(a, s));
diff --git a/multi-sdr-gps-sim_b200/csrc/rx_samples.cuh b/multi-sdr-gps-sim_b200/csrc/rx_samples.cuh
--- a/multi-sdr-gps-sim_b200/csrc/rx_samples.cuh
+++ b/multi-sdr-gps-sim_b200/csrc/rx_samples.cuh
@@ -31,6 +31,12 @@
     const short2 v = reinterpret_cast<const short2 *>(iq)[i];
     I = min(max(v.x >> 4, -128), 127);
     Q = min(max(v.y >> 4, -128), 127);
+}
+
+__device__ __forceinline__ int32_t carrier_entry(int k, double gain) {
+    const int ai = __double2int_rz(__dmul_rn((double) sine512(k + 128), gain));
+    const int aq = __double2int_rz(__dmul_rn((double) sine512(k), gain));
+    return ai + aq * 65536;
 }
 
 __device__ __forceinline__ void fill_carrier_table(int2 *tab, int nthreads) {
diff --git a/multi-sdr-gps-sim_b200/csrc/synth_kernels.cu b/multi-sdr-gps-sim_b200/csrc/synth_kernels.cu
--- a/multi-sdr-gps-sim_b200/csrc/synth_kernels.cu
+++ b/multi-sdr-gps-sim_b200/csrc/synth_kernels.cu
@@ -22,12 +22,7 @@
     const int rem = (int) (idx - (long) b * per_blk), k = rem >> 5, col = rem & 31, c = col % group;
     const BlockChanDev *bc = a.bc + (size_t) b * a.nchan;
     int32_t e = 0;
-    if (c < a.nchan && bc[c].prn > 0) {
-        const double gain = bc[c].gain;
-        const int ai = __double2int_rz(__dmul_rn((double) sine512(k + 128), gain));
-        const int aq = __double2int_rz(__dmul_rn((double) sine512(k), gain));
-        e = ai + aq * 65536;
-    }
+    if (c < a.nchan && bc[c].prn > 0) e = rx::carrier_entry(k, bc[c].gain);
     int32_t *t = a.atab + (size_t) b * kAtabRows * 32 + col;
     t[k * 32] = e;
     t[(k + 256) * 32] = -e;
@@ -438,6 +433,7 @@
 }
 
 cudaError_t launch_tables(const SynthArgs &a, cudaStream_t s) {
+    if (synth_lanes_applicable(a)) return launch_lanes_images(a, s);
     const long total = (long) a.nblk * 256 * 32;
     k_tables<<<(unsigned) ((total + 255) / 256), 256, 0, s>>>(a, group_for(a.nchan));
     return cudaGetLastError();
diff --git a/multi-sdr-gps-sim_b200/csrc/synth_kernels.h b/multi-sdr-gps-sim_b200/csrc/synth_kernels.h
--- a/multi-sdr-gps-sim_b200/csrc/synth_kernels.h
+++ b/multi-sdr-gps-sim_b200/csrc/synth_kernels.h
@@ -63,15 +63,21 @@
     void *out;
     int nblk, nchan, nruns, run_samples, runs_per_cta, ctas_per_block, iq16;
     int lanes;
+    int lanes_prologue_only;
+    int lanes_ctas;
 };
 
 cudaError_t launch_tables(const SynthArgs &a, cudaStream_t s);
+size_t synth_table_words(const SynthArgs &a);
+size_t synth_table_words_max(int max_chan);
 cudaError_t launch_probe(const SynthArgs &a, cudaStream_t s);
 cudaError_t launch_chain(const SynthArgs &a, cudaStream_t s);
 cudaError_t launch_checkpoints(const SynthArgs &a, cudaStream_t s);
 cudaError_t launch_synth(const SynthArgs &a, cudaStream_t s);
 bool synth_lanes_applicable(const SynthArgs &a);
 cudaError_t launch_synth_lanes(const SynthArgs &a, cudaStream_t s);
+cudaError_t launch_lanes_images(const SynthArgs &a, cudaStream_t s);
+size_t lanes_image_host(const BlockChanDev *bc, int nchan, const uint32_t *nav, int nav_stride, void *out);
 void synth_lanes_launch_shape(const SynthArgs &a, int *ctas, int *threads, size_t *smem, int *ctas_per_block,
                               int *runs_per_cta);
 void synth_launch_shape(const SynthArgs &a, int *ctas, int *threads, size_t *smem, int *ctas_per_block, int *runs_per_cta);
diff --git a/multi-sdr-gps-sim_b200/csrc/synth_lanes.cu b/multi-sdr-gps-sim_b200/csrc/synth_lanes.cu
--- a/multi-sdr-gps-sim_b200/csrc/synth_lanes.cu
+++ b/multi-sdr-gps-sim_b200/csrc/synth_lanes.cu
@@ -1,9 +1,14 @@
 #include <cuda_runtime.h>
 #include <stdint.h>
 
+#include <cstddef>
+#include <cstring>
+
 #include "nco_exact.h"
+#include "rx_samples.cuh"
 #include "synth_kernels.h"
 #include "synth_lanes.h"
+#include "synth_tables.h"
 
 namespace gpsb200 {
 
@@ -21,6 +26,16 @@
 struct LaneSteps {
     uint64_t D96, E96;
     uint32_t inv32, e22;
+};
+
+template <int CH>
+struct LanesImage {
+    int32_t tab[CH][512];
+    uint32_t chips[CH][kLaneChipWords];
+    uint32_t nav[CH][kNavWords];
+    uint32_t step[CH];
+    LaneSteps steps[CH];
+    uint32_t band[CH][lanes::kBandList + 1];
 };
 
 template <int CH>
@@ -33,9 +48,33 @@
     LaneSteps steps[CH];
     alignas(16) uint32_t stage[kLaneWarps][kWins * lanes::kWindow];
     uint32_t band[CH][lanes::kBandList + 1];
+    alignas(8) uint64_t bar;
 };
 template <int CH>
 constexpr size_t lanes_smem_bytes() { return sizeof(LanesSmem<CH>) + (size_t) CH * 2048; }
+
+template <int CH>
+struct LanesPieces {
+    using I = LanesImage<CH>;
+    using S = LanesSmem<CH>;
+    static constexpr uint32_t kTab = sizeof(I::tab), kChipsNav = sizeof(I::chips) + sizeof(I::nav),
+                              kSteps = sizeof(I::step) + sizeof(I::steps), kBand = sizeof(I::band);
+    static_assert(offsetof(I, nav) == offsetof(I, chips) + sizeof(I::chips) && offsetof(S, nav) == sizeof(S::chips) &&
+                      offsetof(I, steps) == offsetof(I, step) + sizeof(I::step) &&
+                      offsetof(S, steps) == offsetof(S, step) + sizeof(S::step) &&
+                      offsetof(I, band) == offsetof(I, steps) + sizeof(I::steps) && sizeof(I) == offsetof(I, band) + kBand,
+                  "contiguous pieces");
+    static_assert(kTab % 16 == 0 && kChipsNav % 16 == 0 && kSteps % 16 == 0 && kBand % 16 == 0 &&
+                      offsetof(I, chips) % 16 == 0 && offsetof(I, step) % 16 == 0 && offsetof(I, band) % 16 == 0 &&
+                      offsetof(S, step) % 16 == 0 && offsetof(S, band) % 16 == 0,
+                  "bulk copies: sizes and places multiples of 16 bytes");
+};
+
+__device__ __forceinline__ void bulk_copy(uint32_t dst, const void *src, uint32_t bytes, uint32_t bar) {
+    asm volatile("cp.async.bulk.shared::cluster.global.mbarrier::complete_tx::bytes [%0], [%1], %2, [%3];" ::"r"(dst),
+                 "l"(src), "r"(bytes), "r"(bar)
+                 : "memory");
+}
 
 template <int OFF>
 __device__ __forceinline__ int table_at(uint32_t p, uint32_t ta) {
@@ -109,42 +148,32 @@
 
     const int b = blockIdx.x / a.ctas_per_block;
     const int g = blockIdx.x - b * a.ctas_per_block;
-    const int tid = threadIdx.x, nthr = blockDim.x;
+    const int tid = threadIdx.x;
     const int lane = tid & 31, warp = tid >> 5;
     const int nchan = a.nchan;
     const BlockChanDev *bc = a.bc + (size_t) b * nchan;
 
     {
-        const int32_t *src = a.atab + (size_t) b * kAtabRows * 32;
-        for (int i = tid; i < 512 * CH; i += nthr) {
-            const int k = i / CH, c = i - k * CH;
-            tab[c * 512 + ((k + c * SWZ) & 511)] = c < nchan ? src[k * 32 + c] : 0;
-        }
-        for (int i = tid; i < CH * kLaneChipWords; i += nthr) {
-            const int c = i / kLaneChipWords, w = i - c * kLaneChipWords;
-            uint32_t v = 0;
-            if (c < nchan && bc[c].prn > 0) {
-                const uint32_t *cw = a.chipbits + bc[c].prn * kChipWords;
-                v = w < kChipWords ? cw[w] : __funnelshift_r(cw[w - 32], cw[w - 31], 1);
-            }
-            sm.chips[c][w] = v;
-        }
-        for (int i = tid; i < CH * kNavWords; i += nthr) {
-            const int c = i / kNavWords, w = i - c * kNavWords;
-            uint32_t v = 0;
-            if (c < nchan && bc[c].prn > 0) v = a.nav[((size_t) bc[c].frame * a.nav_stride + c) * kNavWords + w];
-            sm.nav[c][w] = v;
-        }
-        if (warp == kLaneWarps - 1 && lane < CH) {
-            const bool ok = lane < nchan && bc[lane].prn > 0;
-            lanes::ChanRun k;
-            lanes::init_steps(k, ok, ok ? bc[lane].c_carr : 0.0, ok ? bc[lane].c_code : 0.0);
-            sm.steps[lane] = LaneSteps{k.D96, k.E96, k.inv32, k.e22};
-            sm.step[lane] = lanes::fast_step(k);
-            lanes::band_residues(lanes::fast_step(k), &sm.band[lane][0]);
-        }
-    }
-    __syncthreads();
+        using P = LanesPieces<CH>;
+        const uint32_t bar = (uint32_t) __cvta_generic_to_shared(&sm.bar);
+        if (tid == 0) {
+            const LanesImage<CH> &src = reinterpret_cast<const LanesImage<CH> *>(a.atab)[b];
+            asm volatile("mbarrier.init.shared::cta.b64 [%0], %1;" ::"r"(bar), "r"(1) : "memory");
+            asm volatile("fence.mbarrier_init.release.cluster;" ::: "memory");
+            asm volatile("mbarrier.arrive.expect_tx.shared::cta.b64 _, [%0], %1;" ::"r"(bar),
+                         "r"(P::kTab + P::kChipsNav + P::kSteps + P::kBand)
+                         : "memory");
+            bulk_copy((uint32_t) __cvta_generic_to_shared(tab), src.tab, P::kTab, bar);
+            bulk_copy((uint32_t) __cvta_generic_to_shared(sm.chips), src.chips, P::kChipsNav, bar);
+            bulk_copy((uint32_t) __cvta_generic_to_shared(sm.step), src.step, P::kSteps, bar);
+            bulk_copy((uint32_t) __cvta_generic_to_shared(sm.band), src.band, P::kBand, bar);
+        }
+        __syncthreads();
+        asm volatile("{\n\t.reg .pred p;\n\tLANES_IMG_WAIT:\n\t"
+                     "mbarrier.test_wait.parity.shared::cta.b64 p, [%0], 0;\n\t@!p bra LANES_IMG_WAIT;\n\t}" ::"r"(bar)
+                     : "memory");
+    }
+    if (a.lanes_prologue_only) return;
 
     const int ch = lane & (CH - 1), half = lane / CH;
     const bool chan_ok = ch < nchan && bc[ch < nchan ? ch : 0].prn > 0;
@@ -264,6 +293,46 @@
     }
 }
 
+template <int CH>
+__global__ void __launch_bounds__(256) k_lanes_images(SynthArgs a) {
+    constexpr int SWZ = 32 / CH;
+    const int b = blockIdx.x, part = blockIdx.y, tid = threadIdx.x;
+    const int nchan = a.nchan;
+    const BlockChanDev *bc = a.bc + (size_t) b * nchan;
+    LanesImage<CH> &im = reinterpret_cast<LanesImage<CH> *>(a.atab)[b];
+    if (part > 0) {
+        const int c = part - 1, k = tid;
+        const int32_t e = c < nchan && bc[c].prn > 0 ? rx::carrier_entry(k, bc[c].gain) : 0;
+        im.tab[c][(k + c * SWZ) & 511] = e;
+        im.tab[c][(k + 256 + c * SWZ) & 511] = -e;
+        return;
+    }
+    if (tid < CH) {
+        const bool ok = tid < nchan && bc[tid].prn > 0;
+        lanes::ChanRun k;
+        lanes::init_steps(k, ok, ok ? bc[tid].c_carr : 0.0, ok ? bc[tid].c_code : 0.0);
+        im.steps[tid] = LaneSteps{k.D96, k.E96, k.inv32, k.e22};
+        im.step[tid] = lanes::fast_step(k);
+        lanes::band_residues(lanes::fast_step(k), &im.band[tid][0]);
+        im.band[tid][lanes::kBandList] = 0u;
+    }
+    for (int i = tid; i < CH * kLaneChipWords; i += blockDim.x) {
+        const int c = i / kLaneChipWords, w = i - c * kLaneChipWords;
+        uint32_t v = 0;
+        if (c < nchan && bc[c].prn > 0) {
+            const uint32_t *cw = a.chipbits + bc[c].prn * kChipWords;
+            v = w < kChipWords ? cw[w] : __funnelshift_r(cw[w - 32], cw[w - 31], 1);
+        }
+        im.chips[c][w] = v;
+    }
+    for (int i = tid; i < CH * kNavWords; i += blockDim.x) {
+        const int c = i / kNavWords, w = i - c * kNavWords;
+        uint32_t v = 0;
+        if (c < nchan && bc[c].prn > 0) v = a.nav[((size_t) bc[c].frame * a.nav_stride + c) * kNavWords + w];
+        im.nav[c][w] = v;
+    }
+}
+
 }
 
 bool synth_lanes_applicable(const SynthArgs &a) {
@@ -278,7 +347,7 @@
 }
 
 static void lanes_shape(const SynthArgs &a, int *ctas_per_block, int *runs_per_cta) {
-    int per_block = (40 * kLaneCtas * device_sms() + a.nblk - 1) / a.nblk;
+    int per_block = a.lanes_ctas > 0 ? a.lanes_ctas : (40 * kLaneCtas * device_sms() + a.nblk - 1) / a.nblk;
     if (per_block > 16) per_block = 16;
     if (per_block < 1) per_block = 1;
     int per_cta = (a.nruns + per_block - 1) / per_block;
@@ -294,6 +363,66 @@
     cudaError_t e = cudaFuncSetAttribute(k_synth_lanes<IQ16, CH>, cudaFuncAttributeMaxDynamicSharedMemorySize, (int) smem);
     if (e != cudaSuccess) return e;
     k_synth_lanes<IQ16, CH><<<a.nblk * a.ctas_per_block, kLaneWarps * 32, smem, s>>>(a);
+    return cudaGetLastError();
+}
+
+size_t synth_table_words(const SynthArgs &a) {
+    if (!synth_lanes_applicable(a)) return (size_t) kAtabRows * 32;
+    return (a.nchan <= 16 ? sizeof(LanesImage<16>) : sizeof(LanesImage<32>)) / 4;
+}
+
+size_t synth_table_words_max(int max_chan) {
+    const size_t img = (max_chan <= 16 ? sizeof(LanesImage<16>) : sizeof(LanesImage<32>)) / 4;
+    return img > (size_t) kAtabRows * 32 ? img : (size_t) kAtabRows * 32;
+}
+
+template <int CH>
+static void lanes_image_host_t(const BlockChanDev *bc, int nchan, const uint32_t *nav, int nav_stride, void *out) {
+    static const uint8_t q[128] = {GPSB200_QUARTER_SINE};
+    auto sine = [](int k) {
+        k &= 511;
+        const int r = k & 255, v = q[r < 128 ? r : 255 - r];
+        return k < 256 ? v : -v;
+    };
+    LanesImage<CH> &im = *static_cast<LanesImage<CH> *>(out);
+    memset(&im, 0, sizeof im);
+    for (int c = 0; c < CH; c++) {
+        const bool ok = c < nchan && bc[c].prn > 0;
+        if (ok) {
+            for (int k = 0; k < 256; k++) {
+                const int ai = (int) ((double) sine(k + 128) * bc[c].gain), aq = (int) ((double) sine(k) * bc[c].gain);
+                const int32_t e = (int32_t) ((uint32_t) ai + (uint32_t) aq * 65536u);
+                im.tab[c][(k + c * (32 / CH)) & 511] = e;
+                im.tab[c][(k + 256 + c * (32 / CH)) & 511] = (int32_t) (0u - (uint32_t) e);
+            }
+            uint8_t ca[GPSB200_CA_LEN];
+            ca_code(bc[c].prn, ca);
+            for (int n = 0; n < kLaneChipWords * 32; n++)
+                if (ca[n % GPSB200_CA_LEN]) im.chips[c][n >> 5] |= 1u << (n & 31);
+            memcpy(im.nav[c], nav + ((size_t) bc[c].frame * nav_stride + c) * kNavWords, kNavWords * 4);
+        }
+        lanes::ChanRun k;
+        lanes::init_steps(k, ok, ok ? bc[c].c_carr : 0.0, ok ? bc[c].c_code : 0.0);
+        im.steps[c] = LaneSteps{k.D96, k.E96, k.inv32, k.e22};
+        im.step[c] = lanes::fast_step(k);
+        lanes::band_residues(lanes::fast_step(k), &im.band[c][0]);
+    }
+}
+
+size_t lanes_image_host(const BlockChanDev *bc, int nchan, const uint32_t *nav, int nav_stride, void *out) {
+    if (nchan <= 16) {
+        if (out) lanes_image_host_t<16>(bc, nchan, nav, nav_stride, out);
+        return sizeof(LanesImage<16>);
+    }
+    if (out) lanes_image_host_t<32>(bc, nchan, nav, nav_stride, out);
+    return sizeof(LanesImage<32>);
+}
+
+cudaError_t launch_lanes_images(const SynthArgs &a, cudaStream_t s) {
+    if (a.nchan <= 16)
+        k_lanes_images<16><<<dim3((unsigned) a.nblk, 17), 256, 0, s>>>(a);
+    else
+        k_lanes_images<32><<<dim3((unsigned) a.nblk, 33), 256, 0, s>>>(a);
     return cudaGetLastError();
 }
 
```

Result: no change. 71340 (median of 6 runs) (-0.2%).
